# FaspDevTeam/faspsolver

Hardware: AMD Instinct MI355X
Metric: AMG-PCG solve DOF/s (3D 7-pt Poisson 256^3, classical AMG V(1,1) w-Jacobi + PCG, rtol 1e-8) (higher is better)
Workload: dtype f64

## Files before the change

### faspsolver_amd/__init__.py

```python
import ctypes as C
import os
import subprocess

import numpy as np

from . import _types as T
from ._types import *

_HERE = os.path.dirname(os.path.abspath(__file__))
LIB_PATH = os.environ.get("FASP_HIP_LIB") or os.path.join(_HERE, "libfasp_hip.so")
_lib = None

EXPORTS = [
    "fasp_param_amg_init", "fasp_param_solver_init", "fasp_solver_dcsr_krylov_amg",
    "fasp_blas_dcsr_mxv", "fasp_blas_dcsr_aAxpy", "fasp_blas_darray_dotprod",
    "fasp_blas_darray_norm2", "fasp_blas_darray_norminf", "fasp_blas_darray_axpy",
    "fasp_blas_darray_axpby", "fasp_smoother_dcsr_jacobi",
    "fasp_blas_dbsr_mxv", "fasp_blas_dbsr_aAxpy", "fasp_dbsr_getdiaginv", "fasp_smoother_dbsr_jacobi1",
    "fasp_solver_dbsr_pcg", "fasp_solver_dbsr_pbcgs", "fasp_solver_dbsr_pgmres", "fasp_solver_dbsr_pvgmres",
    "fasp_solver_dbsr_pvfgmres", "fasp_hip_bsr_precond_setup", "fasp_hip_bsr_precond_fct", "fasp_hip_bsr_precond_free",
    "fasp_hip_param_input", "fasp_fwrapper_dcsr_krylov_amg_", "fasp_dcsrvec_read2", "fasp_dvec_read",
    "fasp_dbsr_read", "fasp_dcoo_read", "fasp_dcoo_read1", "fasp_dcoo_shift_read", "fasp_dmtx_read", "fasp_dmtxsym_read", "fasp_dvec_write", "fasp_dcsr_write_coo", "fasp_dcsrvec_write2", "fasp_fwrapper_dcsr_amg_", "fasp_fwrapper_dbsr_krylov_amg_", "fasp_hip_free_bsr", "fasp_hip_comm_selftest", "fasp_hip_amg_kernel_info", "fasp_hip_coarse_kernel_info", "fasp_hip_bsr_coarse_kernel_info", "fasp_hip_coding_selftest", "fasp_solver_amg", "fasp_solver_famg", "fasp_hip_amg_solve", "fasp_precond_diag", "fasp_precond_dbsr_diag", "fasp_solver_dcsr_itsolver", "fasp_solver_dcsr_krylov", "fasp_solver_dcsr_krylov_diag", "fasp_solver_dbsr_itsolver", "fasp_solver_dbsr_krylov", "fasp_solver_dbsr_krylov_diag", "fasp_hip_mxv_csr", "fasp_hip_mxv_bsr", "fasp_solver_matfree_init", "fasp_solver_pcg", "fasp_solver_pbcgs", "fasp_solver_pgcg", "fasp_solver_pminres", "fasp_solver_pgmres", "fasp_solver_pvgmres", "fasp_solver_pvfgmres", "fasp_solver_itsolver", "fasp_solver_krylov", "fasp_solver_dcsr_pcg", "fasp_solver_dcsr_pminres", "fasp_solver_dcsr_pgcg", "fasp_solver_dcsr_pgcr", "fasp_solver_dcsr_pbcgs", "fasp_solver_dcsr_pgmres", "fasp_solver_dcsr_pvgmres",
    "fasp_solver_dcsr_pvfgmres", "fasp_hip_precond_setup", "fasp_hip_precond_fct", "fasp_hip_precond_free",
    "fasp_hip_time_bsr_mxv", "fasp_solver_dbsr_krylov_amg", "fasp_hip_bsr_amg_create", "fasp_hip_bsr_amg_create_host",
    "fasp_hip_bsr_amg_destroy", "fasp_hip_bsr_amg_num_levels", "fasp_hip_bsr_amg_get_matrix",
    "fasp_hip_bsr_amg_get_diaginv", "fasp_hip_bsr_solve",
    "fasp_hip_set_device", "fasp_hip_device_count", "fasp_hip_device_identity", "fasp_hip_available",
    "fasp_hip_amg_create", "fasp_hip_amg_create_host", "fasp_hip_amg_upload",
    "fasp_hip_amg_destroy", "fasp_hip_amg_num_levels", "fasp_hip_amg_get_matrix",
    "fasp_hip_amg_get_cfmark", "fasp_hip_solve", "fasp_hip_set_rhs", "fasp_hip_set_guess",
    "fasp_hip_solve_resident", "fasp_hip_get_solution", "fasp_hip_device_synchronize",
    "fasp_hip_precond_amg",
    "fasp_hip_poisson7pt", "fasp_hip_aniso27pt", "fasp_hip_free_system", "fasp_hip_time_kernel", "fasp_hip_measure_ceilings", "fasp_hip_amg_publish", "fasp_hip_amg_attach", "fasp_hip_amg_unpublish",
    "fasp_precond_setup", "fasp_precond_amg", "fasp_precond_famg", "fasp_precond_amli", "fasp_precond_namli", "fasp_amg_data_create", "fasp_amg_data_free", "fasp_param_amg_to_prec", "fasp_param_prec_to_amg", "fasp_mem_free", "fasp_mem_calloc", "fasp_dvec_alloc", "fasp_dvec_set", "fasp_dvec_free", "fasp_dvec_create", "fasp_dcsr_create", "fasp_dcsr_free", "fasp_smoother_dcsr_gs", "fasp_smoother_dcsr_sor", "fasp_smoother_dcsr_L1diag",
    "fasp_hip_tune", "fasp_hip_comm_unique_id", "fasp_hip_comm_init", "fasp_hip_comm_finalize",
    "fasp_hip_comm_rank", "fasp_hip_comm_size", "fasp_hip_version", "fasp_hip_comm_init_shm",
    "fasp_hip_dist_plan", "fasp_hip_dist_level_info", "fasp_hip_dist_get_matrix",
    "fasp_hip_dist_get_list",
    "fasp_blas_dcsr_vmv", "fasp_blas_dcsr_mxv_agg", "fasp_blas_dcsr_aAxpy_agg", "fasp_blas_darray_ax",
    "fasp_blas_darray_axpyz", "fasp_blas_darray_norm1", "fasp_darray_cp", "fasp_darray_set", "fasp_dvec_isnan",
    "fasp_hip_time_matrix", "fasp_hip_bsr_dist_info", "fasp_hip_seq_schedule_selftest", "fasp_hip_seq_chain_selftest", "fasp_hip_cluster_order", "fasp_hip_permute_csr", "fasp_hip_comm_init_ipc", "fasp_hip_comm_stats", "fasp_hip_comm_timing", "fasp_hip_estream_selftest", "fasp_hip_sell_selftest", "fasp_hip_level_op", "fasp_hip_matrix_op",
    "fasp_param_ilu_init", "fasp_ilu_data_create", "fasp_ilu_data_free", "fasp_mem_iludata_check", "fasp_ilu_dcsr_setup",
    "fasp_precond_ilu", "fasp_precond_ilu_forward", "fasp_precond_ilu_backward", "fasp_solver_dcsr_krylov_ilu",
    "fasp_solver_dcsr_krylov_ilu_M", "fasp_smoother_dcsr_ilu", "fasp_fwrapper_dcsr_krylov_ilu_",
    "fasp_hip_ilu_resident_count", "fasp_hip_ilu_time",
    "fasp_ilu_dbsr_setup", "fasp_precond_dbsr_ilu", "fasp_solver_dbsr_krylov_ilu", "fasp_smoother_dbsr_ilu",
    "fasp_fwrapper_dbsr_krylov_ilu_",
    "fasp_hip_bsr_amg_get_ilu", "fasp_hip_bsr_amg_ilu_info", "fasp_hip_bsr_amg_ilu_smooth_time",
]


def build(verbose=False):
    cmd = ["make", "-C", os.path.join(_HERE, "csrc")]
    if not verbose:
        cmd.insert(1, "-s")
    subprocess.run(cmd, check=True)


def lib():
    global _lib
    if _lib is not None:
        return _lib
    if not os.path.exists(LIB_PATH):
        build()
    L = C.CDLL(LIB_PATH)
    P = C.POINTER
    L.fasp_param_amg_init.argtypes = [P(T.AMG_param)]
    L.fasp_param_solver_init.argtypes = [P(T.ITS_param)]
    L.fasp_solver_dcsr_krylov_amg.argtypes = [P(T.dCSRmat), P(T.dvector), P(T.dvector),
                                              P(T.ITS_param), P(T.AMG_param)]
    L.fasp_blas_dcsr_mxv.argtypes = [P(T.dCSRmat), T.c_double_p, T.c_double_p]
    L.fasp_blas_dcsr_aAxpy.argtypes = [C.c_double, P(T.dCSRmat), T.c_double_p, T.c_double_p]
    for f in ("fasp_blas_darray_dotprod", "fasp_blas_darray_norm2", "fasp_blas_darray_norminf"):
        getattr(L, f).restype = C.c_double
    L.fasp_blas_darray_dotprod.argtypes = [C.c_int, T.c_double_p, T.c_double_p]
    L.fasp_blas_darray_norm2.argtypes = [C.c_int, T.c_double_p]
    L.fasp_blas_darray_norminf.argtypes = [C.c_int, T.c_double_p]
    L.fasp_blas_darray_axpy.argtypes = [C.c_int, C.c_double, T.c_double_p, T.c_double_p]
    L.fasp_blas_darray_axpby.argtypes = [C.c_int, C.c_double, T.c_double_p, C.c_double,
                                         T.c_double_p]
    L.fasp_blas_dcsr_vmv.restype = C.c_double
    L.fasp_blas_dcsr_vmv.argtypes = [P(T.dCSRmat), T.c_double_p, T.c_double_p]
    L.fasp_blas_dcsr_mxv_agg.argtypes = [P(T.dCSRmat), T.c_double_p, T.c_double_p]
    L.fasp_blas_dcsr_aAxpy_agg.argtypes = [C.c_double, P(T.dCSRmat), T.c_double_p, T.c_double_p]
    L.fasp_blas_darray_ax.argtypes = [C.c_int, C.c_double, T.c_double_p]
    L.fasp_blas_darray_axpyz.argtypes = [C.c_int, C.c_double, T.c_double_p, T.c_double_p, T.c_double_p]
    L.fasp_blas_darray_norm1.restype = C.c_double
    L.fasp_blas_darray_norm1.argtypes = [C.c_int, T.c_double_p]
    L.fasp_darray_cp.argtypes = [C.c_int, T.c_double_p, T.c_double_p]
    L.fasp_darray_set.argtypes = [C.c_int, T.c_double_p, C.c_double]
    L.fasp_hip_time_matrix.restype = C.c_double
    L.fasp_hip_time_matrix.argtypes = [P(T.dCSRmat), C.c_int, C.c_int, P(C.c_int)]
    L.fasp_dvec_isnan.restype = C.c_short
    L.fasp_dvec_isnan.argtypes = [P(T.dvector)]
    L.fasp_smoother_dcsr_jacobi.argtypes = [P(T.dvector), C.c_int, C.c_int, C.c_int,
                                            P(T.dCSRmat), P(T.dvector), C.c_int, C.c_double]
    L.fasp_blas_dbsr_mxv.argtypes = [P(T.dBSRmat), T.c_double_p, T.c_double_p]
    L.fasp_blas_dbsr_aAxpy.argtypes = [C.c_double, P(T.dBSRmat), T.c_double_p, T.c_double_p]
    L.fasp_dbsr_getdiaginv.argtypes = [P(T.dBSRmat)]
    L.fasp_dbsr_getdiaginv.restype = T.dvector
    L.fasp_smoother_dbsr_jacobi1.argtypes = [P(T.dBSRmat), P(T.dvector), P(T.dvector), T.c_double_p]
    L.fasp_hip_time_bsr_mxv.argtypes = [P(T.dBSRmat), C.c_int]
    L.fasp_hip_time_bsr_mxv.restype = C.c_double
    L.fasp_solver_dcsr_pcg.argtypes = [P(T.dCSRmat), P(T.dvector), P(T.dvector), P(T.precond), C.c_double,
                                       C.c_double, C.c_int, C.c_short, C.c_short]
    L.fasp_solver_dcsr_pbcgs.argtypes = L.fasp_solver_dcsr_pcg.argtypes
    L.fasp_solver_dcsr_pminres.argtypes = L.fasp_solver_dcsr_pcg.argtypes
    L.fasp_solver_dcsr_pgcg.argtypes = L.fasp_solver_dcsr_pcg.argtypes
    L.fasp_solver_dcsr_pvgmres.argtypes = [P(T.dCSRmat), P(T.dvector), P(T.dvector), P(T.precond), C.c_double,
                                           C.c_double, C.c_int, C.c_short, C.c_short, C.c_short]
    L.fasp_solver_dcsr_pvfgmres.argtypes = L.fasp_solver_dcsr_pvgmres.argtypes
    L.fasp_solver_dcsr_pgmres.argtypes = L.fasp_solver_dcsr_pvgmres.argtypes
    L.fasp_solver_dcsr_pgcr.argtypes = L.fasp_solver_dcsr_pvgmres.argtypes
    L.fasp_hip_precond_setup.argtypes = [P(T.dCSRmat), P(T.AMG_param)]
    L.fasp_hip_precond_setup.restype = P(T.precond)
    L.fasp_hip_precond_free.argtypes = [P(T.precond)]
    L.fasp_hip_precond_free.restype = None
    L.fasp_hip_precond_fct.argtypes = [T.c_double_p, T.c_double_p, C.c_void_p]
    L.fasp_hip_precond_fct.restype = None
    L.fasp_solver_dbsr_pcg.argtypes = [P(T.dBSRmat), P(T.dvector), P(T.dvector), P(T.precond), C.c_double,
                                       C.c_double, C.c_int, C.c_short, C.c_short]
    L.fasp_solver_dbsr_pbcgs.argtypes = L.fasp_solver_dbsr_pcg.argtypes
    L.fasp_solver_dbsr_pvgmres.argtypes = [P(T.dBSRmat), P(T.dvector), P(T.dvector), P(T.precond), C.c_double,
                                           C.c_double, C.c_int, C.c_short, C.c_short, C.c_short]
    L.fasp_solver_dbsr_pgmres.argtypes = L.fasp_solver_dbsr_pvgmres.argtypes
    L.fasp_solver_dbsr_pvfgmres.argtypes = L.fasp_solver_dbsr_pvgmres.argtypes
    L.fasp_hip_bsr_precond_setup.argtypes = [P(T.dBSRmat), P(T.AMG_param)]
    L.fasp_hip_bsr_precond_setup.restype = P(T.precond)
    L.fasp_hip_bsr_precond_free.argtypes = [P(T.precond)]
    L.fasp_hip_bsr_precond_free.restype = None
    L.fasp_hip_bsr_precond_fct.argtypes = [T.c_double_p, T.c_double_p, C.c_void_p]
    L.fasp_hip_bsr_precond_fct.restype = None
    L.fasp_dcsrvec_read2.argtypes = [C.c_char_p, C.c_char_p, P(T.dCSRmat), P(T.dvector)]
    L.fasp_dvec_read.argtypes = [C.c_char_p, P(T.dvector)]
    L.fasp_dbsr_read.argtypes = [C.c_char_p, P(T.dBSRmat)]
    L.fasp_hip_free_bsr.argtypes = [P(T.dBSRmat)]
    L.fasp_hip_free_bsr.restype = None
    L.fasp_hip_param_input.argtypes = [C.c_char_p, P(T.ITS_param), P(T.AMG_param)]
    L.fasp_fwrapper_dcsr_krylov_amg_.argtypes = [P(C.c_int), P(C.c_int), T.c_int_p, T.c_int_p, T.c_double_p,
                                                 T.c_double_p, T.c_double_p, P(C.c_double), P(C.c_int), P(C.c_int)]
    L.fasp_fwrapper_dcsr_krylov_amg_.restype = None
    L.fasp_hip_coding_selftest.argtypes = [P(T.dCSRmat), P(C.c_int)]
    L.fasp_hip_amg_kernel_info.argtypes = [C.c_void_p, C.c_int, C.c_int, P(C.c_int), P(C.c_double)]
    L.fasp_hip_coarse_kernel_info.argtypes = [C.c_void_p, P(C.c_int)]
    L.fasp_hip_bsr_coarse_kernel_info.argtypes = [C.c_void_p, P(C.c_int)]
    L.fasp_solver_amg.argtypes = [P(T.dCSRmat), P(T.dvector), P(T.dvector), P(T.AMG_param)]
    L.fasp_hip_amg_solve.argtypes = [C.c_void_p, P(T.dvector), P(T.dvector), P(T.AMG_param), T.c_double_p,
                                     C.c_int, P(T.fasp_hip_stats)]
    L.fasp_solver_dbsr_krylov_amg.argtypes = [P(T.dBSRmat), P(T.dvector), P(T.dvector), P(T.ITS_param),
                                              P(T.AMG_param)]
    L.fasp_hip_bsr_amg_create.argtypes = [P(C.c_void_p), P(T.dBSRmat), P(T.AMG_param)]
    L.fasp_hip_bsr_amg_create_host.argtypes = [P(C.c_void_p), P(T.dBSRmat), P(T.AMG_param)]
    L.fasp_hip_bsr_amg_destroy.argtypes = [C.c_void_p]
    L.fasp_hip_bsr_amg_destroy.restype = None
    L.fasp_hip_bsr_amg_num_levels.argtypes = [C.c_void_p]
    L.fasp_hip_bsr_amg_get_matrix.argtypes = [C.c_void_p, C.c_int, C.c_int, P(T.dBSRmat)]
    L.fasp_hip_bsr_amg_get_diaginv.argtypes = [C.c_void_p, C.c_int]
    L.fasp_hip_bsr_amg_get_diaginv.restype = T.c_double_p
    L.fasp_hip_bsr_solve.argtypes = [C.c_void_p, P(T.dvector), P(T.dvector), P(T.ITS_param), T.c_double_p,
                                     C.c_int, P(T.fasp_hip_stats)]
    L.fasp_hip_amg_create.argtypes = [P(C.c_void_p), P(T.dCSRmat), P(T.AMG_param)]
    L.fasp_hip_amg_create_host.argtypes = L.fasp_hip_amg_create.argtypes
    L.fasp_hip_amg_upload.argtypes = [C.c_void_p]
    L.fasp_hip_amg_destroy.argtypes = [C.c_void_p]
    L.fasp_hip_amg_destroy.restype = None
    L.fasp_hip_amg_num_levels.argtypes = [C.c_void_p]
    L.fasp_hip_amg_get_matrix.argtypes = [C.c_void_p, C.c_int, C.c_int, P(T.dCSRmat)]
    L.fasp_hip_amg_get_cfmark.argtypes = [C.c_void_p, C.c_int, P(T.ivector)]
    L.fasp_hip_solve.argtypes = [C.c_void_p, P(T.dvector), P(T.dvector), P(T.ITS_param),
                                 T.c_double_p, C.c_int, P(T.fasp_hip_stats)]
    L.fasp_hip_set_rhs.argtypes = [C.c_void_p, P(T.dvector)]
    L.fasp_hip_set_guess.argtypes = [C.c_void_p, P(T.dvector)]
    L.fasp_hip_get_solution.argtypes = [C.c_void_p, P(T.dvector)]
    L.fasp_hip_solve_resident.argtypes = [C.c_void_p, P(T.ITS_param), T.c_double_p, C.c_int,
                                          P(T.fasp_hip_stats)]
    L.fasp_hip_precond_amg.argtypes = [C.c_void_p, T.c_double_p, T.c_double_p]
    L.fasp_hip_poisson7pt.argtypes = [C.c_int, C.c_int, C.c_int, P(T.dCSRmat), P(T.dvector),
                                      P(T.dvector)]
    L.fasp_hip_aniso27pt.argtypes = [C.c_int, C.c_double, C.c_double, C.c_double, P(T.dCSRmat), P(T.dvector)]
    L.fasp_hip_free_system.argtypes = [P(T.dCSRmat), P(T.dvector), P(T.dvector)]
    L.fasp_hip_free_system.restype = None
    L.fasp_hip_measure_ceilings.argtypes = [P(C.c_double), C.c_size_t, C.c_int]
    L.fasp_hip_amg_publish.argtypes = [C.c_void_p, C.c_char_p]
    L.fasp_hip_amg_attach.argtypes = [P(C.c_void_p), C.c_char_p]
    L.fasp_hip_amg_unpublish.argtypes = [C.c_char_p]
    L.fasp_hip_time_kernel.restype = C.c_double
    L.fasp_hip_time_kernel.argtypes = [C.c_void_p, C.c_int, C.c_int, C.c_int]
    L.fasp_hip_tune.argtypes = [C.c_char_p, C.c_int]
    L.fasp_hip_comm_unique_id.argtypes = [C.c_char_p]
    L.fasp_hip_comm_init.argtypes = [C.c_int, C.c_int, C.c_char_p]
    L.fasp_hip_version.restype = C.c_char_p
    L.fasp_hip_comm_init_shm.argtypes = [C.c_int, C.c_int, C.c_char_p]
    L.fasp_hip_dist_plan.argtypes = [C.c_void_p, C.c_int, C.c_int, C.c_int]
    L.fasp_hip_dist_level_info.argtypes = [C.c_void_p, C.c_int, T.c_int_p]
    L.fasp_hip_dist_get_matrix.argtypes = [C.c_void_p, C.c_int, C.c_int, P(T.dCSRmat)]
    L.fasp_hip_dist_get_list.argtypes = [C.c_void_p, C.c_int, C.c_int, P(T.ivector)]
    _lib = L
    L.fasp_param_ilu_init.argtypes = [P(T.ILU_param)]
    L.fasp_param_ilu_init.restype = None
    L.fasp_ilu_data_create.argtypes = [C.c_int, C.c_int, P(T.ILU_data)]
    L.fasp_ilu_data_create.restype = None
    L.fasp_ilu_data_free.argtypes = [P(T.ILU_data)]
    L.fasp_ilu_data_free.restype = None
    L.fasp_mem_iludata_check.argtypes = [P(T.ILU_data)]
    L.fasp_mem_iludata_check.restype = C.c_short
    L.fasp_ilu_dcsr_setup.argtypes = [P(T.dCSRmat), P(T.ILU_data), P(T.ILU_param)]
    L.fasp_ilu_dcsr_setup.restype = C.c_short
    for f in ("fasp_precond_ilu", "fasp_precond_ilu_forward", "fasp_precond_ilu_backward"):
        getattr(L, f).argtypes = [T.c_double_p, T.c_double_p, C.c_void_p]
        getattr(L, f).restype = None
    L.fasp_solver_dcsr_krylov_ilu.argtypes = [P(T.dCSRmat), P(T.dvector), P(T.dvector), P(T.ITS_param), P(T.ILU_param)]
    L.fasp_solver_dcsr_krylov_ilu_M.argtypes = [P(T.dCSRmat), P(T.dvector), P(T.dvector), P(T.ITS_param),
                                                P(T.ILU_param), P(T.dCSRmat)]
    L.fasp_smoother_dcsr_ilu.argtypes = [P(T.dCSRmat), P(T.dvector), P(T.dvector), C.c_void_p]
    L.fasp_smoother_dcsr_ilu.restype = None
    L.fasp_fwrapper_dcsr_krylov_ilu_.argtypes = [P(C.c_int), P(C.c_int), T.c_int_p, T.c_int_p, T.c_double_p,
                                                 T.c_double_p, T.c_double_p, P(C.c_double), P(C.c_int), P(C.c_int)]
    L.fasp_fwrapper_dcsr_krylov_ilu_.restype = None
    L.fasp_hip_ilu_time.argtypes = [P(T.ILU_data), C.c_int, C.c_int, T.c_double_p]
    L.fasp_hip_ilu_time.restype = C.c_double
    L.fasp_ilu_dbsr_setup.argtypes = [P(T.dBSRmat), P(T.ILU_data), P(T.ILU_param)]
    L.fasp_ilu_dbsr_setup.restype = C.c_short
    L.fasp_precond_dbsr_ilu.argtypes = [T.c_double_p, T.c_double_p, C.c_void_p]
    L.fasp_precond_dbsr_ilu.restype = None
    L.fasp_solver_dbsr_krylov_ilu.argtypes = [P(T.dBSRmat), P(T.dvector), P(T.dvector), P(T.ITS_param), P(T.ILU_param)]
    L.fasp_solver_dbsr_krylov_ilu.restype = C.c_int
    L.fasp_smoother_dbsr_ilu.argtypes = [P(T.dBSRmat), P(T.dvector), P(T.dvector), C.c_void_p]
    L.fasp_smoother_dbsr_ilu.restype = None
    L.fasp_fwrapper_dbsr_krylov_ilu_.argtypes = [P(C.c_int), P(C.c_int), P(C.c_int), T.c_int_p, T.c_int_p, T.c_double_p,
                                                 T.c_double_p, T.c_double_p, P(C.c_double), P(C.c_int), P(C.c_int)]
    L.fasp_fwrapper_dbsr_krylov_ilu_.restype = None
    L.fasp_hip_bsr_amg_get_ilu.argtypes = [C.c_void_p, C.c_int, P(T.ILU_data)]
    L.fasp_hip_bsr_amg_ilu_info.argtypes = [C.c_void_p, C.c_int, T.c_double_p]
    L.fasp_hip_bsr_amg_ilu_smooth_time.argtypes = [C.c_void_p, C.c_int, C.c_int]
    L.fasp_hip_bsr_amg_ilu_smooth_time.restype = C.c_double
    return L


def solve_bsr_ilu(ia, ja, val, nb, b, x0=None, solver=None, tol=1e-8, maxit=500, lfil=0, print_level=0):
    L = lib()
    ia = np.ascontiguousarray(ia, dtype=np.int32); ja = np.ascontiguousarray(ja, dtype=np.int32)
    val = np.ascontiguousarray(val, dtype=np.float64); b = np.ascontiguousarray(b, dtype=np.float64)
    x = np.zeros(len(b)) if x0 is None else np.array(x0, dtype=np.float64)
    A = T.dBSRmat()
    A.ROW = A.COL = len(ia) - 1; A.NNZ = len(ja); A.nb = nb; A.storage_manner = 0
    A.IA = ia.ctypes.data_as(T.c_int_p); A.JA = ja.ctypes.data_as(T.c_int_p); A.val = val.ctypes.data_as(T.c_double_p)
    bv = T.dvector(len(b), b.ctypes.data_as(T.c_double_p)); xv = T.dvector(len(x), x.ctypes.data_as(T.c_double_p))
    it = T.ITS_param(); L.fasp_param_solver_init(C.byref(it))
    it.itsolver_type = T.SOLVER_BiCGstab if solver is None else solver
    it.tol, it.maxit, it.print_level = tol, maxit, print_level
    prm = T.ILU_param(); L.fasp_param_ilu_init(C.byref(prm))
    prm.ILU_lfil, prm.print_level = lfil, print_level
    st = L.fasp_solver_dbsr_krylov_ilu(C.byref(A), C.byref(bv), C.byref(xv), C.byref(it), C.byref(prm))
    return st, x


def available():
    return bool(lib().fasp_hip_available())


def param_amg_init():
    p = T.AMG_param()
    lib().fasp_param_amg_init(C.byref(p))
    return p


def param_solver_init():
    p = T.ITS_param()
    lib().fasp_param_solver_init(C.byref(p))
    return p


def poisson7pt(nx, ny=None, nz=None):
    ny = nx if ny is None else ny
    nz = nx if nz is None else nz
    A = T.dCSRmat(); b = T.dvector(); u = T.dvector()
    st = lib().fasp_hip_poisson7pt(nx, ny, nz, C.byref(A), C.byref(b), C.byref(u))
    if st < 0:
        raise RuntimeError(f"fasp_hip_poisson7pt failed: {st}")
    ia, ja, a = T.csr_arrays(A)
    f = np.ctypeslib.as_array(b.val, (b.row,)).copy()
    ue = np.ctypeslib.as_array(u.val, (u.row,)).copy()
    lib().fasp_hip_free_system(C.byref(A), C.byref(b), C.byref(u))
    return ia, ja, a, f, ue


def poisson7pt_var(n, p7=None):
    ia, ja, a, f, _ue = p7 if p7 is not None else poisson7pt(n)
    m = len(f)
    h = 1.0 / (n + 1)
    idx = np.arange(m, dtype=np.int64)
    xi = (idx % n + 1) * h
    yi = ((idx // n) % n + 1) * h
    zi = (idx // (n * n) + 1) * h
    kap = 1.0 + 0.8 * np.sin(2 * np.pi * xi) * np.sin(2 * np.pi * yi) * np.sin(2 * np.pi * zi)
    del xi, yi, zi
    cnt = np.diff(ia)
    rows = np.repeat(idx, cnt)
    off = ja != rows
    a2 = np.where(off, a * 0.5 * (kap[rows] + kap[ja]), 0.0)
    rowsum = np.bincount(rows, weights=a2, minlength=m)
    diag = -rowsum + (7 - cnt) * kap / (h * h)
    a2[ia[:-1]] = diag
    return ia, ja, a2, f.copy()


def aniso27pt(n, kx=1.0, ky=1.0, kz=0.01):
    A = T.dCSRmat(); b = T.dvector()
    st = lib().fasp_hip_aniso27pt(n, kx, ky, kz, C.byref(A), C.byref(b))
    if st < 0:
        raise RuntimeError(f"fasp_hip_aniso27pt failed: {st}")
    ia, ja, a = T.csr_arrays(A)
    f = np.ctypeslib.as_array(b.val, (b.row,)).copy()
    lib().fasp_hip_free_system(C.byref(A), C.byref(b), None)
    return ia, ja, a, f


def solver_dcsr_krylov_amg(ia, ja, a, b, x, itparam, amgparam):
    A, _keep = T.as_csr(ia, ja, a)
    bv, _b = T.as_vec(b)
    assert x.dtype == np.float64 and x.flags["C_CONTIGUOUS"]
    xv = T.dvector(x.shape[0], x.ctypes.data_as(T.c_double_p))
    return lib().fasp_solver_dcsr_krylov_amg(C.byref(A), C.byref(bv), C.byref(xv),
                                             C.byref(itparam), C.byref(amgparam))


class AMG:

    def __init__(self, ia, ja, a, amgparam, host_only=False):
        self._A, self._keep = T.as_csr(ia, ja, a)
        self.h = C.c_void_p()
        fn = lib().fasp_hip_amg_create_host if host_only else lib().fasp_hip_amg_create
        self.status = fn(C.byref(self.h), C.byref(self._A), C.byref(amgparam))
        if self.status < 0:
            self.h = C.c_void_p()
            raise RuntimeError(f"fasp_hip_amg_create failed with status {self.status}")
        self.n = self._A.row

    @classmethod
    def attach(cls, name):
        self = cls.__new__(cls)
        self._A = None; self._keep = None
        self.h = C.c_void_p()
        self.status = lib().fasp_hip_amg_attach(C.byref(self.h), name.encode())
        if self.status < 0:
            self.h = C.c_void_p()
            raise RuntimeError(f"fasp_hip_amg_attach({name}) failed with status {self.status}")
        v = T.dCSRmat()
        lib().fasp_hip_amg_get_matrix(self.h, 0, 0, C.byref(v))
        self.n = v.row
        return self

    def publish(self, name):
        st = lib().fasp_hip_amg_publish(self.h, name.encode())
        if st < 0:
            raise RuntimeError(f"fasp_hip_amg_publish({name}) failed with status {st}")

    @staticmethod
    def unpublish(name):
        lib().fasp_hip_amg_unpublish(name.encode())

    @property
    def num_levels(self):
        return lib().fasp_hip_amg_num_levels(self.h)

    def upload(self):
        st = lib().fasp_hip_amg_upload(self.h)
        if st < 0:
            raise RuntimeError(f"fasp_hip_amg_upload failed with status {st}")

    def matrix(self, level, which):
        v = T.dCSRmat()
        st = lib().fasp_hip_amg_get_matrix(self.h, level, which, C.byref(v))
        if st < 0:
            raise IndexError((level, which))
        ia, ja, val = T.csr_arrays(v)
        return v.row, v.col, ia, ja, val

    def cfmark(self, level):
        v = T.ivector()
        if lib().fasp_hip_amg_get_cfmark(self.h, level, C.byref(v)) < 0:
            raise IndexError(level)
        return np.ctypeslib.as_array(v.val, (v.row,)).copy()

    def solve(self, b, itparam, x0=None, hist_cap=600):
        x = np.zeros(self.n) if x0 is None else np.ascontiguousarray(x0, dtype=np.float64).copy()
        bv, _b = T.as_vec(b)
        xv, x = T.as_vec(x)
        hist = np.zeros(hist_cap)
        stats = T.fasp_hip_stats()
        st = lib().fasp_hip_solve(self.h, C.byref(bv), C.byref(xv), C.byref(itparam),
                                  T.dp(hist), hist_cap, C.byref(stats))
        return st, x, hist[:max(stats.nhist, 0)].copy(), stats

    def amg_solve(self, b, amgparam=None, x0=None, hist_cap=600):
        x = np.zeros(self.n) if x0 is None else np.ascontiguousarray(x0, dtype=np.float64).copy()
        bv, _b = T.as_vec(b)
        xv, x = T.as_vec(x)
        hist = np.zeros(hist_cap)
        stats = T.fasp_hip_stats()
        st = lib().fasp_hip_amg_solve(self.h, C.byref(bv), C.byref(xv),
                                      C.byref(amgparam) if amgparam is not None else None,
                                      T.dp(hist), hist_cap, C.byref(stats))
        return st, x, hist[:max(min(stats.nhist, hist_cap), 0)].copy(), stats

    def set_rhs(self, b):
        bv, _b = T.as_vec(b)
        st = lib().fasp_hip_set_rhs(self.h, C.byref(bv))
        if st < 0:
            raise RuntimeError(f"fasp_hip_set_rhs failed: {st}")

    def solve_resident(self, itparam, hist_cap=600):
        st = lib().fasp_hip_set_guess(self.h, None)
        if st < 0:
            raise RuntimeError(f"fasp_hip_set_guess failed: {st}")
        hist = np.zeros(hist_cap)
        stats = T.fasp_hip_stats()
        st = lib().fasp_hip_solve_resident(self.h, C.byref(itparam), T.dp(hist), hist_cap,
                                           C.byref(stats))
        return st, hist[:max(stats.nhist, 0)].copy(), stats

    def get_solution(self):
        x = np.zeros(self.n)
        xv, x = T.as_vec(x)
        st = lib().fasp_hip_get_solution(self.h, C.byref(xv))
        if st < 0:
            raise RuntimeError(f"fasp_hip_get_solution failed: {st}")
        return x

    def kernel_info(self, level, which=0):
        k = C.c_int(0); b = C.c_double(0)
        if lib().fasp_hip_amg_kernel_info(self.h, level, which, C.byref(k), C.byref(b)) < 0:
            raise IndexError((level, which))
        return k.value, b.value

    def coarse_kernel_info(self):
        info = (C.c_int * 8)()
        if lib().fasp_hip_coarse_kernel_info(self.h, info) < 0:
            raise RuntimeError("fasp_hip_coarse_kernel_info failed")
        return tuple(info)

    def precond(self, r):
        r = np.ascontiguousarray(r, dtype=np.float64)
        z = np.zeros_like(r)
        st = lib().fasp_hip_precond_amg(self.h, T.dp(r), T.dp(z))
        if st < 0:
            raise RuntimeError(f"fasp_hip_precond_amg failed: {st}")
        return z

    def dist_plan(self, rank, nranks, min_rows):
        st = lib().fasp_hip_dist_plan(self.h, rank, nranks, min_rows)
        if st < 0:
            raise RuntimeError(f"fasp_hip_dist_plan failed: {st}")

    def dist_info(self, level):
        info = (C.c_int * 8)()
        if lib().fasp_hip_dist_level_info(self.h, level, info) < 0:
            raise IndexError(level)
        keys = ("replicated", "nglobal", "row0", "nloc", "nghost", "nsend", "first_replicated", "nranks")
        return dict(zip(keys, list(info)))

    def dist_matrix(self, level, which):
        v = T.dCSRmat()
        if lib().fasp_hip_dist_get_matrix(self.h, level, which, C.byref(v)) < 0:
            raise IndexError((level, which))
        ia, ja, val = T.csr_arrays(v)
        return v.row, v.col, ia, ja, val

    def dist_list(self, level, which):
        v = T.ivector()
        if lib().fasp_hip_dist_get_list(self.h, level, which, C.byref(v)) < 0:
            raise IndexError((level, which))
        if v.row == 0:
            return np.zeros(0, np.int32)
        return np.ctypeslib.as_array(v.val, (v.row,)).copy()

    def time_kernel(self, kind, level=0, reps=20):
        return lib().fasp_hip_time_kernel(self.h, kind, level, reps)

    def close(self):
        if self.h:
            lib().fasp_hip_amg_destroy(self.h)
            self.h = C.c_void_p()

    def __del__(self):
        try:
            self.close()
        except Exception:
            pass


class BSRAMG:

    def __init__(self, ia, ja, val, nb, amgparam, host_only=False):
        self._A, self._keep = T.as_bsr(ia, ja, val, nb)
        self.h = C.c_void_p()
        fn = lib().fasp_hip_bsr_amg_create_host if host_only else lib().fasp_hip_bsr_amg_create
        self.status = fn(C.byref(self.h), C.byref(self._A), C.byref(amgparam))
        if self.status < 0:
            self.h = C.c_void_p()
            raise RuntimeError(f"fasp_hip_bsr_amg_create failed with status {self.status}")
        self.nb = nb
        self.n = self._A.ROW * nb

    @property
    def num_levels(self):
        return lib().fasp_hip_bsr_amg_num_levels(self.h)

    def matrix(self, level, which):
        v = T.dBSRmat()
        if lib().fasp_hip_bsr_amg_get_matrix(self.h, level, which, C.byref(v)) < 0:
            raise IndexError((level, which))
        ia = np.ctypeslib.as_array(v.IA, (v.ROW + 1,)).copy()
        ja = np.ctypeslib.as_array(v.JA, (max(v.NNZ, 1),))[:v.NNZ].copy()
        nv = v.NNZ * v.nb * v.nb
        val = np.ctypeslib.as_array(v.val, (max(nv, 1),))[:nv].copy()
        return v.ROW, v.COL, v.NNZ, ia, ja, val

    def diaginv(self, level):
        p = lib().fasp_hip_bsr_amg_get_diaginv(self.h, level)
        if not p:
            return None
        v = T.dBSRmat()
        lib().fasp_hip_bsr_amg_get_matrix(self.h, level, 0, C.byref(v))
        return np.ctypeslib.as_array(p, (v.ROW * v.nb * v.nb,)).copy()

    def ilu(self, level):
        d = T.ILU_data()
        st = lib().fasp_hip_bsr_amg_get_ilu(self.h, level, C.byref(d))
        if st < 0:
            raise IndexError(level)
        if st == 0:
            return None
        return {"nb": d.nb, "row": d.row, "nzlu": d.nzlu,
                "ijlu": np.ctypeslib.as_array(d.ijlu, (d.nzlu,)).copy(),
                "luval": np.ctypeslib.as_array(d.luval, (d.nzlu * d.nb * d.nb,)).copy()}

    def ilu_info(self, level):
        info = np.zeros(6)
        st = lib().fasp_hip_bsr_amg_ilu_info(self.h, level, T.dp(info))
        if st < 0:
            raise IndexError(level)
        return tuple(int(v) for v in info) if st else None

    def ilu_smooth_time(self, level=0, reps=20):
        return lib().fasp_hip_bsr_amg_ilu_smooth_time(self.h, level, reps)

    def solve(self, b, itparam, x0=None, hist_cap=1200):
        x = np.zeros(self.n) if x0 is None else np.ascontiguousarray(x0, dtype=np.float64).copy()
        bv, _b = T.as_vec(b)
        xv, x = T.as_vec(x)
        hist = np.zeros(hist_cap)
        stats = T.fasp_hip_stats()
        st = lib().fasp_hip_bsr_solve(self.h, C.byref(bv), C.byref(xv), C.byref(itparam), T.dp(hist),
                                      hist_cap, C.byref(stats))
        return st, x, hist[:max(min(stats.nhist, hist_cap), 0)].copy(), stats

    def precond(self, r):
        r = np.ascontiguousarray(r, dtype=np.float64).copy()
        z = np.zeros_like(r)
        lib().fasp_hip_bsr_precond_fct(T.dp(r), T.dp(z), self.h)
        return z

    def coarse_kernel_info(self):
        info = (C.c_int * 8)()
        if lib().fasp_hip_bsr_coarse_kernel_info(self.h, info) < 0:
            raise RuntimeError("fasp_hip_bsr_coarse_kernel_info failed")
        return tuple(info)

    def dist_info(self):
        info = (C.c_int * 6)()
        lib().fasp_hip_bsr_dist_info(self.h, info)
        return {"replicated": info[0], "row0": info[1], "nloc": info[2], "nghost": info[3], "first_replicated": info[4], "nb": info[5]}

    def free(self):
        if self.h:
            lib().fasp_hip_bsr_amg_destroy(self.h)
            self.h = C.c_void_p()

    def __del__(self):
        try:
            self.free()
        except Exception:
            pass


def solver_dbsr_krylov_amg(ia, ja, val, nb, b, x, itparam, amgparam):
    A, _keep = T.as_bsr(ia, ja, val, nb)
    bv, _b = T.as_vec(b)
    assert x.dtype == np.float64 and x.flags.c_contiguous
    xv = T.dvector(len(x), T.dp(x))
    return lib().fasp_solver_dbsr_krylov_amg(C.byref(A), C.byref(bv), C.byref(xv), C.byref(itparam),
                                             C.byref(amgparam))

# ... 8 lines not shown
```

### faspsolver_amd/csrc/coarse_cg.hip.h

```cpp

static bool small_coarse_ok(long long rows, long long stored_values)
{
    static int enabled = -1;
    if (enabled < 0) {
        const char* e = std::getenv("FASP_HIP_SMALL_COARSE");
        enabled = (e && std::atoi(e) == 0) ? 0 : 1;
    }
    return enabled && rows <= 4096 && stored_values <= 131072;
}
static SmallOut* small_out_dev() { return reinterpret_cast<SmallOut*>(g_ctx.d_partials2); }
static int small_out_fetch(SmallOut& o)
{
    HIPCK(hipMemcpyAsync(g_ctx.h_part, g_ctx.d_partials2, sizeof(SmallOut), hipMemcpyDeviceToHost, g_ctx.stream));
    HIPCK(hipStreamSynchronize(g_ctx.stream));
    std::memcpy(&o, g_ctx.h_part, sizeof(SmallOut));
    return 0;
}

static bool g_persist_disabled = false;
static bool build_persist_plan(fasp_hip_amg* h, int level)
{
    auto& P = h->persist;
    if (P.tried) return P.ok;
    P.tried = true;
    const HostCSR& A = h->H.L[(size_t)level].A;
    const int m = A.row;
    const int nblocks = g_ctx.num_cu, nw = (nblocks - 1) * 8;
    if (m < 1 || m > 6144 || m != A.col || nw < 8 || A.nnz <= 0) return false;
    std::vector<int> order((size_t)m), slots((size_t)m);
    for (int i = 0; i < m; ++i) { order[(size_t)i] = i; slots[(size_t)i] = (A.ia[i + 1] - A.ia[i] + 63) / 64; }
    std::stable_sort(order.begin(), order.end(), [&](int x, int y) { return slots[(size_t)x] > slots[(size_t)y]; });
    std::vector<int> load((size_t)nw, 0), cnt((size_t)nw, 0), wrow((size_t)nw * 8, -1), wend((size_t)nw * 8, 0);
    std::vector<std::pair<int, int>> heap;
    for (int w = 0; w < nw; ++w) heap.emplace_back(0, w);
    auto cmp = [](const std::pair<int, int>& x, const std::pair<int, int>& y) { return x > y; };
    std::make_heap(heap.begin(), heap.end(), cmp);
    for (int i : order) {
        if (slots[(size_t)i] == 0) continue;
        std::pop_heap(heap.begin(), heap.end(), cmp);
        std::pair<int, int> top = heap.back();
        const int w = top.second;
        if (cnt[(size_t)w] >= 8) return false;
        load[(size_t)w] += slots[(size_t)i];
        wrow[(size_t)w * 8 + cnt[(size_t)w]] = i;
        wend[(size_t)w * 8 + cnt[(size_t)w]] = load[(size_t)w];
        cnt[(size_t)w]++;
        heap.back() = std::make_pair(load[(size_t)w], w);
        std::push_heap(heap.begin(), heap.end(), cmp);
    }
    for (int i = 0; i < m; ++i) if (slots[(size_t)i] == 0) return false;
    const int maxload = *std::max_element(load.begin(), load.end());
    const int NE = maxload <= 32 ? 32 : maxload <= 48 ? 48 : maxload <= 56 ? 56 : maxload <= 64 ? 64 : 0;
    if (!NE) return false;
    const size_t tot = (size_t)nw * NE * 64;
    Buf<double> vals(tot);
    Buf<unsigned short> cols(tot);
    std::memset(vals.data(), 0, tot * sizeof(double));
    std::memset(cols.data(), 0, tot * sizeof(unsigned short));
#pragma omp parallel for schedule(dynamic, 16)
    for (int w = 0; w < nw; ++w) {
        int base = 0;
        for (int j = 0; j < cnt[(size_t)w]; ++j) {
            const int row = wrow[(size_t)w * 8 + j];
            const int kb = A.ia[row], len = A.ia[row + 1] - kb;
            for (int e = 0; e < len; ++e) {
                const size_t at = ((size_t)w * NE + base + e / 64) * 64 + (size_t)(e % 64);
                vals[at] = A.val[kb + e];
                cols[at] = (unsigned short)(A.ja[kb + e] * 8);
            }
            base = wend[(size_t)w * 8 + j];
        }
    }
    bool ok = hipMalloc(&P.vals, tot * sizeof(double)) == hipSuccess && hipMalloc(&P.cols, tot * sizeof(unsigned short)) == hipSuccess &&
              hipMalloc(&P.wrow, sizeof(int) * (size_t)nw * 8) == hipSuccess && hipMalloc(&P.wend, sizeof(int) * (size_t)nw * 8) == hipSuccess &&
              hipMalloc(&P.t2, sizeof(double) * 4 * (size_t)m) == hipSuccess && hipMalloc(&P.sync, 1024) == hipSuccess;
    if (ok) ok = hipMemcpy(P.vals, vals.data(), tot * sizeof(double), hipMemcpyHostToDevice) == hipSuccess &&
                 hipMemcpy(P.cols, cols.data(), tot * sizeof(unsigned short), hipMemcpyHostToDevice) == hipSuccess &&
                 hipMemcpy(P.wrow, wrow.data(), sizeof(int) * (size_t)nw * 8, hipMemcpyHostToDevice) == hipSuccess &&
                 hipMemcpy(P.wend, wend.data(), sizeof(int) * (size_t)nw * 8, hipMemcpyHostToDevice) == hipSuccess;
    if (ok) ok = hipMemset(P.t2, 0, sizeof(double) * 4 * (size_t)m) == hipSuccess;
    if (!ok) return false;
    P.NE = NE; P.nblocks = nblocks; P.ok = true;
    return true;
}

template <int NE>
static int launch_spcg_persist(const SpcgPersistArgs& pa, size_t lds)
{
    static bool attr = false;
    if (!attr) {
        HIPCK(hipFuncSetAttribute((const void*)k_spcg_persist<NE>, hipFuncAttributeMaxDynamicSharedMemorySize, 160 * 1024 - 1024));
        attr = true;
    }
    hipLaunchKernelGGL(k_spcg_persist<NE>, dim3(pa.nblocks - (g_tune.spcg_test_hang ? 1 : 0)), dim3(512), lds, g_ctx.stream, pa);
    return FASP_SUCCESS;
}

static int coarse_spcg(fasp_hip_amg* h, DevLevel& D, double tol, int prtlvl)
{
    const DevCSR& A = D.A;
    const int m = A.row;
    const int nn = (int)((unsigned)m * (unsigned)m);
    const int MaxIt = std::max(250, std::min(nn, 1000));
    if (small_coarse_ok(m, A.nnz)) {
        SpcgArgs a{};
        a.A = SmallCSR{m, A.ia, A.ja, A.val};
        a.b = D.b; a.u = D.x; a.p = h->cp; a.r = h->cr; a.t = h->ct; a.u_best = h->cbest;
        a.tol = tol; a.MaxIt = MaxIt; a.x_zero = D.x_zero ? 1 : 0; a.out = small_out_dev(); a.nnz = A.nnz;
        a.lazy = h->lazy_active ? h->d_lazy : nullptr;
        const size_t lds_v = sizeof(double) * 5 * (size_t)m;
        const size_t lds_m = 12 * (size_t)A.nnz + 4 * ((size_t)m + 1);
        static bool attr = false;
        if (!attr) {
            (void)hipFuncSetAttribute((const void*)k_spcg_small<true, true>, hipFuncAttributeMaxDynamicSharedMemorySize, 150 * 1024);
            (void)hipFuncSetAttribute((const void*)k_spcg_small<true, false>, hipFuncAttributeMaxDynamicSharedMemorySize, 150 * 1024);
            attr = true;
        }
        int LD = m; while (LD % 32 != 1) ++LD;
        const size_t lds_w = sizeof(double) * (128 * (size_t)LD + 128);
        const bool one_wave = g_tune.small_onewave && m <= 128 && lds_w <= 148 * 1024;
        if (one_wave && g_tune.small_onewave >= 3) {
            const int NBK = m <= 64 ? 4 : m <= 96 ? 6 : 8, DUP = NBK == 4 ? 4 : 2, RB = NBK / DUP;
            if (!h->reg_img || h->reg_mc != -NBK) {
                const HostCSR& Ah = h->H.L.back().A;
                const int NT = 16 * NBK * DUP;
                std::vector<double> img((size_t)RB * 16 * NT, 0.0);
                for (int row = 0; row < m; ++row)
                    for (int k = Ah.ia[row]; k < Ah.ia[row + 1]; ++k) {
                        const int c = Ah.ja[k], cb = c >> 4, j = c & 15, rb = row >> 4, l = row & 15;
                        const int half = rb / RB, kk = rb % RB, g = half * NBK + cb;
                        img[(size_t)(kk * 16 + j) * NT + 16 * g + l] += Ah.val[k];
                    }
                if (h->reg_img) (void)hipFree(h->reg_img);
                HIPCK(hipMalloc((void**)&h->reg_img, sizeof(double) * img.size()));
                HIPCK(hipMemcpy(h->reg_img, img.data(), sizeof(double) * img.size(), hipMemcpyHostToDevice));
                h->reg_mc = -NBK;
            }
            a.img = h->reg_img;
            const bool ahead = g_tune.small_onewave >= 4;
            h->coarse_kinfo[0] = 1; h->coarse_kinfo[1] = NBK; h->coarse_kinfo[2] = ahead ? 1 : 0;
            if (NBK == 4 && ahead) hipLaunchKernelGGL((k_spcg_dpp<4, 4, true>), dim3(1), dim3(320), 0, g_ctx.stream, a, LD);
            else if (NBK == 4) hipLaunchKernelGGL((k_spcg_dpp<4, 4, false>), dim3(1), dim3(256), 0, g_ctx.stream, a, LD);
            else if (NBK == 6 && ahead) hipLaunchKernelGGL((k_spcg_dpp<6, 2, true>), dim3(1), dim3(256), 0, g_ctx.stream, a, LD);
            else if (NBK == 6) hipLaunchKernelGGL((k_spcg_dpp<6, 2, false>), dim3(1), dim3(192), 0, g_ctx.stream, a, LD);
            else if (ahead) hipLaunchKernelGGL((k_spcg_dpp<8, 2, true>), dim3(1), dim3(320), 0, g_ctx.stream, a, LD);
            else hipLaunchKernelGGL((k_spcg_dpp<8, 2, false>), dim3(1), dim3(256), 0, g_ctx.stream, a, LD);
        }
        else if (one_wave && g_tune.small_onewave >= 2) {
            const int MC = m <= 64 ? 32 : m <= 96 ? 48 : 64;
            if (!h->reg_img || h->reg_mc != MC) {
                const HostCSR& Ah = h->H.L.back().A;
                std::vector<double> img((size_t)MC * SPCG_REG_NT, 0.0);
                for (int row = 0; row < m; ++row)
                    for (int k = Ah.ia[row]; k < Ah.ia[row + 1]; ++k) {
                        const int c = Ah.ja[k], hh = (c >> 1) & 1, kk = 2 * (c >> 2) + (c & 1);
                        if (kk < MC) img[(size_t)kk * SPCG_REG_NT + 2 * row + hh] += Ah.val[k];
                    }
                if (h->reg_img) (void)hipFree(h->reg_img);
                HIPCK(hipMalloc((void**)&h->reg_img, sizeof(double) * img.size()));
                HIPCK(hipMemcpy(h->reg_img, img.data(), sizeof(double) * img.size(), hipMemcpyHostToDevice));
                h->reg_mc = MC;
            }
            a.img = h->reg_img;
            static bool attr_r = false;
            if (!attr_r) {
                (void)hipFuncSetAttribute((const void*)k_spcg_reg<32>, hipFuncAttributeMaxDynamicSharedMemorySize, 150 * 1024);
                (void)hipFuncSetAttribute((const void*)k_spcg_reg<48>, hipFuncAttributeMaxDynamicSharedMemorySize, 150 * 1024);
                (void)hipFuncSetAttribute((const void*)k_spcg_reg<64>, hipFuncAttributeMaxDynamicSharedMemorySize, 150 * 1024);
                attr_r = true;
            }
            const size_t lds_r = sizeof(double) * (2 * (size_t)MC + 4);
            h->coarse_kinfo[0] = 2; h->coarse_kinfo[1] = MC; h->coarse_kinfo[2] = 0;
            if (m <= 64) hipLaunchKernelGGL(k_spcg_reg<32>, dim3(1), dim3(SPCG_REG_NT), lds_r, g_ctx.stream, a, LD);
            else if (m <= 96) hipLaunchKernelGGL(k_spcg_reg<48>, dim3(1), dim3(SPCG_REG_NT), lds_r, g_ctx.stream, a, LD);
            else hipLaunchKernelGGL(k_spcg_reg<64>, dim3(1), dim3(SPCG_REG_NT), lds_r, g_ctx.stream, a, LD);
        }
        else if (one_wave) {
            static bool attr_w = false;
            if (!attr_w) { (void)hipFuncSetAttribute((const void*)k_spcg_wave, hipFuncAttributeMaxDynamicSharedMemorySize, 150 * 1024); attr_w = true; }
            hipLaunchKernelGGL(k_spcg_wave, dim3(1), dim3(64), lds_w, g_ctx.stream, a, LD);
            h->coarse_kinfo[0] = 3; h->coarse_kinfo[1] = 0; h->coarse_kinfo[2] = 0;
        }
        else if (g_tune.small_lds && lds_v + lds_m <= 148 * 1024) {
            hipLaunchKernelGGL((k_spcg_small<true, true>), dim3(1), dim3(SMALL_BLOCK), lds_v + lds_m, g_ctx.stream, a);
            h->coarse_kinfo[0] = 4; h->coarse_kinfo[1] = 2; h->coarse_kinfo[2] = 0;
        }
        else if (g_tune.small_lds && lds_v <= 148 * 1024) {
            hipLaunchKernelGGL((k_spcg_small<true, false>), dim3(1), dim3(SMALL_BLOCK), lds_v, g_ctx.stream, a);
            h->coarse_kinfo[0] = 4; h->coarse_kinfo[1] = 1; h->coarse_kinfo[2] = 0;
        }
        else {
            hipLaunchKernelGGL((k_spcg_small<false, false>), dim3(1), dim3(SMALL_BLOCK), 0, g_ctx.stream, a);
            h->coarse_kinfo[0] = 4; h->coarse_kinfo[1] = 0; h->coarse_kinfo[2] = 0;
        }
        D.x_zero = false;
        if (a.lazy) return FASP_SUCCESS;
        SmallOut o;
        if (small_out_fetch(o) < 0) return ERROR_MISC;
        h->coarse_iters += o.iters;
        if (std::getenv("FASP_HIP_DEBUG_COARSE")) std::printf("[coarse small] status %d iters %d relres %.6e\n", o.status, o.iters, o.relres);
        return o.status;
    }
    const double maxdiff = tol * STAG_RATIO;
    int iter = 0, stag = 1, more_step = 1, iter_best = 0;
    double absres0 = BIGREAL, absres = BIGREAL, relres = BIGREAL, normu = BIGREAL, normr0 = BIGREAL;
    double reldiff, factor, alpha = 0.0, beta, temp1, temp2, absres_best = BIGREAL;
    double *p = h->cp, *r = h->cr, *t = h->ct, *u_best = h->cbest, *u = D.x;
    const double* b = D.b;
    double red[8];
    hipStream_t s = g_ctx.stream;
    (void)prtlvl;

    const bool fused = g_tune.spcg_fused && m <= 8000 && A.val && A.ja && !A.code && !A.pat;
    bool persist = fused && g_tune.spcg_persist && !g_persist_disabled && !comm_shares_devices() &&
                   (size_t)m * 24 <= 150 * 1024 && build_persist_plan(h, (int)(&D - &h->L[0]));
    if (!h->spcg_state) HIPCK(hipMalloc(&h->spcg_state, sizeof(SpcgState)));
    if (fused) {
        if (!D.x_zero) d_resid(A, u, b, r);
        SpcgInitArgs ia{};
        ia.m = m; ia.x_zero = D.x_zero ? 1 : 0; ia.MaxIt = MaxIt; ia.tol = tol; ia.maxdiff = maxdiff;
        ia.b = b; ia.u = u; ia.r = r; ia.p = p; ia.u_best = u_best; ia.st = h->spcg_state;
        hipLaunchKernelGGL(k_spcg_init, dim3(1), dim3(512), 0, s, ia);
        D.x_zero = false;
        goto ITERATE;
    }

    HIPCK(hipMemsetAsync(u_best, 0, sizeof(double) * m, s));

    if (D.x_zero) {
        HIPCK(hipMemcpyAsync(r, b, sizeof(double) * m, hipMemcpyDeviceToDevice, s));
        HIPCK(hipMemsetAsync(u, 0, sizeof(double) * m, s));
        D.x_zero = false;
    } else {
        d_resid(A, u, b, r);
    }
    if (d_dot(m, r, r, red) < 0) return ERROR_MISC;
    absres0 = std::sqrt(red[0]);
    normr0  = std::max(SMALLREAL, absres0);
    relres  = absres0 / normr0;
    if (relres < tol) goto FINISHED;
    HIPCK(hipMemcpyAsync(p, r, sizeof(double) * m, hipMemcpyDeviceToDevice, s));
    temp1 = red[0];

ITERATE:
    {
        int batch = std::max(1, std::min(g_tune.spcg_batch > 0 ? g_tune.spcg_batch : 8, 64));
        const int batch_next = batch;
        if (fused && h->spcg_last_iters > 0) batch = std::max(4, std::min(h->spcg_last_iters + 1, 96));
        SpcgState S{};
        if (!fused) {
            S.temp1 = temp1; S.temp1_prev = temp1; S.absres_best = absres_best; S.normr0 = normr0; S.tol = tol;
            S.maxdiff = maxdiff; S.iter = 0; S.iter_best = 0; S.stag = stag; S.MaxIt = MaxIt; S.stop = SPCG_RUN;
            S.absres = absres; S.relres = relres; S.alpha = 0.0;
            HIPCK(hipMemcpyAsync(h->spcg_state, &S, sizeof(S), hipMemcpyHostToDevice, s));
        }
        double *R[2] = {r, nullptr}, *P[2] = {p, nullptr}, *T[2] = {t, nullptr};
        SpcgBc* bc = nullptr;
        int  cur = 0;
        bool first = true;
        if (fused) {
            if (!h->spcg_fused_buf) HIPCK(hipMalloc(&h->spcg_fused_buf, sizeof(double) * (3 * (size_t)m + 4)));
            R[1] = h->spcg_fused_buf; P[1] = R[1] + m; T[1] = P[1] + m;
            bc = reinterpret_cast<SpcgBc*>(T[1] + m);
        }
        for (;;) {
            if (persist) {
                auto& PP = h->persist;
                PP.launches = (PP.launches + 1u) & 0x1fffffu;
                if (PP.launches == 0u) { HIPCK(hipMemsetAsync(PP.t2, 0, sizeof(double) * 4 * (size_t)m, s)); PP.launches = 1u; }
                SpcgPersistArgs pa{};
                pa.epoch0 = PP.launches << 11;
                pa.m = m; pa.max_steps = MaxIt + 2; pa.nblocks = PP.nblocks; pa.st = h->spcg_state;
                pa.r = r; pa.p = p; pa.u = u; pa.u_best = u_best; pa.t2 = PP.t2; pa.sync = PP.sync;
                pa.vals = PP.vals; pa.cols = PP.cols; pa.wrow = PP.wrow; pa.wend = PP.wend;
                HIPCK(hipMemsetAsync(PP.sync, 0, 1024, s));
                pa.u_lds = (sizeof(double) * 4 * (size_t)m + 1024 <= 160 * 1024) ? 1 : 0;
                const size_t lds = sizeof(double) * (pa.u_lds ? 4 : 3) * (size_t)m;
                int lst;
                if (PP.NE == 32) lst = launch_spcg_persist<32>(pa, lds);
                else if (PP.NE == 48) lst = launch_spcg_persist<48>(pa, lds);
                else if (PP.NE == 56) lst = launch_spcg_persist<56>(pa, lds);
                else lst = launch_spcg_persist<64>(pa, lds);
                if (lst < 0) return lst;
                h->coarse_kinfo[0] = 6; h->coarse_kinfo[1] = PP.NE; h->coarse_kinfo[2] = pa.u_lds;
            }
            for (int q = 0; q < batch && fused && !persist; ++q) {
                SpcgFusedArgs fa{};
                fa.m = m; fa.first = first ? 1 : 0; fa.in = cur; fa.st = h->spcg_state; fa.bc = bc;
                fa.ia = A.ia; fa.ja = A.ja; fa.ja16 = A.jbase ? nullptr : A.ja16; fa.val = A.val;
                for (int k = 0; k < 2; ++k) { fa.r[k] = R[k]; fa.p[k] = P[k]; fa.t[k] = T[k]; }
                fa.u = u; fa.u_best = u_best;
                const int cap = g_tune.spcg_grid > 0 ? g_tune.spcg_grid : 2 * g_ctx.num_cu - 1;
                const dim3 grid(1 + std::max(1, std::min((m + 7) / 8, cap)));
                const size_t lds = sizeof(double) * (size_t)m;
                if (m <= 512 * 4) hipLaunchKernelGGL(k_spcg_fused<4>, grid, dim3(512), lds, s, fa);
                else if (m <= 512 * 10) hipLaunchKernelGGL(k_spcg_fused<10>, grid, dim3(512), lds, s, fa);
                else hipLaunchKernelGGL(k_spcg_fused<16>, grid, dim3(512), lds, s, fa);
                h->coarse_kinfo[0] = 5; h->coarse_kinfo[1] = m <= 512 * 4 ? 4 : m <= 512 * 10 ? 10 : 16; h->coarse_kinfo[2] = 0;
                cur ^= 1; first = false;
            }
            for (int q = 0; q < batch && !fused; ++q) {
                CsrArgs a{}; a.x = p; a.y = t; a.dotv = p; a.partials = g_ctx.d_partials; a.stop = &h->spcg_state->stop;
                SpcgStepArgs sa{};
                sa.m = m; sa.st = h->spcg_state; sa.t = t; sa.p = p; sa.u = u; sa.r = r; sa.u_best = u_best;
                sa.ntp = launch_csr<OP_MXV_DOT>(A, a);
                sa.tp_partials = g_ctx.d_partials;
                if (m <= 512 * 4) hipLaunchKernelGGL(k_spcg_step_reg<4>, dim3(1), dim3(512), 0, s, sa);
                else if (m <= 512 * 10) hipLaunchKernelGGL(k_spcg_step_reg<10>, dim3(1), dim3(512), 0, s, sa);
                else hipLaunchKernelGGL(k_spcg_step, dim3(1), dim3(SMALL_BLOCK), 0, s, sa);
                h->coarse_kinfo[0] = 7; h->coarse_kinfo[1] = m <= 512 * 4 ? 4 : m <= 512 * 10 ? 10 : 0; h->coarse_kinfo[2] = 0;
            }
            bool spec_rr = false;
            if (persist && g_tune.spcg_spec) {
                d_resid(A, u, b, t);
                if (d_dot_to(m, t, t, 14, false) < 0) return ERROR_MISC;
                spec_rr = true;
            }
            HIPCK(hipMemcpyAsync(g_ctx.h_part, h->spcg_state, sizeof(SpcgState), hipMemcpyDeviceToHost, s));
            static_assert(sizeof(SpcgState) % 8 == 0 && sizeof(SpcgState) + 24 <= sizeof(double) * 64, "the error word and the speculative norm travel behind the state");
            if (persist) HIPCK(hipMemcpyAsync(reinterpret_cast<char*>(g_ctx.h_part) + sizeof(SpcgState), h->persist.sync, 16, hipMemcpyDeviceToHost, s));
            if (spec_rr) HIPCK(hipMemcpyAsync(reinterpret_cast<char*>(g_ctx.h_part) + sizeof(SpcgState) + 16, g_ctx.d_red + 14, 8, hipMemcpyDeviceToHost, s));
            HIPCK(hipStreamSynchronize(s));
            std::memcpy(&S, g_ctx.h_part, sizeof(S));
            double spec_val = 0.0;
            if (spec_rr) std::memcpy(&spec_val, reinterpret_cast<char*>(g_ctx.h_part) + sizeof(SpcgState) + 16, 8);
            if (persist) {
                unsigned ew[4];
                std::memcpy(ew, reinterpret_cast<char*>(g_ctx.h_part) + sizeof(SpcgState), 16);
                if (ew[3] != 0u && S.stop == SPCG_RUN) S.stop = SPCG_HANG;
            }
            iter = S.iter; absres_best = S.absres_best; iter_best = S.iter_best;
            batch = batch_next;
            if (fused) {
                normr0 = S.normr0;
                if (S.stop == SPCG_ZERO_RHS) { relres = S.relres; goto FINISHED; }
            }
#ifdef SPCG_PERSIST_STAMPS
            if (persist) {
                unsigned dbg[64];
                (void)hipMemcpy(dbg, h->persist.sync, sizeof(dbg), hipMemcpyDeviceToHost);
                std::printf("[persist stamps, 10 ns ticks, %d steps] lead:", S.iter);
                for (int q = 0; q < 8; ++q) std::printf(" %u", dbg[32 + q]);
                std::printf(" | block 1:");
                for (int q = 0; q < 8; ++q) std::printf(" %u", dbg[40 + q]);
                std::printf("   (spmv meet(second group of records + verdict) read step(tail) pass1-2 pass3 first-group-of-records(block 1) poll-rounds)\n");
            }
#endif
            if (S.stop == SPCG_HANG) {
                std::fprintf(stderr, "### WARNING: fasp_hip: the persistent coarse CG kernel timed out waiting for a block that was not "
                                     "resident (is another process using this GPU?); continuing with the per-iteration kernels\n");
                g_persist_disabled = true;
                persist = false;
                S.stop = SPCG_RUN;
                HIPCK(hipMemcpyAsync(h->spcg_state, &S, sizeof(S), hipMemcpyHostToDevice, s));
                HIPCK(hipStreamSynchronize(s));
                cur = 0; first = true;
                continue;
            }
            if (S.stop == SPCG_RUN) continue;
            if (fused && !persist) { cur = S.pad; r = R[cur]; p = P[cur]; first = true; }
            temp2 = S.tp; temp1 = S.temp1_prev;
            red[0] = S.rr; red[1] = S.uu; red[2] = S.pp; red[3] = S.maxu; red[4] = S.nan;
            alpha = S.alpha; absres = S.absres; relres = S.relres;
            if (S.stop == SPCG_DIV0) goto RESTORE_BESTSOL;
            factor = absres / absres0; (void)factor; (void)alpha;
            if (S.stop == SPCG_NAN) { absres = BIGREAL; goto RESTORE_BESTSOL; }
            if (S.stop == SPCG_SOLSTAG) { iter = ERROR_SOLVER_SOLSTAG; break; }
            if (S.stop == SPCG_MAXIT) { iter = MaxIt + 1; break; }
            normu = std::sqrt(red[1]);
            reldiff = std::fabs(S.alpha) * std::sqrt(red[2]) / normu;
            if ((stag <= MAX_STAG) & (reldiff < maxdiff)) {
                spec_rr = false;
                d_resid(A, u, b, r);
                if (d_dot(m, r, r, red) < 0) return ERROR_MISC;
                absres = std::sqrt(red[0]);
                relres = absres / normr0;
                if (relres < tol) break;
                if (stag >= MAX_STAG) { iter = ERROR_SOLVER_STAG; break; }
                HIPCK(hipMemsetAsync(p, 0, sizeof(double) * m, s));
                ++stag;
            }
            if (relres < tol) {
                if (spec_rr && S.stop != SPCG_HANG) red[0] = spec_val;
                else {
                    spec_rr = false;
                    d_resid(A, u, b, r);
                    if (d_dot(m, r, r, red) < 0) return ERROR_MISC;
                }
                absres = std::sqrt(red[0]);
                relres = absres / normr0;
                if (relres < tol) break;
                if (spec_rr) HIPCK(hipMemcpyAsync(r, t, sizeof(double) * m, hipMemcpyDeviceToDevice, s));
                if (more_step >= MAX_RESTART) { iter = ERROR_SOLVER_TOLSMALL; break; }
                HIPCK(hipMemsetAsync(p, 0, sizeof(double) * m, s));
                ++more_step;
            }
            absres0 = absres;
            temp2 = red[0];
            beta = temp2 / temp1;
            temp1 = temp2;
            d_axpby(m, 1.0, r, beta, p);
            S.temp1 = temp1; S.temp1_prev = temp1; S.stag = stag; S.stop = SPCG_RUN;
            HIPCK(hipMemcpyAsync(h->spcg_state, &S, sizeof(S), hipMemcpyHostToDevice, s));
            HIPCK(hipStreamSynchronize(s));
        }
    }

RESTORE_BESTSOL:
    if (iter != iter_best) {
        d_resid(A, u_best, b, r);
        if (d_dot(m, r, r, red) < 0) return ERROR_MISC;
        absres_best = std::sqrt(red[0]);
        if (absres > absres_best + maxdiff || std::isnan(absres)) {
            HIPCK(hipMemcpyAsync(u, u_best, sizeof(double) * m, hipMemcpyDeviceToDevice, s));
            relres = absres_best / normr0;
        }
    }
FINISHED:
    if (std::getenv("FASP_HIP_DEBUG_COARSE")) std::printf("[coarse batched] iter %d relres %.6e absres %.6e best %d\n", iter, relres, absres, iter_best);
    if (iter > 0) { h->coarse_iters += iter; h->spcg_last_iters = iter; }
    if (iter > MaxIt) return ERROR_SOLVER_MAXIT;
    return iter;
}
```

### faspsolver_amd/csrc/device_csr.hip.h

```cpp

struct DevCSR {
    int     row = 0, col = 0, nnz = 0;
    int*    ia  = nullptr;
    int*    ja  = nullptr;
    double* val = nullptr;
    int*    dpos = nullptr;
    bool    dup_diag = false;
    bool    sorted = false;
    int     lanes = 8;
    int     kind = 0;
    int     tile_rows = 256;
    int     wrows = 64, wcap = 512;
    unsigned char* code = nullptr;
    int*    rowbase = nullptr;
    int*    doff = nullptr;
    double* dval = nullptr;
    unsigned short* pat = nullptr;
    int*    pstart = nullptr;
    int*    plen = nullptr;
    int*    poff = nullptr;
    double* pval = nullptr;
    int     npat = 0, npent = 0;
    unsigned short* ja16 = nullptr;
    int*            jbase = nullptr;
// ... 829 lines not shown
    HIPCK(hipMalloc(&D.sell_tab, sizeof(double) * (size_t)S.nv));
    HIPCK(hipMemcpy(D.sell_code, S.code.data(), sizeof(unsigned) * (size_t)S.slots, hipMemcpyHostToDevice));
    HIPCK(hipMemcpy(D.sell_meta, meta.data(), sizeof(int) * meta.size(), hipMemcpyHostToDevice));
    HIPCK(hipMemcpy(D.sell_rlen, S.rlen.data(), (size_t)H.row, hipMemcpyHostToDevice));
    HIPCK(hipMemcpy(D.sell_tab, S.tab.data(), sizeof(double) * (size_t)S.nv, hipMemcpyHostToDevice));
    D.sell_nv = S.nv; D.sell_obits = S.obits; D.sell_nslice = S.nslice; D.sell_slots = S.slots;
    return FASP_SUCCESS;
}

static int upload_csr(const HostCSR& H, DevCSR& D)
{
    D.row = H.row; D.col = H.col; D.nnz = H.nnz;
    HIPCK(hipMalloc(&D.ia, sizeof(int) * ((size_t)H.row + 1)));
    HIPCK(hipMalloc(&D.ja, sizeof(int) * std::max<size_t>(H.nnz, 1)));
    HIPCK(hipMalloc(&D.val, sizeof(double) * (std::max<size_t>(H.nnz, 1) + 2)));
    HIPCK(hipMemsetAsync(D.val + std::max<size_t>(H.nnz, 1), 0, sizeof(double) * 2, g_ctx.stream));
    HIPCK(hipMemcpyAsync(D.ia, H.ia.data(), sizeof(int) * ((size_t)H.row + 1), hipMemcpyHostToDevice, g_ctx.stream));
    pick_kernel(D);
    auto upload_plain = [&]() -> int {
        HIPCK(hipMemcpyAsync(D.ja, H.ja.data(), sizeof(int) * (size_t)H.nnz, hipMemcpyHostToDevice, g_ctx.stream));
        HIPCK(hipMemcpyAsync(D.val, H.val.data(), sizeof(double) * (size_t)H.nnz, hipMemcpyHostToDevice, g_ctx.stream));
        return 0;
    };
    if (compress_enabled() && H.nnz >= 4096 && (double)H.nnz <= 48.0 * H.row) {
        Buf<unsigned short> pat; Buf<int> prb;
        std::vector<int> pstart, plen, poff; std::vector<double> pval;
        static const bool rowpat_on = !(std::getenv("FASP_HIP_ROWPAT") && std::atoi(std::getenv("FASP_HIP_ROWPAT")) == 0);
        if (rowpat_on && build_rowpat(H, pat, pstart, plen, poff, pval, prb)) {
            D.npat = (int)pstart.size(); D.npent = (int)poff.size();
            HIPCK(hipMalloc(&D.pat, sizeof(unsigned short) * ((size_t)H.row + 2)));
            HIPCK(hipMalloc(&D.pstart, sizeof(int) * pstart.size()));
            HIPCK(hipMalloc(&D.plen, sizeof(int) * plen.size()));
            HIPCK(hipMemcpy(D.plen, plen.data(), sizeof(int) * plen.size(), hipMemcpyHostToDevice));
            HIPCK(hipMalloc(&D.poff, sizeof(int) * std::max<size_t>(poff.size(), 1)));
            HIPCK(hipMalloc(&D.pval, sizeof(double) * std::max<size_t>(pval.size(), 1)));
            HIPCK(hipMemset(D.pat + H.row, 0xff, sizeof(unsigned short) * 2));
            HIPCK(hipMemcpy(D.pat, pat.data(), sizeof(unsigned short) * (size_t)H.row, hipMemcpyHostToDevice));
            HIPCK(hipMemcpy(D.pstart, pstart.data(), sizeof(int) * pstart.size(), hipMemcpyHostToDevice));
            HIPCK(hipMemcpy(D.poff, poff.data(), sizeof(int) * poff.size(), hipMemcpyHostToDevice));
            HIPCK(hipMemcpy(D.pval, pval.data(), sizeof(double) * pval.size(), hipMemcpyHostToDevice));
            if (prb.n) {
                HIPCK(hipMalloc(&D.rowbase, sizeof(int) * ((size_t)H.row + 2)));
                HIPCK(hipMemcpy(D.rowbase, prb.data(), sizeof(int) * (size_t)H.row, hipMemcpyHostToDevice));
                const int nr = H.row, npair = (nr + 1) / 2;
                long long nx = 0;
#pragma omp parallel for schedule(static) reduction(+ : nx)
                for (int w0 = 0; w0 < nr; w0 += 128) {
                    const int    pm = std::min((w0 + 64) / 2, npair - 1);
                    const unsigned domA = pat[(size_t)2 * pm], domB = (2 * pm + 1 < nr) ? pat[(size_t)2 * pm + 1] : 0xffffu;
                    for (int r = w0; r < std::min(w0 + 128, nr); r += 2) {
                        const bool vb = r + 1 < nr;
                        if (!(vb && pat[r] == domA && pat[r + 1] == domB)) nx += vb ? 2 : 1;
                    }
                }
                if (nx * 4 <= nr) D.nxrows = (int)nx;
            } else {
                D.plane = grid_plane_of(poff, H.row);
                if (std::getenv("FASP_HIP_SETUP_TIMING")) std::printf("        [upload_csr %d x %d, %d nnz] %d row patterns; grid plane for the XCD strips: %d rows\n", H.row, H.col, H.nnz, (int)pstart.size(), D.plane);
                const int nr = H.row, npair = (nr + 1) / 2;
                long long nx = 0;
#pragma omp parallel for schedule(static) reduction(+ : nx)
                for (int w0 = 0; w0 < nr; w0 += 128) {
                    const unsigned dom = pat[(size_t)2 * std::min((w0 + 64) / 2, npair - 1)];
                    for (int r = w0; r < std::min(w0 + 128, nr); r += 2) {
                        const bool vb = r + 1 < nr;
                        if (!(vb && pat[r] == dom && pat[r + 1] == dom)) nx += vb ? 2 : 1;
                    }
                }
                if (nx * 4 <= nr) D.nxrows = (int)nx;
            }
            D.kind = 2;
            return upload_plain() < 0 ? ERROR_ALLOC_MEM : FASP_SUCCESS;
        }
        std::vector<int> doff; std::vector<double> dval;
        Buf<unsigned char> code; Buf<int> rowbase;
        if (build_dict8(H, doff, dval, code, rowbase)) {
            HIPCK(hipMalloc(&D.code, (size_t)H.nnz + 256));
            HIPCK(hipMalloc(&D.doff, sizeof(int) * 256));
            HIPCK(hipMalloc(&D.dval, sizeof(double) * 256));
            HIPCK(hipMemcpy(D.code, code.data(), (size_t)H.nnz, hipMemcpyHostToDevice));
            HIPCK(hipMemcpy(D.doff, doff.data(), sizeof(int) * 256, hipMemcpyHostToDevice));
            HIPCK(hipMemcpy(D.dval, dval.data(), sizeof(double) * 256, hipMemcpyHostToDevice));
            if (rowbase.n) {
                HIPCK(hipMalloc(&D.rowbase, sizeof(int) * (size_t)H.row));
                HIPCK(hipMemcpy(D.rowbase, rowbase.data(), sizeof(int) * (size_t)H.row, hipMemcpyHostToDevice));
            }
            D.kind = 2;
            return upload_plain() < 0 ? ERROR_ALLOC_MEM : FASP_SUCCESS;
        }
    }
    static const bool sort_long = !(std::getenv("FASP_HIP_SORT_LONG_ROWS") && std::atoi(std::getenv("FASP_HIP_SORT_LONG_ROWS")) == 0);
    static const int  sort_stream = std::getenv("FASP_HIP_SORT_STREAM") ? std::atoi(std::getenv("FASP_HIP_SORT_STREAM")) : 0;
    const double avg_len = H.row > 0 ? (double)H.nnz / H.row : 0.0;
    const bool do_sort = sort_long && !g_oneshot_upload && H.nnz > 0 && (D.kind == 0 || (D.kind == 2 && sort_stream > 0 && avg_len >= sort_stream));
    static const bool timing = std::getenv("FASP_HIP_SETUP_TIMING") != nullptr;
    double tp = wall_seconds();
    auto lap = [&](const char* what) {
        if (!timing) return;
        const double now = wall_seconds();
        std::printf("        [upload_csr %d x %d, %d nnz] %-10s %8.3f s\n", H.row, H.col, H.nnz, what, now - tp);
        tp = now;
    };
    if (do_sort && D.kind == 0) {
        int maxlen = 0;
#pragma omp parallel for schedule(static) reduction(max : maxlen)
        for (int i = 0; i < H.row; ++i) maxlen = std::max(maxlen, H.ia[i + 1] - H.ia[i]);
        if (g_device_sort && maxlen <= SORT_MAXLEN) {
            const int st = upload_sorted_on_device(H, D, maxlen);
            lap("device sort");
            return st < 0 ? st : build_estream(H.ia.data(), H.row, H.nnz, D);
        }
    }
    if (do_sort) {
        Buf<int> sj((size_t)H.nnz);
        Buf<double> sv((size_t)H.nnz);
        std::vector<int> dp;
        const bool square = H.row == H.col;
        if (square) dp.assign((size_t)H.row, -1);
#pragma omp parallel
        {
            std::vector<std::pair<int, double>> tmp;
#pragma omp for schedule(dynamic, 64)
            for (int i = 0; i < H.row; ++i) {
                const int kb = H.ia[i], ke = H.ia[i + 1];
                tmp.resize((size_t)(ke - kb));
                for (int k = kb; k < ke; ++k) tmp[(size_t)(k - kb)] = {H.ja[k], H.val[k]};
                std::stable_sort(tmp.begin(), tmp.end(),
                                 [](const std::pair<int, double>& x, const std::pair<int, double>& y) { return x.first < y.first; });
                for (int k = kb; k < ke; ++k) {
                    sj[k] = tmp[(size_t)(k - kb)].first; sv[k] = tmp[(size_t)(k - kb)].second;
                    if (square && sj[k] == i) dp[(size_t)i] = k;
                }
            }
        }
        lap("row sort");
        HIPCK(hipMemcpy(D.ja, sj.data(), sizeof(int) * (size_t)H.nnz, hipMemcpyHostToDevice));
        HIPCK(hipMemcpy(D.val, sv.data(), sizeof(double) * (size_t)H.nnz, hipMemcpyHostToDevice));
        lap("memcpy");
        if (square && D.kind == 2) {
            HIPCK(hipMalloc(&D.dpos, sizeof(int) * (size_t)std::max(H.row, 1)));
            HIPCK(hipMemcpy(D.dpos, dp.data(), sizeof(int) * (size_t)H.row, hipMemcpyHostToDevice));
        }
        D.sorted = true;
        if (upload_ja16(D, H.ia.data(), sj.data()) < 0) return ERROR_ALLOC_MEM;
        return build_estream(H.ia.data(), H.row, H.nnz, D);
    }
    if (upload_plain() < 0) return ERROR_ALLOC_MEM;
    if (D.kind == 2 && !g_oneshot_upload && build_xtile(H, D) < 0) return ERROR_ALLOC_MEM;
    if (D.kind == 2 && compress_enabled() && upload_sell(H, D) < 0) return ERROR_ALLOC_MEM;
    if (upload_ja16(D, H.ia.data(), H.ja.data()) < 0) return ERROR_ALLOC_MEM;
    return build_estream(H.ia.data(), H.row, H.nnz, D);
}

struct Tuning { int ilu_smooth_fused = 1, gen2 = 2, ws2_bpc = 3, maxgrid = -1, xcd = 16, nt = 1, kind = -1, lanes = -1, wrows = -1, wcap = -1, compress = 1, rpl = -1, lds_tab = 1, xcd_pat = 64, spcg_batch = 16, small_lds = 1, ja16 = 1, spcg_fused = 1, spcg_grid = 0, spcg_persist = 1, split_rows = 0, gs_multicolor = 0, seq_flow = 1, seq_strip_kb = 0, seq_jobs = 1, seq_spine = 1, seq_grid = 0, seq_chain = 1, seq_chain_n1 = 0, seq_chain_grid = 0, seq_chain_ref = 0, seq_test_hang = 0, seq_rest_lanes = 0, local_square = 1, fuse_zr = 1, fuse_presmooth = 1, seq_lanes = 0, xtile = 1, rp5_max = 45, rp_bpc = 5, rp_xcd = -1, rp_strip = 2, spcg_test_hang = 0, small_onewave = 4, lazy_coarse = 1, rp_stream = -1, renumber = 1, renumber_chunk = 262144, pcg_dev_beta = 1, spcg_spec = 1, ev_every = 4, pcg_fold = 1, seq_chain_touch = 8, seq_chain_touch_t1 = 1, seq_zero_skip = 1, estream = 1, es_dbg = 0, ilu_form = -1, sell = 1; };
static Tuning g_tune;

template <class K>
static int resident_blocks_per_cu(K kernel)
{
    static std::vector<std::pair<const void*, int>> cache;
    const void* key = reinterpret_cast<const void*>(kernel);
    for (const auto& e : cache)
        if (e.first == key) return e.second;
    int nb = 0;
    if (hipOccupancyMaxActiveBlocksPerMultiprocessor(&nb, kernel, BLOCK, 0) != hipSuccess || nb < 1) nb = 4;
    nb = std::min(nb, 8);
    cache.emplace_back(key, nb);
    return nb;
}

template <class K>
static int launch_persistent(K kernel, int ntiles, CsrArgs& a, int blocks_per_cu = 0)
{
    int cap = (blocks_per_cu > 0 ? std::min(blocks_per_cu, resident_blocks_per_cu(kernel)) : resident_blocks_per_cu(kernel)) * g_ctx.num_cu;
    if (g_tune.maxgrid > 0) cap = g_tune.maxgrid;
    cap = std::min(cap, MAXGRID);
    int grid = std::min(cap, ntiles);
    grid = std::max(8, (grid + 7) / 8 * 8);
    hipLaunchKernelGGL(kernel, dim3(grid), dim3(BLOCK), 0, g_ctx.stream, a);
    return grid;
}

static bool sell_active(const DevCSR& M) { return M.sell_code && g_tune.compress && g_tune.sell && g_tune.gen2 >= 2 && !(g_tune.xtile && M.lja16); }
template <int OP>
static int launch_sell(const DevCSR& M, CsrArgs& a)
{
    a.sell_code = M.sell_code; a.sell_sptr = M.sell_meta; a.sell_sbase = M.sell_meta + M.sell_nslice + 1; a.sell_rlen = M.sell_rlen;
    a.sell_tab = M.sell_tab; a.sell_nv = M.sell_nv; a.sell_obits = M.sell_obits;
    const size_t lds = sizeof(double) * ((size_t)M.sell_nv + SELL_NW);
    static bool attr_set = false;
    if (!attr_set) {
        (void)hipFuncSetAttribute(reinterpret_cast<const void*>(k_csr_sell<OP>), hipFuncAttributeMaxDynamicSharedMemorySize, (int)(sizeof(double) * (SELL_MAXV + SELL_NW)));
        attr_set = true;
    }
    static std::vector<std::pair<size_t, int>> cache;
    int nb = 0;
    for (const auto& e : cache)
        if (e.first == lds) nb = e.second;
    if (nb == 0) {
        if (hipOccupancyMaxActiveBlocksPerMultiprocessor(&nb, k_csr_sell<OP>, SELL_BLOCK, lds) != hipSuccess || nb < 1) nb = 1;
        nb = std::min(nb, 2);
        cache.emplace_back(lds, nb);
    }
    int cap = nb * g_ctx.num_cu;
    if (g_tune.maxgrid > 0) cap = g_tune.maxgrid;
    cap = std::min(cap, MAXGRID);
    int grid = std::min(cap, a.ntiles);
    grid = std::max(8, (grid + 7) / 8 * 8);
    hipLaunchKernelGGL(k_csr_sell<OP>, dim3(grid), dim3(SELL_BLOCK), lds, g_ctx.stream, a);
    return grid;
}

template <int OP>
static int launch_rowpat5(CsrArgs& a)
{
    if constexpr (OP == OP_JACOBI || OP == OP_L1DIAG) { (void)a; return 0; }
    else return launch_persistent(k_csr_rowpat5<OP>, a.ntiles, a, 5);
}

constexpr int WIN_ALIGN = DIST_WIN_ALIGN;
struct RowWin { int lo = 0, hi = -1, goff = 0; };
static bool g_jacobi_dot_done = false;

__global__ __launch_bounds__(BLOCK) void k_bridge_gather(int n, const int* __restrict__ perm, const double* __restrict__ s, double* __restrict__ y,
                                                         double* __restrict__ zx, const double* __restrict__ zdiag, double zomega)
{
    for (int k = blockIdx.x * BLOCK + threadIdx.x; k < n; k += gridDim.x * BLOCK) {
        const double v = s[perm[k]];
        y[k] = v;
        if (zx) { const double di = zdiag[k]; zx[k] = (fabs(di) > 1e-20) ? (1 - zomega) * 0.0 + zomega * v / di : 0.0; }
    }
}
__global__ __launch_bounds__(BLOCK) void k_bridge_scatter(int n, const int* __restrict__ perm, const double* __restrict__ x, double* __restrict__ s)
{
    for (int k = blockIdx.x * BLOCK + threadIdx.x; k < n; k += gridDim.x * BLOCK) s[perm[k]] = x[k];
}

template <int OP>
static int launch_csr(const DevCSR& M0, CsrArgs a, RowWin win = RowWin())
{
    if (M0.bridge && win.hi < 0) {
        DevCSR Mn = M0;
        Mn.bridge = nullptr; Mn.bscratch = nullptr; Mn.bridge_dir = 0;
        if (M0.bridge_dir == 1 && OP == OP_MXV) {
            CsrArgs b = a;
            b.y = M0.bscratch; b.zx = nullptr; b.zdiag = nullptr;
            const int G = launch_csr<OP>(Mn, b);
            const int grid = std::max(1, std::min(MAXGRID, (M0.row + BLOCK - 1) / BLOCK));
            hipLaunchKernelGGL(k_bridge_gather, dim3(grid), dim3(BLOCK), 0, g_ctx.stream, M0.row, M0.bridge, (const double*)M0.bscratch, a.y, a.zx, a.zdiag, a.zomega);
            return G;
        }
        if (M0.bridge_dir == 2 && (OP == OP_ADD || OP == OP_SUB || OP == OP_AXPY || OP == OP_MXV)) {
            const int grid = std::max(1, std::min(MAXGRID, (M0.col + BLOCK - 1) / BLOCK));
            hipLaunchKernelGGL(k_bridge_scatter, dim3(grid), dim3(BLOCK), 0, g_ctx.stream, M0.col, M0.bridge, a.x, M0.bscratch);
            CsrArgs b = a;
            b.x = M0.bscratch;
            return launch_csr<OP>(Mn, b);
        }
        std::fprintf(stderr, "### ERROR: fasp_hip: operation %d on a transfer operator with a numbering bridge (direction %d)\n", (int)OP, M0.bridge_dir);
        std::abort();
    }
    if (win.hi < 0 && g_tune.split_rows > 0 && M0.row >= 4 * WIN_ALIGN) {
        const int lo = std::min(g_tune.split_rows, M0.row / 4) / WIN_ALIGN * WIN_ALIGN, hi = (M0.row - lo) / WIN_ALIGN * WIN_ALIGN;
        RowWin w; w.lo = lo; w.hi = hi; w.goff = 0;
        int G = launch_csr<OP>(M0, a, w);
        w.lo = 0; w.hi = lo; w.goff = G;
        G += launch_csr<OP>(M0, a, w);
        w.lo = hi; w.hi = M0.row; w.goff = G;
        return G + launch_csr<OP>(M0, a, w);
    }
    DevCSR M = M0;
    const int w_lo = win.hi >= 0 ? win.lo : 0, w_hi = win.hi >= 0 ? std::min(win.hi, M0.row) : M0.row;
    if (w_hi <= w_lo && win.hi >= 0) return 0;
    if (a.partials) a.partials += win.goff;
    auto set_tiles = [&](int rpb) {
        if (win.hi >= 0 && rpb > 0 && (w_lo % rpb) != 0) {
            std::fprintf(stderr, "### ERROR: fasp_hip: row window at %d with a kernel tile of %d rows (a tuning knob broke the window alignment)\n", w_lo, rpb);
            std::abort();
        }
        a.nrow = w_hi; a.row_lo = w_lo; a.tile0 = w_lo / rpb;
        a.ntiles = (w_hi - w_lo + rpb - 1) / rpb;
        a.tiles_per_xcd = (a.ntiles + 7) / 8;
    };
    auto strips = [&](int rpb) {
        if (!g_tune.rp_strip || M.plane < 8 * rpb || M.plane % (8 * rpb) != 0 || a.ntiles < 4 * (M.plane / rpb)) return false;
        a.xcd_map = -2; a.tpp = M.plane / rpb; a.tiles_per_xcd = a.tpp / 8;
        return true;
    };
    if (M.code && g_tune.compress) M.kind = 4;
    if (M.pat && g_tune.compress) M.kind = 5;
    if (g_tune.kind >= 0 && !(g_tune.kind == 4 && !M.code) && !(g_tune.kind == 5 && !M.pat)) M.kind = g_tune.kind;
    if (g_tune.lanes > 0) M.lanes = g_tune.lanes;
    if (g_tune.wrows > 0) M.wrows = g_tune.wrows;
    if (g_tune.wcap > 0) M.wcap = g_tune.wcap;
    const bool lstream_ok = g_tune.gen2 && M.kind == 2 && M.wrows == 64 && M.wcap == 512 && (double)M.nnz <= 7.6 * M.row;
    if (OP == OP_JACOBI && M.kind != 0 && M.kind < 4 && (M.dup_diag || !M.dpos) && !lstream_ok) M.kind = 0;
    a.xcd_map = g_tune.xcd;
    a.nt = g_tune.nt;
    if (g_tune.rp_stream > 0 || (g_tune.rp_stream < 0 && (size_t)M.row * 8 > (size_t)96 << 20)) a.nt |= 4;
    a.nrow = M.row; a.ia = M.ia; a.ja = M.ja; a.val = M.val; a.dpos = M.dpos;
    a.ja16 = g_tune.ja16 ? M.ja16 : nullptr;
    a.jbase = g_tune.ja16 ? M.jbase : nullptr;
    if (M.jbase && M.kind != 0) { a.ja16 = nullptr; a.jbase = nullptr; }
    if (M.kind == 1 || M.kind == 3) M.kind = 0;
    const int rpb = M.kind >= 4 ? BLOCK : M.kind == 2 ? 4 * M.wrows : BLOCK / M.lanes;
    set_tiles(rpb);
    if (M.kind == 5 && g_tune.gen2 && M.nxrows >= 0 && !M.rowbase && g_tune.rpl <= 0) {
// ... 185 lines not shown
```

### faspsolver_amd/csrc/hierarchy.hip.h

```cpp

struct DevLevel {
    DevCSR  A, P, R;
    double* diag = nullptr;
    double* l1   = nullptr;
    double *b = nullptr, *xa = nullptr, *xb = nullptr, *w = nullptr;
    double* x  = nullptr;
    double* xo = nullptr;
    bool    x_zero = true;
    bool    presmoothed = false;
    double* halo_pending = nullptr;
    bool    owns_b = true;
    bool    replicated = true;
    int     nloc = 0;
    int     nvec = 0;
    int     row0 = 0;
    int     nglobal = 0;
    std::vector<int> send_off, recv_off;
    int*    d_send_idx = nullptr;
    double* d_sendbuf  = nullptr;
    bool    has_halo() const { return !replicated && nvec > nloc; }
    struct Sched {
        bool built = false, multicolor = false; int* d_order = nullptr; int* d_ptr = nullptr; std::vector<int> ptr;
        int ns = 0, L = 1, LR = 1, pfmax = 1, kt = 0, par = 1, nstrips = 0, nchunk = 0, maxent = 0; bool nolower = false, flow_ok = false, rowlevels = false, independent = false; int nrows = 0, nvirt = 0, nclasses = 0; long long nghost = 0, slot_bytes = 0;
        std::vector<int> cptr;
        void* d_strips = nullptr; void* d_chunks = nullptr; unsigned char* d_slots = nullptr; int* d_gpos = nullptr; int* d_cstrip = nullptr; int* d_lchunks = nullptr;
        int* d_ria = nullptr; int* d_rja = nullptr; double* d_rval = nullptr; double* d_rec = nullptr; double* d_dr = nullptr; int* d_tr = nullptr; double* d_W = nullptr; unsigned* d_prog = nullptr;
        bool chain = false; int nb = 0, npad = 0, n1b = 0, rx = 0, rg = 0; long long t1_steps = 0, t2_steps = 0, nband = 0, nt1 = 0, nt2 = 0;
        double* d_band = nullptr; double* d_drd = nullptr; void* d_blk = nullptr; double* d_t1v = nullptr; double* d_t2v = nullptr;
        unsigned short* d_t1c = nullptr; unsigned short* d_t2c = nullptr; double* d_G2 = nullptr; int* d_t1need = nullptr; int* d_t2need = nullptr;
        std::vector<void*> owned;
        void release()
        {
            if (!owned.empty()) { for (void* q : owned) (void)hipFree(q); owned.clear(); }
            else { if (d_order) (void)hipFree(d_order); if (d_ptr) (void)hipFree(d_ptr); }
            d_order = nullptr; d_ptr = nullptr; built = false;
        }
    };
    Sched   sched[5];
    struct Poly { bool built = false; double* dinv = nullptr; double k[6] = {0, 0, 0, 0, 0, 0}; double* w[5] = {nullptr, nullptr, nullptr, nullptr, nullptr}; };
    Poly    poly;
    int*    d_perm = nullptr;
    bool    diag_uniform = false;
    double  diag_value = 0.0;
    int*    d_mark = nullptr;
    double* w2 = nullptr;
    double* kw[4] = {nullptr, nullptr, nullptr, nullptr};
};

struct EventPair { hipEvent_t a, b; };

}

using namespace fasp;

struct SchedJob { int level = 0, kind = 0, st = 0; bool uploaded = false; SplitHost H; DevLevel::Sched S; std::thread th; };

struct fasp_hip_amg {
    std::vector<std::vector<int>> perm;
    std::vector<std::unique_ptr<SchedJob>> sched_jobs;
    bool                  sched_jobs_started = false;
    std::mutex            sched_mu;
    HostHierarchy         H;
    DistPlan              dist;
    bool                  distributed = false;
    std::vector<DevLevel> L;
    AMG_param             param;
    bool                  want_zr = false;
    bool                  pre_marked = false;
    int                   zr_G = 0;
    double *b = nullptr, *u = nullptr, *p = nullptr, *t = nullptr, *r = nullptr;
    double *cp = nullptr, *cr = nullptr, *ct = nullptr, *cbest = nullptr;
    std::vector<double*> gm[2];
    size_t               gm_len[2] = {0, 0};
    double*              gm_hh = nullptr;
    double*              spcg_fused_buf = nullptr;
    int                  spcg_last_iters = 0;
    SpcgState*           spcg_state = nullptr;
    struct Persist { bool tried = false, ok = false; int NE = 0, nblocks = 0; double* vals = nullptr; unsigned short* cols = nullptr;
                     int *wrow = nullptr, *wend = nullptr; double* t2 = nullptr; unsigned* sync = nullptr; unsigned launches = 0; } persist;
    std::vector<double>  amli_coef;
    std::vector<int>     level_cycle_type;
    bool                 use_fmg = false;
    std::vector<EventPair> ev;
    int                    ev_used = 0;
    long long              coarse_iters = 0, vcycles = 0;
    int                    coarse_kinfo[6] = {0, 0, 0, 0, 0, 0};
    int*                   d_lazy = nullptr; int* h_lazy = nullptr; bool lazy_active = false, coarse_sync = false;
    double*                reg_img = nullptr; int reg_mc = 0;
    double                 upload_seconds = 0.0;
};

namespace fasp {

static void free_level(DevLevel& D)
{
    D.A.release(); D.P.release(); D.R.release();
    if (D.diag) (void)hipFree(D.diag);
    if (D.l1) (void)hipFree(D.l1);
    if (D.b && D.owns_b) (void)hipFree(D.b);
    if (D.xa) (void)hipFree(D.xa);
    if (D.xb) (void)hipFree(D.xb);
    if (D.w) (void)hipFree(D.w);
    if (D.d_send_idx) (void)hipFree(D.d_send_idx);
    if (D.d_sendbuf) (void)hipFree(D.d_sendbuf);
    for (auto& sc : D.sched) sc.release();
    if (D.poly.dinv) (void)hipFree(D.poly.dinv);
    for (double* q : D.poly.w) if (q) (void)hipFree(q);
    if (D.d_mark) (void)hipFree(D.d_mark);
    if (D.d_perm) (void)hipFree(D.d_perm);
    D.d_perm = nullptr;
    if (D.w2) (void)hipFree(D.w2);
    for (double* q : D.kw) if (q) (void)hipFree(q);
    D = DevLevel();
}

static int alloc_vec(double** p, size_t n)
{
    HIPCK(hipMalloc(p, sizeof(double) * std::max<size_t>(n, 1)));
    return FASP_SUCCESS;
}

static int upload_diag(const HostCSR& A, DevLevel& D)
{
    const int n = A.row;
    std::vector<double> d(n, 0.0), s(n, 0.0);
    std::vector<int>    dp(n, -1);
    int                 ndup = 0;
#pragma omp parallel for schedule(static) reduction(+ : ndup)
    for (int i = 0; i < n; ++i) {
        double di = 0.0, si = 0.0;
        int    hits = 0;
        for (int k = A.ia[i]; k < A.ia[i + 1]; ++k) {
            if (A.ja[k] == i) { di = A.val[k]; dp[i] = k; ++hits; }
            si += (A.val[k] >= 0.0) ? A.val[k] : -A.val[k];
        }
        d[i] = di; s[i] = si;
        if (hits > 1) ++ndup;
    }
    D.A.dup_diag = ndup > 0;
    {
        bool same = n > 0;
        for (int i = 1; i < n && same; ++i) same = std::memcmp(&d[(size_t)i], &d[0], sizeof(double)) == 0;
        D.diag_uniform = same;
        D.diag_value = same ? d[0] : 0.0;
    }
    if (!D.A.sorted) {
        HIPCK(hipMalloc(&D.A.dpos, sizeof(int) * std::max(n, 1)));
        HIPCK(hipMemcpy(D.A.dpos, dp.data(), sizeof(int) * n, hipMemcpyHostToDevice));
    }
    if (alloc_vec(&D.diag, n) < 0 || alloc_vec(&D.l1, n) < 0) return ERROR_ALLOC_MEM;
    HIPCK(hipMemcpy(D.diag, d.data(), sizeof(double) * n, hipMemcpyHostToDevice));
    HIPCK(hipMemcpy(D.l1, s.data(), sizeof(double) * n, hipMemcpyHostToDevice));
    return FASP_SUCCESS;
}

__global__ __launch_bounds__(BLOCK) void k_pack(int n, const int* __restrict__ idx,
                                                 const double* __restrict__ v, double* __restrict__ out)
{
    for (int i = blockIdx.x * BLOCK + threadIdx.x; i < n; i += gridDim.x * BLOCK) out[i] = v[idx[i]];
}

static int halo_exchange(DevLevel& D, double* v, hipStream_t stream = nullptr)
{
    if (!stream) stream = g_ctx.stream;
    if (D.replicated || comm_size() <= 1 || D.send_off.empty()) return FASP_SUCCESS;
    const int P = comm_size(), me = comm_rank();
    const int nsend = D.send_off.back();
    if (nsend > 0)
        hipLaunchKernelGGL(k_pack, dim3(vec_grid(nsend)), dim3(BLOCK), 0, stream, nsend, D.d_send_idx, v,
                           D.d_sendbuf);
    std::vector<CommXfer> sends, recvs;
    for (int q = 0; q < P; ++q) {
        if (q == me) continue;
        const int ns = D.send_off[q + 1] - D.send_off[q], nr = D.recv_off[q + 1] - D.recv_off[q];
        if (ns > 0) sends.push_back({q, D.d_sendbuf + D.send_off[q], (size_t)ns});
        if (nr > 0) recvs.push_back({q, v + D.nloc + D.recv_off[q], (size_t)nr});
    }
    const int st = comm_exchange(sends.data(), (int)sends.size(), recvs.data(), (int)recvs.size(), stream);
    if (st < 0) comm_mark_failed();
    return st;
}

static int g_seq_partition = std::getenv("FASP_HIP_SEQ_PARTITION") && std::atoi(std::getenv("FASP_HIP_SEQ_PARTITION")) != 0;
static int g_halo_overlap = 1;

static int g_coarse_mode = -1, g_coarse_split_min = 16384;
static bool coarse_split_active(const DevCSR& M)
{
    return (g_coarse_mode == 1 || (g_coarse_mode < 0 && comm_is_peer_window())) && comm_size() > 1 && M.row >= g_coarse_split_min;
}
template <int OP>
static int rep_launch(const DevCSR& M, CsrArgs a)
{
    if (!coarse_split_active(M) || a.partials || a.zx) return launch_csr<OP>(M, a);
    const int P = comm_size(), me = comm_rank();
    const int nwin = (M.row + WIN_ALIGN - 1) / WIN_ALIGN, per = (nwin + P - 1) / P;
    std::vector<int> counts((size_t)P), displs((size_t)P);
    for (int q = 0; q < P; ++q) {
        const int lo = std::min(M.row, q * per * WIN_ALIGN), hi = std::min(M.row, (q + 1) * per * WIN_ALIGN);
        displs[(size_t)q] = lo; counts[(size_t)q] = hi - lo;
    }
    RowWin w; w.lo = displs[(size_t)me]; w.hi = w.lo + counts[(size_t)me]; w.goff = 0;
    int G = 0;
    if (w.hi > w.lo) G = launch_csr<OP>(M, a, w);
    if (comm_allgatherv(a.y + w.lo, counts[(size_t)me], a.y, counts.data(), displs.data(), g_ctx.stream) < 0) { comm_mark_failed(); return -1; }
    return G;
}

template <int OP>
static int dist_launch(DevLevel& V, const DevCSR& M, CsrArgs a, const DevLevel* Out = nullptr)
{
    double* v = const_cast<double*>(a.x);
    if (V.replicated && (!Out || Out->replicated) && comm_size() > 1) return rep_launch<OP>(M, a);
    if (V.replicated || comm_size() <= 1 || V.send_off.empty()) return launch_csr<OP>(M, a);
    if (!g_halo_overlap || M.win_hi < 0) {
        if (halo_exchange(V, v) < 0) return -1;
        return launch_csr<OP>(M, a);
    }
    bool local_ok = hipEventRecord(g_ctx.ev_ready, g_ctx.stream) == hipSuccess &&
                    hipStreamWaitEvent(g_ctx.comm_stream, g_ctx.ev_ready, 0) == hipSuccess;
    if (!local_ok) {
        comm_mark_failed();
        (void)hipStreamSynchronize(g_ctx.stream);
        (void)halo_exchange(V, v);
        (void)launch_csr<OP>(M, a);
        return -1;
    }
    RowWin w;
    w.lo = M.win_lo; w.hi = M.win_hi; w.goff = 0;
    int G = launch_csr<OP>(M, a, w);
    const int hst = halo_exchange(V, v, g_ctx.comm_stream);
    if (hipEventRecord(g_ctx.ev_halo, g_ctx.comm_stream) != hipSuccess ||
// ... 214 lines not shown
```

### faspsolver_amd/csrc/small_solvers.hip.h

```cpp
#pragma once

#include <hip/hip_runtime.h>

namespace fasp {

constexpr int SMALL_BLOCK = 512;
constexpr int SMALL_WAVES = SMALL_BLOCK / 64;
constexpr int SMALL_MAX_RESTART = 32;
constexpr int GM_NE = 16;

struct SmallOut {
    int    status;
    int    iters;
    double relres, absres;
};

__device__ __forceinline__ double dpp_mov_f64(double x, const int ctrl, const int row_mask)
{
    const long long b = __double_as_longlong(x);
    int lo = (int)(b & 0xffffffffll), hi = (int)(b >> 32);
    switch (ctrl) {
        case 0x111: lo = __builtin_amdgcn_update_dpp(0, lo, 0x111, 0xf, 0xf, true); hi = __builtin_amdgcn_update_dpp(0, hi, 0x111, 0xf, 0xf, true); break;
        case 0x112: lo = __builtin_amdgcn_update_dpp(0, lo, 0x112, 0xf, 0xf, true); hi = __builtin_amdgcn_update_dpp(0, hi, 0x112, 0xf, 0xf, true); break;
        case 0x114: lo = __builtin_amdgcn_update_dpp(0, lo, 0x114, 0xf, 0xf, true); hi = __builtin_amdgcn_update_dpp(0, hi, 0x114, 0xf, 0xf, true); break;
// ... 1608 lines not shown
                    for (int st = 1; st < i; ++st) {
                        const double nc = ns * shr1(cur) + bj;
                        cur = (tid >= 1) ? nc : cur;
                    }
                    const double np = g_s * hl + g_c * shr1(cur);
                    const double curL = rdl(cur, i - 1);
                    double g = t * t;
                    g += curL * curL;
                    double gamma = sqrt(g);
                    if (gamma == 0.0) gamma = epsmac;
                    const double ci = curL / gamma, si = t / gamma;
                    const double rsi = -si * rprev, rsp = ci * rprev;
                    const double hfin = si * t + ci * curL;
                    g_c = (tid == i) ? ci : g_c;
                    g_s = (tid == i) ? si : g_s;
                    if (tid >= 1 && tid < i) hh[(tid - 1) * R + (i - 1)] = np;
                    if (tid == 0) {
                        hh[(i - 1) * R + (i - 1)] = hfin; hh[i * R + (i - 1)] = t;
                        c[i - 1] = ci; sn[i - 1] = si; rs[i] = rsi; rs[i - 1] = rsp; sc_rnorm = fabs(rsi);
                    }
                }
            } else {
            for (int j = 0; j < i; ++j) {
                const double* pj = P(j);
                double hv[1] = {0.0};
                for (int e = tid; e < n; e += SMALL_BLOCK) hv[0] += pj[e] * pi[e];
                blk_reduce1<1>(hv, sh2, par);
                const double h = hv[0];
                if (tid == 0) hh[j * R + (i - 1)] = h;
                for (int e = tid; e < n; e += SMALL_BLOCK) pi[e] += -h * pj[e];
            }
            {
                double tv[1] = {0.0};
                for (int e = tid; e < n; e += SMALL_BLOCK) tv[0] += pi[e] * pi[e];
                blk_reduce1<1>(tv, sh2, par);
                t = sqrt(tv[0]);
            }
            if (t != 0.0) {
                const double s = 1.0 / t;
                for (int e = tid; e < n; e += SMALL_BLOCK) pi[e] *= s;
            }
            }
            if (!(n <= 64 * GM_NE)) GMT(2);
            if (!(n <= 64 * GM_NE) && tid == 0) {
                hh[i * R + (i - 1)] = t;
                for (int j = 1; j < i; ++j) {
                    const double tt = hh[(j - 1) * R + (i - 1)];
                    hh[(j - 1) * R + (i - 1)] = sn[j - 1] * hh[j * R + (i - 1)] + c[j - 1] * tt;
                    hh[j * R + (i - 1)] = -sn[j - 1] * tt + c[j - 1] * hh[j * R + (i - 1)];
                }
                double g = hh[i * R + (i - 1)] * hh[i * R + (i - 1)];
                g += hh[(i - 1) * R + (i - 1)] * hh[(i - 1) * R + (i - 1)];
                double gamma = sqrt(g);
                if (gamma == 0.0) gamma = epsmac;
                c[i - 1] = hh[(i - 1) * R + (i - 1)] / gamma;
                sn[i - 1] = hh[i * R + (i - 1)] / gamma;
                rs[i] = -sn[i - 1] * rs[i - 1];
                rs[i - 1] = c[i - 1] * rs[i - 1];
                hh[(i - 1) * R + (i - 1)] = sn[i - 1] * hh[i * R + (i - 1)] + c[i - 1] * hh[(i - 1) * R + (i - 1)];
                sc_rnorm = fabs(rs[i]);
            }
            GMT(3);
            __syncthreads();
            GMT(4);
            absres = r_norm = sc_rnorm;
            relres = absres / absres0;
            if (relres < tol) break;
        }

        if (tid == 0) {
            rs[i - 1] = rs[i - 1] / hh[(i - 1) * R + (i - 1)];
            for (int k = i - 2; k >= 0; k--) {
                double tt = 0.0;
                int j = k + 1;
                for (; j + 5 < i; j += 6) {
                    double hv[6], rv[6];
#pragma unroll
                    for (int e = 0; e < 6; ++e) { hv[e] = hh[k * R + j + e]; rv[e] = rs[j + e]; }
#pragma unroll
                    for (int e = 0; e < 6; ++e) tt -= hv[e] * rv[e];
                }
                for (; j < i; j++) tt -= hh[k * R + j] * rs[j];
                tt += rs[k];
                rs[k] = tt / hh[k * R + k];
            }
        }
        __syncthreads();
        for (int e = tid; e < n; e += SMALL_BLOCK) {
            double we = P(i - 1)[e] * rs[i - 1];
            for (int j = i - 2; j >= 0; j--) we += rs[j] * P(j)[e];
            w[e] = we;
            x[e] += we;
        }
        __syncthreads();

        if (relres < tol) {
            g_resid(x, b, w);
            r_norm = sqrt(blk_dot(n, w, w, sh));
            absres = r_norm;
            relres = absres / absres0;
            if (relres < tol) break;
            for (int e = tid; e < n; e += SMALL_BLOCK) P(0)[e] = w[e];
            i = 0;
        }

        if (tid == 0)
            for (int j = i; j > 0; j--) {
                rs[j - 1] = -sn[j - 1] * rs[j];
                rs[j] = c[j - 1] * rs[j];
            }
        __syncthreads();
        if (i) {
            double* pi = P(i);
            double* p0 = P(0);
            for (int e = tid; e < n; e += SMALL_BLOCK) {
                double v = pi[e];
                v = v + (rs[i] - 1.0) * v;
                for (int j = i - 1; j > 0; j--) v += rs[j] * P(j)[e];
                pi[e] = v;
                double q = p0[e];
                q = q + (rs[0] - 1.0) * q;
                p0[e] = q + v;
            }
        }
        __syncthreads();
        cr = r_norm / r_norm_old;
    }

FINISHED:
#ifdef GM_TIMING
    if (tid == 0 && iter > 20) printf("[gmres_small] iters %d: other %.2f spmv %.2f (wavefront 0: rows < 512 %.2f, rows >= 512 %.2f, barrier %.2f) mgs %.2f givens %.2f barrier %.2f us per iteration\n", iter, gmt[0] * 0.01 / iter, (gmt[1] + gmt[5] + gmt[6]) * 0.01 / iter, gmt[5] * 0.01 / iter, gmt[6] * 0.01 / iter, gmt[1] * 0.01 / iter, gmt[2] * 0.01 / iter, gmt[3] * 0.01 / iter, gmt[4] * 0.01 / iter);
#endif
    if (tid == 0) {
        a.out->iters = iter;
        a.out->status = iter >= MaxIt ? -48 : iter;
        a.out->relres = relres;
        a.out->absres = absres;
    }
}

constexpr int SPCG_HANG = 8;
#ifndef SPCG_POLL_GROUP
#define SPCG_POLL_GROUP 6
#endif

struct SpcgPersistArgs {
    int        m, max_steps, nblocks;
    int        u_lds;
    SpcgState* st;
    double    *r, *p, *u, *u_best;
    double*    t2;
    unsigned*  sync;
    unsigned   epoch0;
    const double*         vals;
    const unsigned short* cols;
    const int*            wrow;
    const int*            wend;
};

__device__ __forceinline__ void lds_barrier()
{
    asm volatile("s_waitcnt lgkmcnt(0)\n\ts_barrier" ::: "memory");
}
template <int NQ, int NW>
__device__ __forceinline__ void blk_reduce_dpp(double (&v)[NQ], double* sh, unsigned maxmask = 0u)
{
    const int lane = threadIdx.x & 63, w = threadIdx.x >> 6;
#pragma unroll
    for (int q = 0; q < NQ; ++q) {
        const bool mx = (maxmask >> q) & 1u;
        const double x = mx ? wave_max_to_lane63(v[q]) : wave_sum_to_lane63(v[q]);
        if (lane == 63) sh[w * NQ + q] = x;
    }
    lds_barrier();
#pragma unroll
    for (int q = 0; q < NQ; ++q) {
        const bool mx = (maxmask >> q) & 1u;
        double x = sh[q];
        for (int k = 1; k < NW; ++k) {
            const double y = sh[k * NQ + q];
            x = mx ? fmax(x, y) : x + y;
        }
        v[q] = x;
    }
    lds_barrier();
}

__device__ __forceinline__ bool absres_improves(double rr, double best, double maxdiff) { return sqrt(rr) < best - maxdiff; }

template <int NE, bool LEAD>
__device__ __forceinline__ void spcg_persist_body(const SpcgPersistArgs& a)
{
    constexpr int NT = 512, NW = 8, E = 12, CH = 6;
    extern __shared__ __attribute__((aligned(16))) double dyn[];
    __shared__ double sh[NW * 4];
    __shared__ int    s_flag;
    typedef __attribute__((address_space(1))) unsigned           gu32;
    typedef __attribute__((address_space(1))) unsigned long long gu64;
    const int tid = threadIdx.x, lane = tid & 63, m = a.m;
    const int wave = __builtin_amdgcn_readfirstlane(tid >> 6);
    constexpr bool lead = LEAD;
    double* sp = dyn;
    double* sr = dyn + m;
    double* st = dyn + 2 * m;
    double* su = dyn + 3 * m;
    gu32* g_err = (gu32*)(a.sync + 3);
    gu64* g_verdict = (gu64*)(a.sync + 8);
    __shared__ int s_hang;
    typedef unsigned int pu32x4 __attribute__((ext_vector_type(4)));
    SpcgState& S = *a.st;
    if (S.stop != SPCG_RUN) return;

    double   v[NE];
    unsigned cpk[NE / 2];
    int      my_rows = 0, endsv = 0, rowsv = -1;
    if (!lead) {
        const int gw = ((int)blockIdx.x - 1) * NW + wave;
        const double* pv = a.vals + ((size_t)gw * NE) * 64 + lane;
        const unsigned short* pc = a.cols + ((size_t)gw * NE) * 64 + lane;
#pragma unroll
        for (int k = 0; k < NE; ++k) v[k] = __builtin_nontemporal_load(pv + (size_t)k * 64);
#pragma unroll
        for (int k = 0; k < NE / 2; ++k)
            cpk[k] = (unsigned)__builtin_nontemporal_load(pc + (size_t)(2 * k) * 64) |
                     ((unsigned)__builtin_nontemporal_load(pc + (size_t)(2 * k + 1) * 64) << 16);
        if (lane < 8) { endsv = a.wend[gw * 8 + lane]; rowsv = a.wrow[gw * 8 + lane]; }
        my_rows = __popcll(__ballot(lane < 8 && rowsv >= 0));
    }
    for (int i = tid; i < m; i += NT) { sp[i] = a.p[i]; sr[i] = a.r[i]; }
    const bool u_lds = a.u_lds != 0;
    if (lead && u_lds) for (int i = tid; i < m; i += NT) su[i] = a.u[i];
    double temp1 = S.temp1;
    const double absres_best0 = S.absres_best, normr0 = S.normr0, tol = S.tol, maxdiff = S.maxdiff;
    const int    it0 = S.iter, stag = S.stag, MaxIt = S.MaxIt;
    double best = absres_best0;
    int    iter_best = S.iter_best;
    double o_tp = S.tp, o_rr = S.rr, o_uu = S.uu, o_pp = S.pp, o_maxu = S.maxu, o_nan = S.nan, o_alpha = S.alpha,
           o_absres = S.absres, o_relres = S.relres, o_temp1_prev = S.temp1_prev;
    int steps_done = 0, my_stop = SPCG_RUN;
    if (tid == 0) {
        s_hang = 0;
        if (lead)
            __hip_atomic_store(g_verdict, ((unsigned long long)(a.epoch0 + 1u) << 32) | (unsigned)SPCG_RUN, __ATOMIC_RELAXED, __HIP_MEMORY_SCOPE_AGENT);
    }
    __syncthreads();
#ifdef SPCG_PERSIST_STAMPS
    unsigned long long tk[8] = {0, 0, 0, 0, 0, 0, 0, 0}, tl = __builtin_amdgcn_s_memrealtime();
#define STAMP(q) do { const unsigned long long tn_ = __builtin_amdgcn_s_memrealtime(); tk[q] += tn_ - tl; tl = tn_; } while (0)
#else
#define STAMP(q) do { } while (0)
#endif

    for (int step = 0; step < a.max_steps; ++step) {
        const int par = step & 1;
        const unsigned ep = a.epoch0 + (unsigned)step + 1u;
        const __amdgpu_buffer_rsrc_t tr =
            __builtin_amdgcn_make_buffer_rsrc(a.t2 + (size_t)par * 2 * m, 0, (int)((unsigned)m * 16u), 0x00020000);
        if (!lead && my_rows > 0 && my_stop == SPCG_RUN) {
            double acc = 0.0;
            int    j = 0;
            int    next_end = __builtin_amdgcn_readlane(endsv, 0);
#pragma unroll
            for (int k = 0; k < NE; ++k) {
                const unsigned off = (k & 1) ? (cpk[k >> 1] >> 16) : (cpk[k >> 1] & 0xffffu);
                const double x = *reinterpret_cast<const double*>(reinterpret_cast<const char*>(sp) + off);
                acc += v[k] * x;
                if ((k & 7) == 7) __builtin_amdgcn_sched_barrier(0);
                if (k + 1 == next_end) {
                    const double ssum = wave_sum_to_lane63(acc);
                    const int row = __builtin_amdgcn_readlane(rowsv, j);
                    if (lane == 63) {
                        const unsigned long long bits = (unsigned long long)__double_as_longlong(ssum);
                        const pu32x4 rec = {(unsigned)bits, ep, (unsigned)(bits >> 32), ep};
                        __builtin_amdgcn_raw_buffer_store_b128(rec, tr, row * 16, 0, 16 );
                    }
                    acc = 0.0;
                    ++j;
                    next_end = (j < 8) ? __builtin_amdgcn_readlane(endsv, j & 7) : -1;
                    if (j >= my_rows) next_end = -1;
                }
            }
        }
        STAMP(0);
        {
            const unsigned long long t0 = __builtin_amdgcn_s_memrealtime();
            bool hung = false;
            unsigned long long vr0 = 0ull;
            if (tid == 0) vr0 = __hip_atomic_load(g_verdict + par, __ATOMIC_RELAXED, __HIP_MEMORY_SCOPE_AGENT);
#pragma unroll 1
            for (int e0 = 0; e0 < E && !hung; e0 += SPCG_POLL_GROUP) {
#ifdef SPCG_PERSIST_STAMPS
                if (e0 == 6 && !LEAD) STAMP(6);
#endif
                unsigned pend = 0u;
#pragma unroll
                for (int e = 0; e < SPCG_POLL_GROUP; ++e) if (tid + (e0 + e) * NT < m) pend |= 1u << e;
                while (pend) {
#ifdef SPCG_PERSIST_STAMPS
                    tk[7] += 1;
#endif
                    pu32x4 q[SPCG_POLL_GROUP];
#pragma unroll
                    for (int e = 0; e < SPCG_POLL_GROUP; ++e)
                        q[e] = __builtin_amdgcn_raw_buffer_load_b128(tr, ((pend >> e) & 1u) ? (tid + (e0 + e) * NT) * 16 : (int)0xfffffff0u, 0, 16 );
#pragma unroll
                    for (int e = 0; e < SPCG_POLL_GROUP; ++e)
                        if (((pend >> e) & 1u) && q[e].y == ep && q[e].w == ep) {
                            st[tid + (e0 + e) * NT] = __longlong_as_double((long long)(((unsigned long long)q[e].z << 32) | q[e].x));
                            pend &= ~(1u << e);
                        }
                    if (pend && __builtin_amdgcn_s_memrealtime() - t0 > 200000000ull) { hung = true; break; }
                }
            }
            if (tid == 0 && !hung) {
                int flag = -1;
                for (bool first = true;; first = false) {
                    const unsigned long long vr = first ? vr0 : __hip_atomic_load(g_verdict + par, __ATOMIC_RELAXED, __HIP_MEMORY_SCOPE_AGENT);
                    if ((unsigned)(vr >> 32) == ep) { flag = (int)(unsigned)vr; break; }
                    __builtin_amdgcn_s_sleep(1);
                    if (__builtin_amdgcn_s_memrealtime() - t0 > 200000000ull) { hung = true; break; }
                }
                s_flag = flag;
            }
            if (hung) {
                s_hang = 1;
                __hip_atomic_store(g_err, 1u, __ATOMIC_RELAXED, __HIP_MEMORY_SCOPE_AGENT);
            }
        }
        lds_barrier();
        STAMP(1);
        if (s_hang) { my_stop = SPCG_HANG; break; }
        const int flag = s_flag;
        if (flag != SPCG_RUN) break;
        if (my_stop != SPCG_RUN) break;
        STAMP(2);
        double v1[1] = {0.0};
#pragma unroll 1
        for (int e0 = 0; e0 < E; e0 += CH) {
            double tv[CH], pv[CH];
#pragma unroll
            for (int e = 0; e < CH; ++e) { const int i = min(tid + (e0 + e) * NT, m - 1); tv[e] = st[i]; pv[e] = sp[i]; }
#pragma unroll
            for (int e = 0; e < CH; ++e) if (tid + (e0 + e) * NT < m) v1[0] += tv[e] * pv[e];
        }
        blk_reduce_dpp<1, NW>(v1, sh);
        const double tp = v1[0];
        if (!(fabs(tp) > 1e-40)) {
            o_tp = tp; steps_done = step + 1; my_stop = SPCG_DIV0;
            break;
        }
        const double alpha = temp1 / tp;
        double red[3] = {0.0, 0.0, 0.0};
#pragma unroll 1
        for (int e0 = 0; e0 < E; e0 += CH) {
            double tv[CH], rv[CH], pv[CH], uv[CH];
#pragma unroll
            for (int e = 0; e < CH; ++e) {
                const int i = min(tid + (e0 + e) * NT, m - 1);
                tv[e] = st[i]; rv[e] = sr[i];
                pv[e] = lead ? sp[i] : 0.0;
                uv[e] = lead ? (u_lds ? su[i] : a.u[i]) : 0.0;
            }
#pragma unroll
            for (int e = 0; e < CH; ++e) {
                const int i = tid + (e0 + e) * NT;
                if (i < m) {
                    const double rn = rv[e] - alpha * tv[e];
                    sr[i] = rn;
                    red[0] += rn * rn;
                    if (lead) {
                        const double ui = uv[e] + alpha * pv[e];
                        if (u_lds) su[i] = ui; else a.u[i] = ui;
                        red[1] += ui * ui; red[2] += pv[e] * pv[e];
                    }
                }
            }
        }
        double maxu = 1.0, nan_u = 0.0;
        if (lead) {
            blk_reduce_dpp<3, NW>(red, sh);
            nan_u = (red[1] != red[1]) ? 1.0 : 0.0;
            if (!(red[1] > 2.0 * m * 1e-40)) {
                double mx[1] = {0.0};
                for (int i = tid; i < m; i += NT) mx[0] = fmax(mx[0], fabs(u_lds ? su[i] : a.u[i]));
                blk_reduce_dpp<1, NW>(mx, sh, 1u);
                maxu = mx[0];
            }
        } else {
            double r1[1] = {red[0]};
            blk_reduce_dpp<1, NW>(r1, sh);
            red[0] = r1[0];
        }
        const double rr = red[0], beta = rr / temp1;
        STAMP(4);
        const bool keep_best = lead && absres_improves(rr, best, maxdiff);
        if (lead) {
            const int it = it0 + step + 1;
            STAMP(6);
            const double sq = sqrt(lane == 0 ? rr : lane == 1 ? red[1] : red[2]);
            auto bc = [&](double x, int from) -> double {
                const unsigned long long bb = (unsigned long long)__double_as_longlong(x);
                const unsigned lo = (unsigned)__builtin_amdgcn_readlane((int)(unsigned)bb, from);
                const unsigned hi = (unsigned)__builtin_amdgcn_readlane((int)(unsigned)(bb >> 32), from);
                return __longlong_as_double((long long)(((unsigned long long)hi << 32) | lo));
            };
            const double absres = bc(sq, 0), normu = bc(sq, 1), sq_pp = bc(sq, 2);
            const double fac = fabs(alpha) * sq_pp;
            const double qd = (lane == 0 ? absres : fac) / (lane == 0 ? normr0 : normu);
            const double relres = bc(qd, 0), reldiff = bc(qd, 1);
            int stop = SPCG_RUN;
            if (nan_u > 0.0) stop = SPCG_NAN;
            else {
                if (absres < best - maxdiff) { best = absres; iter_best = it; }
                if (maxu <= 1e-20) stop = SPCG_SOLSTAG;
                else if ((stag <= 20) & (reldiff < maxdiff)) stop = SPCG_STAG;
                else if (relres < tol) stop = SPCG_CONV;
                if (stop == SPCG_RUN && it >= MaxIt) stop = SPCG_MAXIT;
            }
            o_tp = tp; o_rr = rr; o_uu = red[1]; o_pp = red[2]; o_maxu = maxu; o_nan = nan_u;
            o_alpha = alpha; o_absres = absres; o_relres = relres; o_temp1_prev = temp1;
            my_stop = stop;
            if (tid == 0)
                __hip_atomic_store(g_verdict + (par ^ 1), ((unsigned long long)(ep + 1u) << 32) | (unsigned)stop, __ATOMIC_RELAXED,
                                   __HIP_MEMORY_SCOPE_AGENT);
        }
#pragma unroll 1
        for (int e0 = 0; e0 < E; e0 += CH) {
            double rv[CH], pv[CH];
#pragma unroll
            for (int e = 0; e < CH; ++e) {
                const int i = min(tid + (e0 + e) * NT, m - 1);
                rv[e] = sr[i]; pv[e] = sp[i];
            }
#pragma unroll
            for (int e = 0; e < CH; ++e) {
                const int i = tid + (e0 + e) * NT;
                if (i < m) {
                    sp[i] = 1.0 * rv[e] + beta * pv[e];
                    if (keep_best) a.u_best[i] = u_lds ? su[i] : a.u[i];
                }
            }
        }
        STAMP(5);
        temp1 = rr;
        steps_done = step + 1;
        lds_barrier();
        STAMP(3);
    }
#ifdef SPCG_PERSIST_STAMPS
    if (tid == 0 && blockIdx.x < 2)
        for (int q = 0; q < 8; ++q) a.sync[32 + blockIdx.x * 8 + q] = (unsigned)tk[q];
#endif
#undef STAMP

    if (lead) {
        for (int i = tid; i < m; i += NT) { a.r[i] = sr[i]; a.p[i] = sp[i]; if (u_lds) a.u[i] = su[i]; }
        if (tid == 0) {
            S.tp = o_tp; S.rr = o_rr; S.uu = o_uu; S.pp = o_pp; S.maxu = o_maxu; S.nan = o_nan;
            S.alpha = o_alpha; S.absres = o_absres; S.relres = o_relres;
            S.absres_best = best; S.iter_best = iter_best; S.iter = it0 + steps_done;
            S.temp1_prev = o_temp1_prev;
            S.temp1 = (my_stop == SPCG_DIV0) ? S.temp1 : temp1;
            S.stop = my_stop;
        }
    }
}

template <int NE>
__global__ __launch_bounds__(512) void k_spcg_persist(SpcgPersistArgs a)
{
    if (blockIdx.x == 0) spcg_persist_body<NE, true>(a);
    else spcg_persist_body<NE, false>(a);
}

}
```

### faspsolver_amd/csrc/solver.hip

```cpp
#include <hip/hip_runtime.h>

#include <fcntl.h>
#include <omp.h>
#include <sys/mman.h>
#include <sys/stat.h>
#include <unistd.h>

#include <algorithm>
#include <cfloat>
#include <cmath>
#include <cstdio>
#include <cstdlib>
#include <cstring>
#include <functional>
#include <condition_variable>
#include <memory>
#include <mutex>
#include <string>
#include <thread>
#include <vector>

#include "fasp_comm.h"
#include "fasp_internal.h"
#include "kernels.hip.h"
// ... 376 lines not shown
        st = host_setup_rs(A, amgparam, h->H);
        g_on_level_ready = nullptr; g_on_level_matrix = nullptr; g_on_level_ready_ctx = nullptr;
        lap("host setup");
        if (st >= 0) {
            { std::lock_guard<std::mutex> lk(up.mu); up.coarsest = (int)h->H.L.size() - 1; }
            AheadUpload::on_ready((int)h->H.L.size() - 1, &up);
        }
        { std::lock_guard<std::mutex> lk(up.mu); up.done = true; }
        up.cv.notify_one();
        up.th.join();
        lap("wait for the level uploads");
        if (st >= 0) st = up.status;
        {
            const int last = (int)h->H.L.size() - 1;
            std::lock_guard<std::mutex> lk(h->sched_mu);
            for (auto& J : h->sched_jobs)
                if (J && J->level >= last) {
                    if (J->th.joinable()) J->th.join();
                    if (J->uploaded) J->S.release();
                    J.reset();
                }
        }
        if (st < 0) { h->L.resize(h->H.L.size()); fasp_hip_amg_destroy(h); return st; }
        h->param = *amgparam;
    } else {
        st = fasp_hip_amg_create_host(&h, A, amgparam);
        if (st < 0) return st;
        lap("host setup");
    }
    try { st = upload_hierarchy(h); }
    catch (const std::bad_alloc&) { std::printf("### ERROR: fasp_hip: host allocation failed during the upload\n"); st = ERROR_ALLOC_MEM; }
    lap("upload_hierarchy");
    if (st < 0) { fasp_hip_amg_destroy(h); return st; }
    *out = h;
    return FASP_SUCCESS;
}

void fasp_hip_amg_destroy(fasp_hip_amg* h)
{
    FASP_ENTRY();
    if (h) sched_jobs_join(h);
    if (!h) return;
    if (g_ctx.ready) (void)hipStreamSynchronize(g_ctx.stream);
    for (auto& D : h->L) free_level(D);
    double* v[] = {h->b, h->u, h->p, h->t, h->r, h->cp, h->cr, h->ct, h->cbest};
    for (double* q : v)
        if (q) (void)hipFree(q);
    if (h->d_lazy) (void)hipFree(h->d_lazy);
    if (h->reg_img) (void)hipFree(h->reg_img);
    if (h->h_lazy) (void)hipHostFree(h->h_lazy);
    for (auto& e : h->ev) { (void)hipEventDestroy(e.a); (void)hipEventDestroy(e.b); }
    for (int s = 0; s < 2; ++s)
        for (double* q : h->gm[s])
            if (q) (void)hipFree(q);
    if (h->gm_hh) (void)hipFree(h->gm_hh);
    if (h->spcg_state) (void)hipFree(h->spcg_state);
    if (h->spcg_fused_buf) (void)hipFree(h->spcg_fused_buf);
    {
        auto& P = h->persist;
        void* q[] = {P.vals, P.cols, P.wrow, P.wend, P.t2, P.sync};
        for (void* x : q) if (x) (void)hipFree(x);
    }
    ShmMapping map{nullptr, 0};
    for (size_t q = 0; q < g_attached.size(); ++q)
        if (g_attached[q].first == h) { map = g_attached[q].second; g_attached.erase(g_attached.begin() + (long)q); break; }
    delete h;
    if (map.base) munmap(map.base, map.bytes);
}

int fasp_hip_coding_selftest(const dCSRmat* A, int* kind_out)
{
    FASP_ENTRY();
    if (!A || !kind_out) return ERROR_INPUT_PAR;
    HostCSR M;
    M.row = A->row; M.col = A->col; M.nnz = A->nnz;
    M.ia.alloc((size_t)A->row + 1); M.ja.alloc((size_t)std::max(A->nnz, 1)); M.val.alloc((size_t)std::max(A->nnz, 1));
    std::memcpy(M.ia.data(), A->IA, sizeof(int) * ((size_t)A->row + 1));
    std::memcpy(M.ja.data(), A->JA, sizeof(int) * (size_t)A->nnz);
    std::memcpy(M.val.data(), A->val, sizeof(double) * (size_t)A->nnz);
    const bool square = M.row == M.col;
    *kind_out = 0;
    if (!(M.nnz >= 4096 && (double)M.nnz <= 48.0 * M.row)) return FASP_SUCCESS;
    auto bits = [](double v) { unsigned long long b; std::memcpy(&b, &v, 8); return b; };
    {
        Buf<unsigned short> pat; Buf<int> rb;
        std::vector<int> pstart, plen, poff; std::vector<double> pval;
        if (build_rowpat(M, pat, pstart, plen, poff, pval, rb)) {
            *kind_out = 5;
            for (int r = 0; r < M.row; ++r) {
                const int id = pat[r], base = square ? r : rb[r];
                if (plen[id] != M.ia[r + 1] - M.ia[r]) return ERROR_MISC;
                for (int j = 0; j < plen[id]; ++j) {
                    const int k = M.ia[r] + j;
                    if (base + poff[pstart[id] + j] != M.ja[k] || bits(pval[pstart[id] + j]) != bits(M.val[k])) return ERROR_MISC;
                }
                for (int j = plen[id]; j < (plen[id] + 7) / 8 * 8; ++j)
                    if (poff[pstart[id] + j] != 0 || bits(pval[pstart[id] + j]) != 0ull) return ERROR_MISC;
            }
            return FASP_SUCCESS;
        }
    }
    {
        std::vector<int> doff; std::vector<double> dval;
        Buf<unsigned char> code; Buf<int> rb;
        if (build_dict8(M, doff, dval, code, rb)) {
            *kind_out = 4;
            for (int r = 0; r < M.row; ++r) {
                const int base = square ? r : rb[r];
                for (int k = M.ia[r]; k < M.ia[r + 1]; ++k)
                    if (base + doff[code[k]] != M.ja[k] || bits(dval[code[k]]) != bits(M.val[k])) return ERROR_MISC;
            }
        }
    }
    return FASP_SUCCESS;
}

int fasp_hip_amg_num_levels(const fasp_hip_amg* h) { return h ? (int)h->H.L.size() : ERROR_INPUT_PAR; }

int fasp_hip_amg_kernel_info(const fasp_hip_amg* h, int level, int which, int* kind, double* matrix_bytes)
{
    FASP_ENTRY();
    if (!h || level < 0 || level >= (int)h->L.size() || which < 0 || which > 2) return ERROR_INPUT_PAR;
    const DevLevel& D = h->L[level];
    const DevCSR& M = which == 0 ? D.A : which == 1 ? D.P : D.R;
    if (!M.ia) return ERROR_INPUT_PAR;
    int k = M.kind;
    double bytes = 12.0 * M.nnz + 4.0 * (M.row + 1.0);
    if (M.kind == 0 && M.ja16 && g_tune.ja16) bytes = 10.0 * M.nnz + 4.0 * (M.row + 1.0) + (M.jbase ? 4.0 * M.row : 0.0);
    if (M.code && g_tune.compress) { k = 4; bytes = 1.0 * M.nnz + 4.0 * (M.row + 1.0) + (M.rowbase ? 4.0 * M.row : 0.0); }
    if (M.pat && g_tune.compress) { k = 5; bytes = 2.0 * M.row + (M.rowbase ? 4.0 * M.row : 0.0) + 12.0 * M.npent; }
    if (k == 5 && g_tune.gen2 && M.nxrows >= 0 && !M.rowbase) k = 6;
    else if (k == 5 && g_tune.gen2 >= 2 && M.nxrows >= 0 && M.rowbase && (double)M.nnz <= 0.1 * g_tune.rp5_max * M.row) k = 9;
    if (k == 2 && g_tune.gen2 && M.wrows == 64 && M.wcap == 512 && (double)M.nnz <= 7.6 * M.row) k = 7;
    else if (k == 2 && g_tune.gen2 >= 2 && g_tune.xtile && M.lja16 && M.wrows == 64 && M.wcap == 512) {
        k = 10;
        bytes = 10.0 * M.nnz + 4.0 * (M.row + 1.0) + 4.0 * M.ntcols + 4.0 * ((M.row + 63) / 64 + 1.0);
    }
    else if (k == 2 && sell_active(M) && M.wrows == 64 && M.wcap == 512) {
        k = 11;
        bytes = 4.0 * (double)M.sell_slots + 1.0 * M.row + 4.0 * (2.0 * M.sell_nslice + 1.0) + 8.0 * M.sell_nv;
    }
    else if (k == 2 && g_tune.gen2 >= 2 && M.wrows == 64 && M.wcap == 512) k = 8;
    if (kind) *kind = k;
    if (matrix_bytes) *matrix_bytes = bytes;
    return FASP_SUCCESS;
}

int fasp_hip_coarse_kernel_info(const fasp_hip_amg* h, int* info)
{
    FASP_ENTRY();
    if (!h || !info) return ERROR_INPUT_PAR;
    for (int i = 0; i < 6; ++i) info[i] = h->coarse_kinfo[i];
    info[6] = g_ctx.num_cu; info[7] = 0;
    return FASP_SUCCESS;
}

int fasp_hip_bsr_coarse_kernel_info(const fasp_hip_amg_bsr* h, int* info)
{
    FASP_ENTRY();
    if (!h || !info) return ERROR_INPUT_PAR;
    for (int i = 0; i < 6; ++i) info[i] = h->coarse_kinfo[i];
    info[6] = g_ctx.num_cu; info[7] = 0;
    return FASP_SUCCESS;
}

int fasp_hip_amg_get_matrix(const fasp_hip_amg* h, int level, int which, dCSRmat* view)
{
    FASP_ENTRY();
    if (!h || !view || level < 0 || level >= (int)h->H.L.size()) return ERROR_INPUT_PAR;
    const HostLevel& L = h->H.L[level];
    if (which != 0 && !L.has_coarse) return ERROR_INPUT_PAR;
    *view = which == 0 ? L.A.view() : which == 1 ? L.P.view() : L.R.view();
    return FASP_SUCCESS;
}

int fasp_hip_amg_get_cfmark(const fasp_hip_amg* h, int level, ivector* view)
{
    FASP_ENTRY();
    if (!h || !view || level < 0 || level >= (int)h->H.L.size() || !h->H.L[level].has_coarse)
        return ERROR_INPUT_PAR;
    view->row = h->H.L[level].A.row;
    view->val = const_cast<int*>(h->H.L[level].cfmark.data());
    return FASP_SUCCESS;
}

int fasp_hip_set_rhs(fasp_hip_amg* h, const dvector* b)
{
    FASP_ENTRY();
    if (!h || !b || h->L.empty()) return ERROR_INPUT_PAR;
    const DevLevel& D0 = h->L[0];
    if (b->row != D0.nglobal) return ERROR_MAT_SIZE;
    HIPCK(hipMemcpyAsync(h->b, b->val + D0.row0, sizeof(double) * D0.nloc, hipMemcpyHostToDevice, g_ctx.stream));
    HIPCK(hipStreamSynchronize(g_ctx.stream));
    return FASP_SUCCESS;
}

int fasp_hip_set_guess(fasp_hip_amg* h, const dvector* x)
{
    FASP_ENTRY();
    if (!h || h->L.empty()) return ERROR_INPUT_PAR;
    const DevLevel& D0 = h->L[0];
    if (x) {
        if (x->row != D0.nglobal) return ERROR_MAT_SIZE;
        HIPCK(hipMemcpyAsync(h->u, x->val + D0.row0, sizeof(double) * D0.nloc, hipMemcpyHostToDevice, g_ctx.stream));
    } else {
        HIPCK(hipMemsetAsync(h->u, 0, sizeof(double) * D0.nvec, g_ctx.stream));
    }
    HIPCK(hipStreamSynchronize(g_ctx.stream));
    return FASP_SUCCESS;
}

int fasp_hip_get_solution(fasp_hip_amg* h, dvector* x)
{
    FASP_ENTRY();
    if (!h || !x || h->L.empty()) return ERROR_INPUT_PAR;
    const DevLevel& D0 = h->L[0];
    if (x->row != D0.nglobal) return ERROR_MAT_SIZE;
    HIPCK(hipMemcpyAsync(x->val + D0.row0, h->u, sizeof(double) * D0.nloc, hipMemcpyDeviceToHost, g_ctx.stream));
    HIPCK(hipStreamSynchronize(g_ctx.stream));
    return FASP_SUCCESS;
}

int fasp_hip_device_synchronize(void)
{
    FASP_ENTRY();
    if (!g_ctx.ready) return FASP_SUCCESS;
    HIPCK(hipStreamSynchronize(g_ctx.stream));
    return FASP_SUCCESS;
}

int fasp_hip_solve_resident(fasp_hip_amg* h, const ITS_param* itparam, double* hist, int hist_cap,
                            fasp_hip_stats* stats)
{
    FASP_ENTRY();
    if (!h || !itparam) return ERROR_INPUT_PAR;
    if (h->L.empty()) return ERROR_INPUT_PAR;
    int st = check_supported(itparam, &h->param);
    if (st < 0) return st;
    if (itparam->tol < SMALLREAL)
        std::printf("### WARNING: Convergence tolerance is too small! [%s:%d]\n", "ITS_CHECK", 74);
    if (itparam->maxit <= 0)
        std::printf("### WARNING: Max number of iterations must be POSITIVE! [%s:%d]\n", "ITS_CHECK", 78);

    h->ev_used = 0;
    h->use_fmg = itparam->precond_type == PREC_FMG;
    const long long ci0 = h->coarse_iters, vc0 = h->vcycles;
    Hist   H{hist, hist_cap, 0};
    PcgOut po{BIGREAL, BIGREAL, BIGREAL};
    const double t0 = wall_seconds();
    switch (itparam->itsolver_type) {
        case SOLVER_BiCGstab:
        {
            KOps K = csr_ops(h, 0, true);
            st = bicgstab_device(K, h->b, h->u, itparam->tol, itparam->maxit, itparam->print_level, &H, &po);
        } break;
        case SOLVER_GMRES:
        case SOLVER_VGMRES:
        case SOLVER_VFGMRES:
        {
            KOps K = csr_ops(h, 0, true);
            st = gmres_device(K, h->b, h->u, itparam->itsolver_type == SOLVER_VFGMRES ? 1 : itparam->itsolver_type == SOLVER_GMRES ? 3 : 0, itparam->tol,
                              itparam->abstol, itparam->maxit, (short)itparam->restart, itparam->stop_type,
                              itparam->print_level, &H, &po);
        } break;
        case SOLVER_MinRes:
        {
            KOps K = csr_ops(h, 0, true);
            st = minres_device(K, h->b, h->u, itparam->tol, itparam->abstol, itparam->maxit, itparam->stop_type,
                               itparam->print_level, &H, &po);
        } break;
        case SOLVER_GCG:
        {
            KOps K = csr_ops(h, 0, true);
            st = gcg_device(K, h->b, h->u, itparam->tol, itparam->abstol, itparam->maxit, itparam->stop_type,
                            itparam->print_level, &H, &po);
        } break;
        case SOLVER_GCR:
        {
            KOps K = csr_ops(h, 0, true);
            st = gcr_device(K, h->b, h->u, itparam->tol, itparam->abstol, itparam->maxit, (short)itparam->restart,
                            itparam->stop_type, itparam->print_level, &H, &po);
        } break;
        default:
        {
            KOps K = csr_ops(h, 0, true);
            PcgVecs V{h->b, h->u, h->p, h->t, h->r};
            st = pcg_device(K, V, itparam->tol, itparam->abstol, itparam->maxit, itparam->stop_type,
                            itparam->print_level, H, po);
        }
    }
    HIPCK(hipStreamSynchronize(g_ctx.stream));
    if (seq_err_check() < 0) return ERROR_MISC;
    const double t_solve = wall_seconds() - t0;

    if (stats) {
        stats->iters = st; stats->nhist = H.n; stats->relres = po.relres; stats->absres = po.absres;
        stats->normr0 = po.normr0; stats->solve_seconds = t_solve; stats->upload_seconds = 0.0;
        double ms = 0.0;
        for (int i = 0; i < h->ev_used; ++i) {
            float e = 0.f;
            if (hipEventElapsedTime(&e, h->ev[i].a, h->ev[i].b) == hipSuccess) ms += e;
        }
        stats->spmv_launches = h->ev_used;
        stats->spmv_ms = h->ev_used ? ms / h->ev_used : 0.0;
        stats->coarse_iters = h->coarse_iters - ci0;
        stats->vcycles = h->vcycles - vc0;
// ... 1287 lines not shown
dvector fasp_dbsr_getdiaginv(const dBSRmat* A)
{
    FASP_ENTRY();
    dvector out{0, nullptr};
    if (!A || A->nb < 1 || A->nb > 7) {
        std::fprintf(stderr, "### ERROR: fasp_dbsr_getdiaginv: block size %d not supported (1..7)\n", A ? A->nb : -1);
        return out;
    }
    out.row = A->ROW * A->nb * A->nb;
    out.val = (double*)std::calloc((size_t)std::max(out.row, 1), sizeof(double));
    (void)bsr_diaginv(A, out.val);
    return out;
}

void fasp_smoother_dbsr_jacobi1(dBSRmat* A, dvector* b, dvector* u, double* diaginv)
{
    FASP_ENTRY();
    TmpBSR M(A);
    if (!M.ok) die_bsr(__func__);
    const size_t n = (size_t)A->ROW * A->nb;
    TmpVec du(u->val, n), dun(nullptr, n), db(b->val, n), dd(diaginv, (size_t)A->ROW * A->nb * A->nb);
    BsrArgs a{}; a.x = du.d; a.y = dun.d; a.b = db.d; a.dinv = dd.d;
    launch_bsr<2>(M, a);
    dun.get(u->val);
}

double fasp_hip_time_bsr_mxv(const dBSRmat* A, int reps)
{
    FASP_ENTRY();
    TmpBSR M(A);
    if (!M.ok || reps <= 0) return -1.0;
    TmpVec dx(nullptr, (size_t)A->COL * A->nb), dy(nullptr, (size_t)A->ROW * A->nb);
    (void)hipMemsetAsync(dx.d, 0, sizeof(double) * dx.n, g_ctx.stream);
    BsrArgs a{}; a.x = dx.d; a.y = dy.d;
    hipEvent_t e0, e1;
    (void)hipEventCreate(&e0); (void)hipEventCreate(&e1);
    launch_bsr<0>(M, a); launch_bsr<0>(M, a);
    (void)hipEventRecord(e0, g_ctx.stream);
    for (int i = 0; i < reps; ++i) launch_bsr<0>(M, a);
    (void)hipEventRecord(e1, g_ctx.stream);
    (void)hipEventSynchronize(e1);
    float ms = 0.f;
    (void)hipEventElapsedTime(&ms, e0, e1);
    (void)hipEventDestroy(e0); (void)hipEventDestroy(e1);
    return (double)ms / reps;
}

void fasp_smoother_dcsr_jacobi(dvector* u, const int i_1, const int i_n, const int s, dCSRmat* A, dvector* b,
                               int L, const double w)
{
    FASP_ENTRY();
    (void)s;
    TmpCSR M(A);
    if (!M.ok) die_no_device(__func__);
    const int n = A->row;
    const int lo = std::min(i_1, i_n), hi = std::max(i_1, i_n);
    if (lo != 0 || hi != n - 1) {
        std::fprintf(stderr, "### ERROR: fasp_smoother_dcsr_jacobi (device): only full sweeps 0..n-1 supported\n");
        std::exit(ERROR_INPUT_PAR);
    }
    std::vector<double> d(n, 0.0);
    bool dup = false;
    for (int i = 0; i < n; ++i) {
        int hits = 0;
        for (int k = A->IA[i]; k < A->IA[i + 1]; ++k)
            if (A->JA[k] == i) { d[i] = A->val[k]; ++hits; }
        dup = dup || hits > 1;
    }
    M.D.dup_diag = dup;
    TmpVec du(u->val, n), du2(nullptr, n), db(b->val, n), dd(d.data(), n);
    double *x = du.d, *xo = du2.d;
    while (L--) {
        CsrArgs a{};
        a.x = x; a.y = xo; a.b = db.d; a.diag = dd.d; a.omega = w;
        launch_csr<OP_JACOBI>(M.D, a);
        std::swap(x, xo);
    }
    (void)hipStreamSynchronize(g_ctx.stream);
    (void)hipMemcpy(u->val, x, sizeof(double) * n, hipMemcpyDeviceToHost);
}

#ifdef FLOW_TIMING
extern "C" int fasp_hip_flow_times(unsigned long long* out, int n)
{
    FASP_ENTRY();
    return hipMemcpyFromSymbol(out, HIP_SYMBOL(fasp::g_flow_times), sizeof(unsigned long long) * (size_t)std::min(n, 8192)) == hipSuccess ? 0 : -1;
}
#endif

static int g_time_cold = 0;
int fasp_hip_tune(const char* key, int value)
{
    FASP_ENTRY();
    if (!key) return ERROR_INPUT_PAR;
    if (!std::strcmp(key, "maxgrid")) g_tune.maxgrid = value;
    else if (!std::strcmp(key, "xcd")) g_tune.xcd = value;
    else if (!std::strcmp(key, "gen2")) g_tune.gen2 = value;
    else if (!std::strcmp(key, "ws2_bpc")) g_tune.ws2_bpc = value;
    else if (!std::strcmp(key, "nt")) g_tune.nt = value;
    else if (!std::strcmp(key, "kind")) g_tune.kind = value;
    else if (!std::strcmp(key, "compress")) g_tune.compress = value;
    else if (!std::strcmp(key, "rpl")) g_tune.rpl = value;
    else if (!std::strcmp(key, "lds_tab")) g_tune.lds_tab = value;
    else if (!std::strcmp(key, "xcd_pat")) g_tune.xcd_pat = value;
    else if (!std::strcmp(key, "spcg_batch")) g_tune.spcg_batch = value;
    else if (!std::strcmp(key, "spcg_fused")) g_tune.spcg_fused = value;
    else if (!std::strcmp(key, "spcg_persist")) { g_tune.spcg_persist = value; if (value) g_persist_disabled = false; }
    else if (!std::strcmp(key, "spcg_test_hang")) g_tune.spcg_test_hang = value;
    else if (!std::strcmp(key, "spcg_grid")) g_tune.spcg_grid = value;
    else if (!std::strcmp(key, "small_lds")) g_tune.small_lds = value;
    else if (!std::strcmp(key, "small_onewave")) g_tune.small_onewave = value;
    else if (!std::strcmp(key, "ja16")) g_tune.ja16 = value;
    else if (!std::strcmp(key, "device_sort")) g_device_sort = value;
    else if (!std::strcmp(key, "halo_overlap")) g_halo_overlap = value;
    else if (!std::strcmp(key, "coarse_mode")) g_coarse_mode = value;
    else if (!std::strcmp(key, "coarse_split_min")) g_coarse_split_min = value;
    else if (!std::strcmp(key, "split_rows")) g_tune.split_rows = value;
    else if (!std::strcmp(key, "gs_multicolor")) g_tune.gs_multicolor = value;
    else if (!std::strcmp(key, "seq_flow")) { g_tune.seq_flow = value; if (value) g_flow_disabled = false; }
    else if (!std::strcmp(key, "ilu_smooth_fused")) g_tune.ilu_smooth_fused = value;
    else if (!std::strcmp(key, "ilu_form")) g_tune.ilu_form = value;
    else if (!std::strcmp(key, "seq_strip_kb")) g_tune.seq_strip_kb = value;
    else if (!std::strcmp(key, "seq_jobs")) g_tune.seq_jobs = value;
    else if (!std::strcmp(key, "local_square")) g_tune.local_square = value;
    else if (!std::strcmp(key, "seq_grid")) g_tune.seq_grid = value;
    else if (!std::strcmp(key, "seq_chain")) g_tune.seq_chain = value;
    else if (!std::strcmp(key, "seq_chain_n1")) g_tune.seq_chain_n1 = value;
    else if (!std::strcmp(key, "seq_chain_grid")) g_tune.seq_chain_grid = value;
    else if (!std::strcmp(key, "seq_test_hang")) g_tune.seq_test_hang = value;
    else if (!std::strcmp(key, "seq_rest_lanes")) g_tune.seq_rest_lanes = value;
    else if (!std::strcmp(key, "seq_chain_ref")) g_tune.seq_chain_ref = value;
    else if (!std::strcmp(key, "seq_spine")) g_tune.seq_spine = value;
    else if (!std::strcmp(key, "seq_partition")) g_seq_partition = value;
    else if (!std::strcmp(key, "fuse_zr")) g_tune.fuse_zr = value;
    else if (!std::strcmp(key, "fuse_presmooth")) g_tune.fuse_presmooth = value;
    else if (!std::strcmp(key, "seq_lanes")) g_tune.seq_lanes = value;
    else if (!std::strcmp(key, "lazy_coarse")) g_tune.lazy_coarse = value;
    else if (!std::strcmp(key, "xtile")) g_tune.xtile = value;
    else if (!std::strcmp(key, "rp5_max")) g_tune.rp5_max = value;
    else if (!std::strcmp(key, "rp_bpc")) g_tune.rp_bpc = value;
    else if (!std::strcmp(key, "rp_stream")) g_tune.rp_stream = value;
    else if (!std::strcmp(key, "renumber")) g_tune.renumber = value;
    else if (!std::strcmp(key, "renumber_chunk")) g_tune.renumber_chunk = value;
    else if (!std::strcmp(key, "time_cold")) g_time_cold = value;
    else if (!std::strcmp(key, "estream")) g_tune.estream = value;
    else if (!std::strcmp(key, "sell")) g_tune.sell = value;
    else if (!std::strcmp(key, "es_dbg")) g_tune.es_dbg = value;
    else if (!std::strcmp(key, "pcg_dev_beta")) g_tune.pcg_dev_beta = value;
    else if (!std::strcmp(key, "seq_chain_touch")) g_tune.seq_chain_touch = value;
    else if (!std::strcmp(key, "seq_chain_touch_t1")) g_tune.seq_chain_touch_t1 = value;
    else if (!std::strcmp(key, "seq_zero_skip")) g_tune.seq_zero_skip = value;
    else if (!std::strcmp(key, "pcg_fold")) g_tune.pcg_fold = value;
    else if (!std::strcmp(key, "spcg_spec")) g_tune.spcg_spec = value;
    else if (!std::strcmp(key, "ev_every")) g_tune.ev_every = value;
    else if (!std::strcmp(key, "rp_xcd")) g_tune.rp_xcd = value;
    else if (!std::strcmp(key, "rp_strip")) g_tune.rp_strip = value;
    else if (!std::strcmp(key, "host_parallel_min")) g_parallel_min_nnz = value;
    else if (!std::strcmp(key, "lanes")) g_tune.lanes = value;
    else if (!std::strcmp(key, "wrows")) g_tune.wrows = value;
    else if (!std::strcmp(key, "wcap")) g_tune.wcap = value;
    else return ERROR_INPUT_PAR;
    return FASP_SUCCESS;
}

int fasp_hip_sell_selftest(const dCSRmat* A, int cap_percent, int* info, double* bytes, int* ia_out, int* ja_out, double* val_out, const double* x, double* y)
{
    if (!A || !info || A->row < 0 || A->nnz < 0) return ERROR_INPUT_PAR;
    HostCSR M;
    M.row = A->row; M.col = A->col; M.nnz = A->nnz;
    M.ia.view(A->IA, (size_t)A->row + 1); M.ja.view(A->JA, (size_t)std::max(A->nnz, 1)); M.val.view(A->val, (size_t)std::max(A->nnz, 1));
    SellHost S;
    int why = 0;
    const bool ok = build_sell(M, S, cap_percent > 0 ? cap_percent : SELL_CAP_PERCENT, &why);
    info[0] = ok ? 1 : 0; info[1] = why; info[2] = S.nv; info[3] = S.vbits; info[4] = S.obits; info[5] = S.nslice;
    info[6] = ok ? (int)std::min<long long>(S.slots / 64, 0x7fffffff) : 0; info[7] = SELL_MAXV;
    if (bytes) *bytes = ok ? S.bytes(M.row) : 0.0;
    if (!ok) return FASP_SUCCESS;
    if (ia_out && ja_out && val_out) sell_decode_host(S, M.row, ia_out, ja_out, val_out);
    if (x && y) sell_mxv_host(S, M.row, x, y);
    return FASP_SUCCESS;
}

int fasp_hip_estream_selftest(const int* ia, int nrow, int nnz, int per_wave, int wmax, int* info)
{
    if (!ia || nrow < 1 || nnz < 1 || per_wave < 8 || wmax < 32) return ERROR_INPUT_PAR;
    return estream_selftest_host(ia, nrow, nnz, per_wave, wmax, info);
}

int fasp_hip_measure_ceilings(double* out, size_t bytes, int reps)
{
    FASP_ENTRY();
    if (!out || bytes < (1u << 20) || reps <= 0) return ERROR_INPUT_PAR;
    if (ctx_init() != FASP_SUCCESS) return ERROR_MISC;
    f64x2_t *p = nullptr, *q = nullptr, *r = nullptr;
    HIPCK(hipMalloc(&p, bytes)); HIPCK(hipMalloc(&q, bytes)); HIPCK(hipMalloc(&r, bytes));
    HIPCK(hipMemsetAsync(p, 0, bytes, g_ctx.stream)); HIPCK(hipMemsetAsync(q, 0, bytes, g_ctx.stream));
    HIPCK(hipMemsetAsync(r, 0, bytes, g_ctx.stream));
    const size_t n16 = bytes / 16;
    hipEvent_t e0, e1;
    HIPCK(hipEventCreate(&e0)); HIPCK(hipEventCreate(&e1));
    const int grid = 4 * g_ctx.num_cu;
    for (int which = 0; which < 3; ++which) {
        auto run = [&]() {
            if (which == 0) hipLaunchKernelGGL(k_read16, dim3(grid), dim3(BLOCK), 0, g_ctx.stream, n16, p, (double*)q);
            else if (which == 1) hipLaunchKernelGGL(k_copy16, dim3(grid), dim3(BLOCK), 0, g_ctx.stream, n16, p, q);
            else hipLaunchKernelGGL(k_triad16, dim3(grid), dim3(BLOCK), 0, g_ctx.stream, n16, 0.5, p, q, r);
        };
        run(); run();
        HIPCK(hipEventRecord(e0, g_ctx.stream));
        for (int i = 0; i < reps; ++i) run();
        HIPCK(hipEventRecord(e1, g_ctx.stream));
        HIPCK(hipEventSynchronize(e1));
        float ms = 0.f;
        HIPCK(hipEventElapsedTime(&ms, e0, e1));
        out[which] = (double)(which + 1) * (double)bytes * reps / ((double)ms * 1e-3) / 1e9;
    }
    (void)hipEventDestroy(e0); (void)hipEventDestroy(e1);
    (void)hipFree(p); (void)hipFree(q); (void)hipFree(r);
    return FASP_SUCCESS;
}

double fasp_hip_time_kernel(fasp_hip_amg* h, int kind, int level, int reps)
{
    FASP_ENTRY();
    if (!h || level < 0 || level >= (int)h->L.size() || reps <= 0) return -1.0;
    DevLevel& D = h->L[level];
    const int n = D.A.row;
    hipEvent_t e0, e1;
    if (hipEventCreate(&e0) != hipSuccess || hipEventCreate(&e1) != hipSuccess) return -1.0;
    double* x = D.xa; double* y = D.xb; double* w = D.w;
    auto run = [&]() {
        switch (kind) {
            case 0: d_mxv(D.A, x, y); break;
            case 1: d_aAxpy(-1.0, D.A, x, y); break;
            case 2: { CsrArgs a{}; a.x = x; a.y = y; a.b = w; a.diag = D.diag; a.omega = 0.6667; launch_csr<OP_JACOBI>(D.A, a); } break;
            case 3: hipLaunchKernelGGL(k_dot, dim3(vec_grid(n)), dim3(BLOCK), 0, g_ctx.stream, n, x, y, g_ctx.d_partials); break;
            case 4: d_axpy(n, 0.5, x, y); break;
            case 5: { CsrArgs a{}; a.x = x; a.y = y; a.dotv = x; a.partials = g_ctx.d_partials; launch_csr<OP_MXV_DOT>(D.A, a); } break;
            case 6: if (D.R.ia) d_mxv(D.R, w, h->L[level + 1].xa); break;
            case 7: if (D.P.ia) d_aAxpy(1.0, D.P, h->L[level + 1].xa, y); break;
            case 8:
                if (D.A.val) hipLaunchKernelGGL(k_read16, dim3(2048), dim3(BLOCK), 0, g_ctx.stream, (size_t)D.A.nnz / 2, (const f64x2_t*)D.A.val, y);
                break;
            case 10: case 11: case 12: case 13: (void)seq_sweep(h, level, kind - 10, 1, 1.0); break;
            default: break;
        }
    };
    (void)hipMemsetAsync(x, 0, sizeof(double) * n, g_ctx.stream);
    (void)hipMemsetAsync(y, 0, sizeof(double) * n, g_ctx.stream);
    (void)hipMemsetAsync(w, 0, sizeof(double) * n, g_ctx.stream);
    double* const keep_b = D.b; double* const keep_x = D.x;
    if (kind >= 10) { D.b = w; D.x = x; }
    if (g_time_cold) {
        double* big = nullptr;
        const size_t bigb = (size_t)512 << 20;
        if (hipMalloc(&big, bigb + 4096) != hipSuccess) return -1.0;
        (void)hipMemsetAsync(big, 0, bigb, g_ctx.stream);
        double tot = 0.0;
        for (int i = 0; i < reps + 1; ++i) {
            if (g_time_cold >= 2) (void)hipMemsetAsync(big, 0, bigb, g_ctx.stream);
            else hipLaunchKernelGGL(k_read16, dim3(1024), dim3(BLOCK), 0, g_ctx.stream, bigb / 16, (const f64x2_t*)big, big + bigb / 8);
            (void)hipEventRecord(e0, g_ctx.stream);
            run();
            (void)hipEventRecord(e1, g_ctx.stream);
            (void)hipEventSynchronize(e1);
            float ms1 = 0.f;
            (void)hipEventElapsedTime(&ms1, e0, e1);
            if (i >= 1) tot += ms1;
        }
        (void)hipFree(big);
        D.b = keep_b; D.x = keep_x;
        (void)hipEventDestroy(e0); (void)hipEventDestroy(e1);
        return tot / reps;
    }
    run(); run();
    (void)hipEventRecord(e0, g_ctx.stream);
    for (int i = 0; i < reps; ++i) run();
    (void)hipEventRecord(e1, g_ctx.stream);
    (void)hipEventSynchronize(e1);
    D.b = keep_b; D.x = keep_x;
    float ms = 0.f;
    (void)hipEventElapsedTime(&ms, e0, e1);
    (void)hipEventDestroy(e0); (void)hipEventDestroy(e1);
    return (double)ms / reps;
}


static int row_op_host(DevLevel& D, int which, int op, const double* x, const double* b, double* y, double* y2, double scalar, double* red)
{
    if (which < 0 || which > 2 || op < 0 || op > 8 || !x || !y) return ERROR_INPUT_PAR;
    const DevCSR& M = which == 0 ? D.A : which == 1 ? D.P : D.R;
    if (!M.ia || ((op == 5 || op == 6) && which != 0) || ((op == 1 || op >= 5) && !b) || (op == 8 && !y2)) return ERROR_INPUT_PAR;
    const size_t nr = (size_t)std::max(M.row, 1), nc = (size_t)std::max(M.col, 1);
    double *dx = nullptr, *db = nullptr, *dy = nullptr, *dy2 = nullptr;
    int st = FASP_SUCCESS;
    auto run = [&]() -> int {
        HIPCK(hipMalloc(&dx, 8 * nc)); HIPCK(hipMalloc(&db, 8 * nr)); HIPCK(hipMalloc(&dy, 8 * nr)); HIPCK(hipMalloc(&dy2, 8 * nr));
        HIPCK(hipMemcpy(dx, x, 8 * (size_t)M.col, hipMemcpyHostToDevice));
        HIPCK(hipMemcpy(dy, y, 8 * (size_t)M.row, hipMemcpyHostToDevice));
        if (b) HIPCK(hipMemcpy(db, b, 8 * (size_t)M.row, hipMemcpyHostToDevice));
        CsrArgs a{};
        a.x = dx; a.y = dy; a.b = db;
        int G = 0;
        bool have_red = false;
        switch (op) {
            case 0: G = launch_csr<OP_MXV>(M, a); break;
// ... 110 lines not shown
```

### include/fasp_hip_dev.h

```cpp
#ifndef FASP_HIP_DEV_H
#define FASP_HIP_DEV_H
#include "fasp_hip.h"
#ifdef __cplusplus
extern "C" {
#endif

double fasp_hip_time_kernel(fasp_hip_amg* h, int kind, int level, int reps);
double fasp_hip_time_matrix(const dCSRmat* A, int op, int reps, int* kind_out);
double fasp_hip_seq_schedule_selftest(const dCSRmat* A, const int* seq, int ns, int strip_kb, int lanes, int spine, int* info);
int fasp_hip_cluster_order(const dCSRmat* A, int chunk, int* order);
int fasp_hip_permute_csr(const dCSRmat* A, const int* rperm, const int* cinv, int* ia, int* ja, double* val);
double fasp_hip_seq_chain_selftest(const dCSRmat* A, const int* seq, int ns, int n1_blocks, int form, double w, int* info, double* out_u);
int fasp_hip_measure_ceilings(double* out, size_t bytes, int reps);

int    fasp_hip_ilu_resident_count(void);
double fasp_hip_ilu_time(ILU_data* iludata, int which, int reps, double* info);
int    fasp_hip_bsr_amg_get_ilu(const fasp_hip_amg_bsr* h, int level, ILU_data* view);
int    fasp_hip_bsr_amg_ilu_info(const fasp_hip_amg_bsr* h, int level, double info[6]);
double fasp_hip_bsr_amg_ilu_smooth_time(fasp_hip_amg_bsr* h, int level, int reps);

int fasp_hip_tune(const char* key, int value);
int fasp_hip_coarse_kernel_info(const fasp_hip_amg* h, int* info);
int fasp_hip_bsr_coarse_kernel_info(const fasp_hip_amg_bsr* h, int* info);

int fasp_hip_comm_stats(double* out8, int reset);
int fasp_hip_comm_timing(int on);

int fasp_hip_dist_plan(fasp_hip_amg* h, int rank, int nranks, int min_rows);
int fasp_hip_dist_level_info(const fasp_hip_amg* h, int level, int* info);
int fasp_hip_dist_get_matrix(const fasp_hip_amg* h, int level, int which, dCSRmat* view);
int fasp_hip_dist_get_list(const fasp_hip_amg* h, int level, int which, ivector* view);
int  fasp_hip_estream_selftest(const int* ia, int nrow, int nnz, int per_wave, int wmax, int* info);
int  fasp_hip_sell_selftest(const dCSRmat* A, int cap_percent, int* info, double* bytes, int* ia_out, int* ja_out, double* val_out, const double* x, double* y);
int  fasp_hip_level_op(fasp_hip_amg* h, int level, int which, int op, const double* x, const double* b, double* y, double* y2, double scalar, double* red);
int  fasp_hip_matrix_op(const dCSRmat* A, int op, const double* x, const double* b, double* y, double* y2, double scalar, double* red, int* kind_out);
int  fasp_hip_comm_selftest(void);

#ifdef __cplusplus
}
#endif
#endif
```

Baseline: 482.5 million.

## Fold coarse PCG init and final residual check into persistent kernel

The persistent coarse-grid PCG kernel now does the initialization itself when started, so the separate init launch goes away. After convergence it also computes the true residual b-Au and its norm inside the kernel, which replaces the host-side speculative residual and dot launches. The sync words move behind the state so that one device-to-host copy returns both the state and the error flags, and the per-launch sync memset is dropped. This removes several small launches and copies per coarse solve, at the cost of more complex in-kernel epoch handshakes and a fallback path when a hang is detected.

```diff
diff --git a/faspsolver_amd/__init__.py b/faspsolver_amd/__init__.py
--- a/faspsolver_amd/__init__.py
+++ b/faspsolver_amd/__init__.py
@@ -20,7 +20,7 @@
     "fasp_solver_dbsr_pcg", "fasp_solver_dbsr_pbcgs", "fasp_solver_dbsr_pgmres", "fasp_solver_dbsr_pvgmres",
     "fasp_solver_dbsr_pvfgmres", "fasp_hip_bsr_precond_setup", "fasp_hip_bsr_precond_fct", "fasp_hip_bsr_precond_free",
     "fasp_hip_param_input", "fasp_fwrapper_dcsr_krylov_amg_", "fasp_dcsrvec_read2", "fasp_dvec_read",
-    "fasp_dbsr_read", "fasp_dcoo_read", "fasp_dcoo_read1", "fasp_dcoo_shift_read", "fasp_dmtx_read", "fasp_dmtxsym_read", "fasp_dvec_write", "fasp_dcsr_write_coo", "fasp_dcsrvec_write2", "fasp_fwrapper_dcsr_amg_", "fasp_fwrapper_dbsr_krylov_amg_", "fasp_hip_free_bsr", "fasp_hip_comm_selftest", "fasp_hip_amg_kernel_info", "fasp_hip_coarse_kernel_info", "fasp_hip_bsr_coarse_kernel_info", "fasp_hip_coding_selftest", "fasp_solver_amg", "fasp_solver_famg", "fasp_hip_amg_solve", "fasp_precond_diag", "fasp_precond_dbsr_diag", "fasp_solver_dcsr_itsolver", "fasp_solver_dcsr_krylov", "fasp_solver_dcsr_krylov_diag", "fasp_solver_dbsr_itsolver", "fasp_solver_dbsr_krylov", "fasp_solver_dbsr_krylov_diag", "fasp_hip_mxv_csr", "fasp_hip_mxv_bsr", "fasp_solver_matfree_init", "fasp_solver_pcg", "fasp_solver_pbcgs", "fasp_solver_pgcg", "fasp_solver_pminres", "fasp_solver_pgmres", "fasp_solver_pvgmres", "fasp_solver_pvfgmres", "fasp_solver_itsolver", "fasp_solver_krylov", "fasp_solver_dcsr_pcg", "fasp_solver_dcsr_pminres", "fasp_solver_dcsr_pgcg", "fasp_solver_dcsr_pgcr", "fasp_solver_dcsr_pbcgs", "fasp_solver_dcsr_pgmres", "fasp_solver_dcsr_pvgmres",
+    "fasp_dbsr_read", "fasp_dcoo_read", "fasp_dcoo_read1", "fasp_dcoo_shift_read", "fasp_dmtx_read", "fasp_dmtxsym_read", "fasp_dvec_write", "fasp_dcsr_write_coo", "fasp_dcsrvec_write2", "fasp_fwrapper_dcsr_amg_", "fasp_fwrapper_dbsr_krylov_amg_", "fasp_hip_free_bsr", "fasp_hip_comm_selftest", "fasp_hip_amg_kernel_info", "fasp_hip_coarse_kernel_info", "fasp_hip_coarse_tail_info", "fasp_hip_bsr_coarse_kernel_info", "fasp_hip_coding_selftest", "fasp_solver_amg", "fasp_solver_famg", "fasp_hip_amg_solve", "fasp_precond_diag", "fasp_precond_dbsr_diag", "fasp_solver_dcsr_itsolver", "fasp_solver_dcsr_krylov", "fasp_solver_dcsr_krylov_diag", "fasp_solver_dbsr_itsolver", "fasp_solver_dbsr_krylov", "fasp_solver_dbsr_krylov_diag", "fasp_hip_mxv_csr", "fasp_hip_mxv_bsr", "fasp_solver_matfree_init", "fasp_solver_pcg", "fasp_solver_pbcgs", "fasp_solver_pgcg", "fasp_solver_pminres", "fasp_solver_pgmres", "fasp_solver_pvgmres", "fasp_solver_pvfgmres", "fasp_solver_itsolver", "fasp_solver_krylov", "fasp_solver_dcsr_pcg", "fasp_solver_dcsr_pminres", "fasp_solver_dcsr_pgcg", "fasp_solver_dcsr_pgcr", "fasp_solver_dcsr_pbcgs", "fasp_solver_dcsr_pgmres", "fasp_solver_dcsr_pvgmres",
     "fasp_solver_dcsr_pvfgmres", "fasp_hip_precond_setup", "fasp_hip_precond_fct", "fasp_hip_precond_free",
     "fasp_hip_time_bsr_mxv", "fasp_solver_dbsr_krylov_amg", "fasp_hip_bsr_amg_create", "fasp_hip_bsr_amg_create_host",
     "fasp_hip_bsr_amg_destroy", "fasp_hip_bsr_amg_num_levels", "fasp_hip_bsr_amg_get_matrix",
@@ -143,6 +143,7 @@
     L.fasp_hip_coding_selftest.argtypes = [P(T.dCSRmat), P(C.c_int)]
     L.fasp_hip_amg_kernel_info.argtypes = [C.c_void_p, C.c_int, C.c_int, P(C.c_int), P(C.c_double)]
     L.fasp_hip_coarse_kernel_info.argtypes = [C.c_void_p, P(C.c_int)]
+    L.fasp_hip_coarse_tail_info.argtypes = [C.c_void_p, P(C.c_double)]
     L.fasp_hip_bsr_coarse_kernel_info.argtypes = [C.c_void_p, P(C.c_int)]
     L.fasp_solver_amg.argtypes = [P(T.dCSRmat), P(T.dvector), P(T.dvector), P(T.AMG_param)]
     L.fasp_hip_amg_solve.argtypes = [C.c_void_p, P(T.dvector), P(T.dvector), P(T.AMG_param), T.c_double_p,
@@ -440,6 +441,12 @@
             raise RuntimeError("fasp_hip_coarse_kernel_info failed")
         return tuple(info)
 
+    def coarse_tail_info(self):
+        info = (C.c_double * 4)()
+        if lib().fasp_hip_coarse_tail_info(self.h, info) < 0:
+            raise RuntimeError("fasp_hip_coarse_tail_info failed")
+        return tuple(info)
+
     def precond(self, r):
         r = np.ascontiguousarray(r, dtype=np.float64)
         z = np.zeros_like(r)
diff --git a/faspsolver_amd/csrc/coarse_cg.hip.h b/faspsolver_amd/csrc/coarse_cg.hip.h
--- a/faspsolver_amd/csrc/coarse_cg.hip.h
+++ b/faspsolver_amd/csrc/coarse_cg.hip.h
@@ -73,12 +73,12 @@
     }
     bool ok = hipMalloc(&P.vals, tot * sizeof(double)) == hipSuccess && hipMalloc(&P.cols, tot * sizeof(unsigned short)) == hipSuccess &&
               hipMalloc(&P.wrow, sizeof(int) * (size_t)nw * 8) == hipSuccess && hipMalloc(&P.wend, sizeof(int) * (size_t)nw * 8) == hipSuccess &&
-              hipMalloc(&P.t2, sizeof(double) * 4 * (size_t)m) == hipSuccess && hipMalloc(&P.sync, 1024) == hipSuccess;
+              hipMalloc(&P.t2, sizeof(double) * 8 * (size_t)m) == hipSuccess && hipMalloc(&P.sync, 1024) == hipSuccess;
     if (ok) ok = hipMemcpy(P.vals, vals.data(), tot * sizeof(double), hipMemcpyHostToDevice) == hipSuccess &&
                  hipMemcpy(P.cols, cols.data(), tot * sizeof(unsigned short), hipMemcpyHostToDevice) == hipSuccess &&
                  hipMemcpy(P.wrow, wrow.data(), sizeof(int) * (size_t)nw * 8, hipMemcpyHostToDevice) == hipSuccess &&
                  hipMemcpy(P.wend, wend.data(), sizeof(int) * (size_t)nw * 8, hipMemcpyHostToDevice) == hipSuccess;
-    if (ok) ok = hipMemset(P.t2, 0, sizeof(double) * 4 * (size_t)m) == hipSuccess;
+    if (ok) ok = hipMemset(P.t2, 0, sizeof(double) * 8 * (size_t)m) == hipSuccess && hipMemset(P.sync, 0, 1024) == hipSuccess;
     if (!ok) return false;
     P.NE = NE; P.nblocks = nblocks; P.ok = true;
     return true;
@@ -214,13 +214,21 @@
     const bool fused = g_tune.spcg_fused && m <= 8000 && A.val && A.ja && !A.code && !A.pat;
     bool persist = fused && g_tune.spcg_persist && !g_persist_disabled && !comm_shares_devices() &&
                    (size_t)m * 24 <= 150 * 1024 && build_persist_plan(h, (int)(&D - &h->L[0]));
-    if (!h->spcg_state) HIPCK(hipMalloc(&h->spcg_state, sizeof(SpcgState)));
+    const bool tail = persist && g_tune.spcg_tail;
+    const bool x_zero0 = D.x_zero;
+    bool start_in_kernel = tail;
+    if (persist) { auto& TI = h->persist.tail_info; TI[0] = std::nan(""); TI[1] = TI[2] = TI[3] = 0.0; }
+    SpcgInitArgs ia{};
+    ia.m = m; ia.x_zero = x_zero0 ? 1 : 0; ia.MaxIt = MaxIt; ia.tol = tol; ia.maxdiff = maxdiff;
+    ia.b = b; ia.u = u; ia.r = r; ia.p = p; ia.u_best = u_best;
+    if (!h->spcg_state) {
+        HIPCK(hipMalloc(&h->spcg_state, sizeof(SpcgState) + 1024));
+        HIPCK(hipMemset(h->spcg_state, 0, sizeof(SpcgState) + 1024));
+    }
+    ia.st = h->spcg_state;
     if (fused) {
         if (!D.x_zero) d_resid(A, u, b, r);
-        SpcgInitArgs ia{};
-        ia.m = m; ia.x_zero = D.x_zero ? 1 : 0; ia.MaxIt = MaxIt; ia.tol = tol; ia.maxdiff = maxdiff;
-        ia.b = b; ia.u = u; ia.r = r; ia.p = p; ia.u_best = u_best; ia.st = h->spcg_state;
-        hipLaunchKernelGGL(k_spcg_init, dim3(1), dim3(512), 0, s, ia);
+        if (!start_in_kernel) hipLaunchKernelGGL(k_spcg_init, dim3(1), dim3(512), 0, s, ia);
         D.x_zero = false;
         goto ITERATE;
     }
@@ -266,14 +274,22 @@
         for (;;) {
             if (persist) {
                 auto& PP = h->persist;
+                unsigned* const sync_tail = reinterpret_cast<unsigned*>(reinterpret_cast<char*>(h->spcg_state) + sizeof(SpcgState));
+                if (g_tune.spcg_launches > 0) { PP.launches = (unsigned)g_tune.spcg_launches & 0x1fffffu; g_tune.spcg_launches = 0; }
                 PP.launches = (PP.launches + 1u) & 0x1fffffu;
-                if (PP.launches == 0u) { HIPCK(hipMemsetAsync(PP.t2, 0, sizeof(double) * 4 * (size_t)m, s)); PP.launches = 1u; }
+                if (PP.launches == 0u) {
+                    HIPCK(hipMemsetAsync(PP.t2, 0, sizeof(double) * 8 * (size_t)m, s));
+                    HIPCK(hipMemsetAsync(sync_tail, 0, 1024, s));
+                    PP.launches = 1u;
+                }
                 SpcgPersistArgs pa{};
                 pa.epoch0 = PP.launches << 11;
                 pa.m = m; pa.max_steps = MaxIt + 2; pa.nblocks = PP.nblocks; pa.st = h->spcg_state;
-                pa.r = r; pa.p = p; pa.u = u; pa.u_best = u_best; pa.t2 = PP.t2; pa.sync = PP.sync;
+                pa.r = r; pa.p = p; pa.u = u; pa.u_best = u_best; pa.t2 = PP.t2; pa.sync = tail ? sync_tail : PP.sync;
                 pa.vals = PP.vals; pa.cols = PP.cols; pa.wrow = PP.wrow; pa.wend = PP.wend;
-                HIPCK(hipMemsetAsync(PP.sync, 0, 1024, s));
+                pa.start = start_in_kernel ? 1 : 0; pa.tail = tail ? 1 : 0;
+                pa.x_zero = x_zero0 ? 1 : 0; pa.MaxIt = MaxIt; pa.tol = tol; pa.maxdiff = maxdiff; pa.b = b; pa.t = t;
+                if (!tail) HIPCK(hipMemsetAsync(PP.sync, 0, 1024, s));
                 pa.u_lds = (sizeof(double) * 4 * (size_t)m + 1024 <= 160 * 1024) ? 1 : 0;
                 const size_t lds = sizeof(double) * (pa.u_lds ? 4 : 3) * (size_t)m;
                 int lst;
@@ -311,23 +327,44 @@
                 h->coarse_kinfo[0] = 7; h->coarse_kinfo[1] = m <= 512 * 4 ? 4 : m <= 512 * 10 ? 10 : 0; h->coarse_kinfo[2] = 0;
             }
             bool spec_rr = false;
-            if (persist && g_tune.spcg_spec) {
+            if (persist && !tail && g_tune.spcg_spec) {
                 d_resid(A, u, b, t);
                 if (d_dot_to(m, t, t, 14, false) < 0) return ERROR_MISC;
                 spec_rr = true;
             }
-            HIPCK(hipMemcpyAsync(g_ctx.h_part, h->spcg_state, sizeof(SpcgState), hipMemcpyDeviceToHost, s));
             static_assert(sizeof(SpcgState) % 8 == 0 && sizeof(SpcgState) + 24 <= sizeof(double) * 64, "the error word and the speculative norm travel behind the state");
-            if (persist) HIPCK(hipMemcpyAsync(reinterpret_cast<char*>(g_ctx.h_part) + sizeof(SpcgState), h->persist.sync, 16, hipMemcpyDeviceToHost, s));
+            HIPCK(hipMemcpyAsync(g_ctx.h_part, h->spcg_state, sizeof(SpcgState) + (persist && tail ? 24 : 0), hipMemcpyDeviceToHost, s));
+            if (persist && !tail) HIPCK(hipMemcpyAsync(reinterpret_cast<char*>(g_ctx.h_part) + sizeof(SpcgState), h->persist.sync, 16, hipMemcpyDeviceToHost, s));
             if (spec_rr) HIPCK(hipMemcpyAsync(reinterpret_cast<char*>(g_ctx.h_part) + sizeof(SpcgState) + 16, g_ctx.d_red + 14, 8, hipMemcpyDeviceToHost, s));
             HIPCK(hipStreamSynchronize(s));
             std::memcpy(&S, g_ctx.h_part, sizeof(S));
+            if (persist) {
+                unsigned ew[4];
+                std::memcpy(ew, reinterpret_cast<char*>(g_ctx.h_part) + sizeof(SpcgState), 16);
+                const unsigned launch = h->persist.launches;
+                const bool raised = ew[3] == launch;
+                if (tail) {
+                    spec_rr = ew[2] == launch;
+                    if (raised && start_in_kernel && ew[1] != launch) {
+                        hipLaunchKernelGGL(k_spcg_init, dim3(1), dim3(512), 0, s, ia);
+                        HIPCK(hipMemcpyAsync(g_ctx.h_part, h->spcg_state, sizeof(SpcgState), hipMemcpyDeviceToHost, s));
+                        HIPCK(hipStreamSynchronize(s));
+                        std::memcpy(&S, g_ctx.h_part, sizeof(S));
+                        spec_rr = false;
+                        if (S.stop == SPCG_RUN) S.stop = SPCG_HANG;
+                    }
+                    else if (raised && S.stop != SPCG_RUN) g_persist_disabled = true;
+                    start_in_kernel = false;
+                }
+                if (raised && S.stop == SPCG_RUN) S.stop = SPCG_HANG;
+            }
             double spec_val = 0.0;
             if (spec_rr) std::memcpy(&spec_val, reinterpret_cast<char*>(g_ctx.h_part) + sizeof(SpcgState) + 16, 8);
             if (persist) {
-                unsigned ew[4];
-                std::memcpy(ew, reinterpret_cast<char*>(g_ctx.h_part) + sizeof(SpcgState), 16);
-                if (ew[3] != 0u && S.stop == SPCG_RUN) S.stop = SPCG_HANG;
+                auto& TI = h->persist.tail_info;
+                if (TI[3] == 0.0) TI[1] = (double)S.stop;
+                TI[3] += 1.0;
+                TI[2] = (double)h->persist.launches;
             }
             iter = S.iter; absres_best = S.absres_best; iter_best = S.iter_best;
             batch = batch_next;
@@ -338,7 +375,7 @@
 #ifdef SPCG_PERSIST_STAMPS
             if (persist) {
                 unsigned dbg[64];
-                (void)hipMemcpy(dbg, h->persist.sync, sizeof(dbg), hipMemcpyDeviceToHost);
+                (void)hipMemcpy(dbg, tail ? (const void*)(reinterpret_cast<char*>(h->spcg_state) + sizeof(SpcgState)) : (const void*)h->persist.sync, sizeof(dbg), hipMemcpyDeviceToHost);
                 std::printf("[persist stamps, 10 ns ticks, %d steps] lead:", S.iter);
                 for (int q = 0; q < 8; ++q) std::printf(" %u", dbg[32 + q]);
                 std::printf(" | block 1:");
@@ -387,6 +424,7 @@
                     d_resid(A, u, b, r);
                     if (d_dot(m, r, r, red) < 0) return ERROR_MISC;
                 }
+                h->persist.tail_info[0] = red[0];
                 absres = std::sqrt(red[0]);
                 relres = absres / normr0;
                 if (relres < tol) break;
diff --git a/faspsolver_amd/csrc/device_csr.hip.h b/faspsolver_amd/csrc/device_csr.hip.h
--- a/faspsolver_amd/csrc/device_csr.hip.h
+++ b/faspsolver_amd/csrc/device_csr.hip.h
@@ -1005,7 +1005,7 @@
     return build_estream(H.ia.data(), H.row, H.nnz, D);
 }
 
-struct Tuning { int ilu_smooth_fused = 1, gen2 = 2, ws2_bpc = 3, maxgrid = -1, xcd = 16, nt = 1, kind = -1, lanes = -1, wrows = -1, wcap = -1, compress = 1, rpl = -1, lds_tab = 1, xcd_pat = 64, spcg_batch = 16, small_lds = 1, ja16 = 1, spcg_fused = 1, spcg_grid = 0, spcg_persist = 1, split_rows = 0, gs_multicolor = 0, seq_flow = 1, seq_strip_kb = 0, seq_jobs = 1, seq_spine = 1, seq_grid = 0, seq_chain = 1, seq_chain_n1 = 0, seq_chain_grid = 0, seq_chain_ref = 0, seq_test_hang = 0, seq_rest_lanes = 0, local_square = 1, fuse_zr = 1, fuse_presmooth = 1, seq_lanes = 0, xtile = 1, rp5_max = 45, rp_bpc = 5, rp_xcd = -1, rp_strip = 2, spcg_test_hang = 0, small_onewave = 4, lazy_coarse = 1, rp_stream = -1, renumber = 1, renumber_chunk = 262144, pcg_dev_beta = 1, spcg_spec = 1, ev_every = 4, pcg_fold = 1, seq_chain_touch = 8, seq_chain_touch_t1 = 1, seq_zero_skip = 1, estream = 1, es_dbg = 0, ilu_form = -1, sell = 1; };
+struct Tuning { int ilu_smooth_fused = 1, gen2 = 2, ws2_bpc = 3, maxgrid = -1, xcd = 16, nt = 1, kind = -1, lanes = -1, wrows = -1, wcap = -1, compress = 1, rpl = -1, lds_tab = 1, xcd_pat = 64, spcg_batch = 16, small_lds = 1, ja16 = 1, spcg_fused = 1, spcg_grid = 0, spcg_persist = 1, split_rows = 0, gs_multicolor = 0, seq_flow = 1, seq_strip_kb = 0, seq_jobs = 1, seq_spine = 1, seq_grid = 0, seq_chain = 1, seq_chain_n1 = 0, seq_chain_grid = 0, seq_chain_ref = 0, seq_test_hang = 0, seq_rest_lanes = 0, local_square = 1, fuse_zr = 1, fuse_presmooth = 1, seq_lanes = 0, xtile = 1, rp5_max = 45, rp_bpc = 5, rp_xcd = -1, rp_strip = 2, spcg_test_hang = 0, small_onewave = 4, lazy_coarse = 1, rp_stream = -1, renumber = 1, renumber_chunk = 262144, pcg_dev_beta = 1, spcg_spec = 1, spcg_tail = 1, spcg_launches = 0, ev_every = 4, pcg_fold = 1, seq_chain_touch = 8, seq_chain_touch_t1 = 1, seq_zero_skip = 1, estream = 1, es_dbg = 0, ilu_form = -1, sell = 1; };
 static Tuning g_tune;
 
 template <class K>
diff --git a/faspsolver_amd/csrc/hierarchy.hip.h b/faspsolver_amd/csrc/hierarchy.hip.h
--- a/faspsolver_amd/csrc/hierarchy.hip.h
+++ b/faspsolver_amd/csrc/hierarchy.hip.h
@@ -77,7 +77,8 @@
     int                  spcg_last_iters = 0;
     SpcgState*           spcg_state = nullptr;
     struct Persist { bool tried = false, ok = false; int NE = 0, nblocks = 0; double* vals = nullptr; unsigned short* cols = nullptr;
-                     int *wrow = nullptr, *wend = nullptr; double* t2 = nullptr; unsigned* sync = nullptr; unsigned launches = 0; } persist;
+                     int *wrow = nullptr, *wend = nullptr; double* t2 = nullptr; unsigned* sync = nullptr; unsigned launches = 0;
+                     double tail_info[4] = {0.0, 0.0, 0.0, 0.0};  } persist;
     std::vector<double>  amli_coef;
     std::vector<int>     level_cycle_type;
     bool                 use_fmg = false;
diff --git a/faspsolver_amd/csrc/small_solvers.hip.h b/faspsolver_amd/csrc/small_solvers.hip.h
--- a/faspsolver_amd/csrc/small_solvers.hip.h
+++ b/faspsolver_amd/csrc/small_solvers.hip.h
@@ -1784,6 +1784,12 @@
     double*    t2;
     unsigned*  sync;
     unsigned   epoch0;
+    int        start;
+    int        tail;
+    int        x_zero, MaxIt;
+    double     tol, maxdiff;
+    const double* b;
+    double*    t;
     const double*         vals;
     const unsigned short* cols;
     const int*            wrow;
@@ -1841,7 +1847,8 @@
     __shared__ int s_hang;
     typedef unsigned int pu32x4 __attribute__((ext_vector_type(4)));
     SpcgState& S = *a.st;
-    if (S.stop != SPCG_RUN) return;
+    if (!a.start && S.stop != SPCG_RUN) return;
+    const unsigned launch = a.epoch0 >> 11;
 
     double   v[NE];
     unsigned cpk[NE / 2];
@@ -1859,17 +1866,52 @@
         if (lane < 8) { endsv = a.wend[gw * 8 + lane]; rowsv = a.wrow[gw * 8 + lane]; }
         my_rows = __popcll(__ballot(lane < 8 && rowsv >= 0));
     }
-    for (int i = tid; i < m; i += NT) { sp[i] = a.p[i]; sr[i] = a.r[i]; }
     const bool u_lds = a.u_lds != 0;
-    if (lead && u_lds) for (int i = tid; i < m; i += NT) su[i] = a.u[i];
-    double temp1 = S.temp1;
-    const double absres_best0 = S.absres_best, normr0 = S.normr0, tol = S.tol, maxdiff = S.maxdiff;
-    const int    it0 = S.iter, stag = S.stag, MaxIt = S.MaxIt;
-    double best = absres_best0;
-    int    iter_best = S.iter_best;
-    double o_tp = S.tp, o_rr = S.rr, o_uu = S.uu, o_pp = S.pp, o_maxu = S.maxu, o_nan = S.nan, o_alpha = S.alpha,
-           o_absres = S.absres, o_relres = S.relres, o_temp1_prev = S.temp1_prev;
-    int steps_done = 0, my_stop = SPCG_RUN;
+    double temp1, best, normr0, tol, maxdiff;
+    int    it0, stag, MaxIt, iter_best;
+    double o_tp, o_rr, o_uu, o_pp, o_maxu, o_nan, o_alpha, o_absres, o_relres, o_temp1_prev;
+    if (a.start) {
+        double v0[1] = {0.0};
+        for (int i = tid; i < m; i += NT) {
+            const double ri = a.x_zero ? a.b[i] : a.r[i];
+            sp[i] = ri; sr[i] = ri;
+            v0[0] += ri * ri;
+            if (lead) {
+                a.u_best[i] = 0.0;
+                if (a.x_zero) { if (u_lds) su[i] = 0.0; else a.u[i] = 0.0; }
+                else if (u_lds) su[i] = a.u[i];
+            }
+        }
+        blk_reduce_dpp<1, NW>(v0, sh);
+        const double absres0 = sqrt(v0[0]);
+        temp1 = v0[0]; best = 1e+20; normr0 = fmax(1e-20, absres0) ; tol = a.tol; maxdiff = a.maxdiff;
+        it0 = 0; stag = 1; MaxIt = a.MaxIt; iter_best = 0;
+        o_tp = 0.0; o_rr = v0[0]; o_uu = 0.0; o_pp = 0.0; o_maxu = 0.0; o_nan = 0.0; o_alpha = 0.0;
+        o_absres = 1e+20; o_relres = absres0 / normr0; o_temp1_prev = v0[0];
+        if (o_relres < tol) {
+            if (lead) {
+                for (int i = tid; i < m; i += NT) { a.r[i] = sr[i]; a.p[i] = sp[i]; if (u_lds) a.u[i] = su[i]; }
+                if (tid == 0) {
+                    SpcgState Z{};
+                    Z.temp1 = temp1; Z.temp1_prev = temp1; Z.absres_best = 1e+20; Z.normr0 = normr0; Z.tol = tol; Z.maxdiff = maxdiff;
+                    Z.absres = 1e+20; Z.relres = o_relres; Z.rr = temp1;
+                    Z.iter = 0; Z.iter_best = 0; Z.stag = 1; Z.MaxIt = MaxIt; Z.pad = 0;
+                    Z.stop = SPCG_ZERO_RHS;
+                    S = Z;
+                    a.sync[1] = launch;
+                }
+            }
+            return;
+        }
+    } else {
+        for (int i = tid; i < m; i += NT) { sp[i] = a.p[i]; sr[i] = a.r[i]; }
+        if (lead && u_lds) for (int i = tid; i < m; i += NT) su[i] = a.u[i];
+        temp1 = S.temp1; best = S.absres_best; normr0 = S.normr0; tol = S.tol; maxdiff = S.maxdiff;
+        it0 = S.iter; stag = S.stag; MaxIt = S.MaxIt; iter_best = S.iter_best;
+        o_tp = S.tp; o_rr = S.rr; o_uu = S.uu; o_pp = S.pp; o_maxu = S.maxu; o_nan = S.nan; o_alpha = S.alpha;
+        o_absres = S.absres; o_relres = S.relres; o_temp1_prev = S.temp1_prev;
+    }
+    int steps_done = 0, my_stop = SPCG_RUN, end_flag = SPCG_RUN;
     if (tid == 0) {
         s_hang = 0;
         if (lead)
@@ -1883,36 +1925,39 @@
 #define STAMP(q) do { } while (0)
 #endif
 
+    auto product = [&](const __amdgpu_buffer_rsrc_t tr, const unsigned ep, const bool resid) __attribute__((always_inline)) {
+        double acc = 0.0;
+        int    j = 0;
+        int    next_end = __builtin_amdgcn_readlane(endsv, 0);
+#pragma unroll
+        for (int k = 0; k < NE; ++k) {
+            const unsigned off = (k & 1) ? (cpk[k >> 1] >> 16) : (cpk[k >> 1] & 0xffffu);
+            const double x = *reinterpret_cast<const double*>(reinterpret_cast<const char*>(sp) + off);
+            acc += v[k] * x;
+            if ((k & 7) == 7) __builtin_amdgcn_sched_barrier(0);
+            if (k + 1 == next_end) {
+                double ssum = wave_sum_to_lane63(acc);
+                const int row = __builtin_amdgcn_readlane(rowsv, j);
+                if (lane == 63) {
+                    if (resid) ssum = a.b[row] - ssum;
+                    const unsigned long long bits = (unsigned long long)__double_as_longlong(ssum);
+                    const pu32x4 rec = {(unsigned)bits, ep, (unsigned)(bits >> 32), ep};
+                    __builtin_amdgcn_raw_buffer_store_b128(rec, tr, row * 16, 0, 16 );
+                }
+                acc = 0.0;
+                ++j;
+                next_end = (j < 8) ? __builtin_amdgcn_readlane(endsv, j & 7) : -1;
+                if (j >= my_rows) next_end = -1;
+            }
+        }
+    };
+
     for (int step = 0; step < a.max_steps; ++step) {
         const int par = step & 1;
         const unsigned ep = a.epoch0 + (unsigned)step + 1u;
         const __amdgpu_buffer_rsrc_t tr =
             __builtin_amdgcn_make_buffer_rsrc(a.t2 + (size_t)par * 2 * m, 0, (int)((unsigned)m * 16u), 0x00020000);
-        if (!lead && my_rows > 0 && my_stop == SPCG_RUN) {
-            double acc = 0.0;
-            int    j = 0;
-            int    next_end = __builtin_amdgcn_readlane(endsv, 0);
-#pragma unroll
-            for (int k = 0; k < NE; ++k) {
-                const unsigned off = (k & 1) ? (cpk[k >> 1] >> 16) : (cpk[k >> 1] & 0xffffu);
-                const double x = *reinterpret_cast<const double*>(reinterpret_cast<const char*>(sp) + off);
-                acc += v[k] * x;
-                if ((k & 7) == 7) __builtin_amdgcn_sched_barrier(0);
-                if (k + 1 == next_end) {
-                    const double ssum = wave_sum_to_lane63(acc);
-                    const int row = __builtin_amdgcn_readlane(rowsv, j);
-                    if (lane == 63) {
-                        const unsigned long long bits = (unsigned long long)__double_as_longlong(ssum);
-                        const pu32x4 rec = {(unsigned)bits, ep, (unsigned)(bits >> 32), ep};
-                        __builtin_amdgcn_raw_buffer_store_b128(rec, tr, row * 16, 0, 16 );
-                    }
-                    acc = 0.0;
-                    ++j;
-                    next_end = (j < 8) ? __builtin_amdgcn_readlane(endsv, j & 7) : -1;
-                    if (j >= my_rows) next_end = -1;
-                }
-            }
-        }
+        if (!lead && my_rows > 0 && my_stop == SPCG_RUN) product(tr, ep, false);
         STAMP(0);
         {
             const unsigned long long t0 = __builtin_amdgcn_s_memrealtime();
@@ -1956,14 +2001,14 @@
             }
             if (hung) {
                 s_hang = 1;
-                __hip_atomic_store(g_err, 1u, __ATOMIC_RELAXED, __HIP_MEMORY_SCOPE_AGENT);
+                __hip_atomic_store(g_err, launch, __ATOMIC_RELAXED, __HIP_MEMORY_SCOPE_AGENT);
             }
         }
         lds_barrier();
         STAMP(1);
         if (s_hang) { my_stop = SPCG_HANG; break; }
         const int flag = s_flag;
-        if (flag != SPCG_RUN) break;
+        if (flag != SPCG_RUN) { end_flag = flag; break; }
         if (my_stop != SPCG_RUN) break;
         STAMP(2);
         double v1[1] = {0.0};
@@ -2085,6 +2130,47 @@
 #endif
 #undef STAMP
 
+    if (a.tail && end_flag == SPCG_CONV) {
+        const __amdgpu_buffer_rsrc_t ur = __builtin_amdgcn_make_buffer_rsrc(a.t2 + (size_t)4 * m, 0, (int)((unsigned)m * 16u), 0x00020000);
+        const __amdgpu_buffer_rsrc_t rr_ = __builtin_amdgcn_make_buffer_rsrc(a.t2 + (size_t)6 * m, 0, (int)((unsigned)m * 16u), 0x00020000);
+        const unsigned ep_u = a.epoch0 + 2046u, ep_r = a.epoch0 + 2047u;
+        auto collect = [&](const __amdgpu_buffer_rsrc_t tr, const unsigned ep, double* dst) {
+            const unsigned long long t0 = __builtin_amdgcn_s_memrealtime();
+            bool hung = false;
+#pragma unroll 1
+            for (int i = tid; i < m && !hung; i += NT)
+                for (;;) {
+                    const pu32x4 q = __builtin_amdgcn_raw_buffer_load_b128(tr, i * 16, 0, 16 );
+                    if (q.y == ep && q.w == ep) { dst[i] = __longlong_as_double((long long)(((unsigned long long)q.z << 32) | q.x)); break; }
+                    if (__builtin_amdgcn_s_memrealtime() - t0 > 200000000ull) { hung = true; break; }
+                }
+            if (hung) {
+                s_hang = 1;
+                __hip_atomic_store(g_err, launch, __ATOMIC_RELAXED, __HIP_MEMORY_SCOPE_AGENT);
+            }
+            lds_barrier();
+            return s_hang != 0;
+        };
+        if (lead) {
+            for (int i = tid; i < m; i += NT) {
+                const unsigned long long bits = (unsigned long long)__double_as_longlong(u_lds ? su[i] : a.u[i]);
+                const pu32x4 rec = {(unsigned)bits, ep_u, (unsigned)(bits >> 32), ep_u};
+                __builtin_amdgcn_raw_buffer_store_b128(rec, ur, i * 16, 0, 16 );
+            }
+            if (!collect(rr_, ep_r, st)) {
+                double n2[1] = {0.0};
+                for (int i = tid; i < m; i += NT) { const double ti = st[i]; a.t[i] = ti; n2[0] += ti * ti; }
+                blk_reduce_dpp<1, NW>(n2, sh);
+                if (tid == 0) {
+                    *reinterpret_cast<double*>(a.sync + 4) = n2[0];
+                    a.sync[2] = launch;
+                }
+            }
+        } else if (!collect(ur, ep_u, sp)) {
+            if (my_rows > 0) product(rr_, ep_r, true);
+        }
+    }
+
     if (lead) {
         for (int i = tid; i < m; i += NT) { a.r[i] = sr[i]; a.p[i] = sp[i]; if (u_lds) a.u[i] = su[i]; }
         if (tid == 0) {
@@ -2092,8 +2178,10 @@
             S.alpha = o_alpha; S.absres = o_absres; S.relres = o_relres;
             S.absres_best = best; S.iter_best = iter_best; S.iter = it0 + steps_done;
             S.temp1_prev = o_temp1_prev;
-            S.temp1 = (my_stop == SPCG_DIV0) ? S.temp1 : temp1;
+            S.temp1 = (my_stop == SPCG_DIV0 && !a.start) ? S.temp1 : temp1;
             S.stop = my_stop;
+            if (a.start) { S.normr0 = normr0; S.tol = tol; S.maxdiff = maxdiff; S.stag = stag; S.MaxIt = MaxIt; S.pad = 0; }
+            a.sync[1] = launch;
         }
     }
 }
diff --git a/faspsolver_amd/csrc/solver.hip b/faspsolver_amd/csrc/solver.hip
--- a/faspsolver_amd/csrc/solver.hip
+++ b/faspsolver_amd/csrc/solver.hip
@@ -552,6 +552,14 @@
     if (!h || !info) return ERROR_INPUT_PAR;
     for (int i = 0; i < 6; ++i) info[i] = h->coarse_kinfo[i];
     info[6] = g_ctx.num_cu; info[7] = 0;
+    return FASP_SUCCESS;
+}
+
+int fasp_hip_coarse_tail_info(const fasp_hip_amg* h, double* info)
+{
+    FASP_ENTRY();
+    if (!h || !info) return ERROR_INPUT_PAR;
+    for (int i = 0; i < 4; ++i) info[i] = h->persist.tail_info[i];
     return FASP_SUCCESS;
 }
 
@@ -2145,6 +2153,8 @@
     else if (!std::strcmp(key, "seq_zero_skip")) g_tune.seq_zero_skip = value;
     else if (!std::strcmp(key, "pcg_fold")) g_tune.pcg_fold = value;
     else if (!std::strcmp(key, "spcg_spec")) g_tune.spcg_spec = value;
+    else if (!std::strcmp(key, "spcg_tail")) g_tune.spcg_tail = value;
+    else if (!std::strcmp(key, "spcg_launches")) g_tune.spcg_launches = value;
     else if (!std::strcmp(key, "ev_every")) g_tune.ev_every = value;
     else if (!std::strcmp(key, "rp_xcd")) g_tune.rp_xcd = value;
     else if (!std::strcmp(key, "rp_strip")) g_tune.rp_strip = value;
diff --git a/include/fasp_hip_dev.h b/include/fasp_hip_dev.h
--- a/include/fasp_hip_dev.h
+++ b/include/fasp_hip_dev.h
@@ -21,6 +21,7 @@
 
 int fasp_hip_tune(const char* key, int value);
 int fasp_hip_coarse_kernel_info(const fasp_hip_amg* h, int* info);
+int fasp_hip_coarse_tail_info(const fasp_hip_amg* h, double* info);
 int fasp_hip_bsr_coarse_kernel_info(const fasp_hip_amg_bsr* h, int* info);
 
 int fasp_hip_comm_stats(double* out8, int reset);
```

Result: no change. 478.8 million (-0.8%).
